# MKimiSH/video-filler

Measured on AMD Instinct MI355X. Metric: netG+netD fwd+bwd images/sec, 128x128 center-mask, higher is better.
Workload: dtype f32

## Files before the change

include/vf_hip.h:

```cpp
#ifndef VF_HIP_H
#define VF_HIP_H
#include <stddef.h>
#include <stdint.h>
#ifdef __cplusplus
extern "C" {
#endif

typedef struct vf_ctx vf_ctx;

enum { VF_ACT_NONE = 0, VF_ACT_LRELU = 1, VF_ACT_RELU = 2, VF_ACT_TANH = 3, VF_ACT_SIGMOID = 4 };

const char* vf_last_error(void);
int vf_version(void);
int vf_ctx_create(vf_ctx** out, int device, void* stream);
int vf_ctx_destroy(vf_ctx* ctx);
int vf_ctx_set_mfma_mode(vf_ctx* ctx, int mode);
int vf_ctx_set_stream(vf_ctx* ctx, void* stream);
int vf_ctx_set_workspace(vf_ctx* ctx, void* ptr, size_t bytes);
size_t vf_workspace_bytes_hint(void);
int vf_stream_synchronize(vf_ctx* ctx);
int vf_malloc(void** out, size_t bytes);
int vf_free(void* ptr);
int vf_memcpy_h2d(vf_ctx* ctx, void* dst, const void* src, size_t bytes);
int vf_memcpy_d2h(vf_ctx* ctx, void* dst, const void* src, size_t bytes);
// ... 192 lines not shown
                     float* pred_mapped, int B, int C, int fs, int overlapPred);

enum {
  VF_METRICS_N = 0, VF_METRICS_SSE = 1, VF_METRICS_SAE = 2, VF_METRICS_SSIM_Q = 3, VF_METRICS_SSIM_N = 4,
  VF_METRICS_FLICKER = 5, VF_METRICS_COLS = 6
};
int vf_frame_metrics(vf_ctx* ctx, const void* a, const void* b, int kind, int N, int C, int H, int W, int vh, int vw,
                     const unsigned char* mask, int clip, int64_t* table);

int vf_channel_copy(vf_ctx* ctx, const float* src, int Csrc, int c_src, float* dst, int Cdst, int c_dst, int Ccopy,
                    int64_t npix);
int vf_noise_fill(vf_ctx* ctx, float* out, int64_t n, uint64_t seed, const int32_t* counter_dev, uint64_t counter,
                  int normal);

int vf_wgrad_group_begin(vf_ctx* ctx);
int vf_wgrad_group_end(vf_ctx* ctx);
int vf_wgrad_group_abort(vf_ctx* ctx);
int vf_wgrad_group_count(vf_ctx* ctx, int* count);
int vf_wgrad_group_end_partial(vf_ctx* ctx, int count);

int vf_bias_grad_plan(int64_t P, int C, int* cq, int* rows_per_block, int* gx, int* gy);
int vf_bias_grad_multi(vf_ctx* ctx, const void* desc_dev, int n, int blocks1, int blocks2);

typedef struct vf_comm vf_comm;
#define VF_COMM_ID_BYTES 128
int vf_comm_available(void);
int vf_comm_unique_id(void* id128);
int vf_comm_init(vf_comm** out, const void* id128, int world, int rank);
int vf_comm_world(const vf_comm* c);
int vf_comm_rank(const vf_comm* c);
int vf_comm_allreduce_async(vf_comm* c, vf_ctx* ctx, void* buf, int64_t count, int dtype, int op, int* ticket);
int vf_comm_allreduce_avg_async(vf_comm* c, vf_ctx* ctx, float* buf, int64_t n, int* ticket);
int vf_comm_reduce_scatter_avg_async(vf_comm* c, vf_ctx* ctx, float* buf, int64_t shard_count, int* ticket);
int vf_comm_allgather_async(vf_comm* c, vf_ctx* ctx, float* buf, int64_t shard_count, int* ticket);
int vf_comm_broadcast_async(vf_comm* c, vf_ctx* ctx, float* buf, int64_t count, int root, int* ticket);
int vf_comm_wait(vf_comm* c, vf_ctx* ctx, int ticket);
int vf_comm_allreduce_inline(vf_comm* c, vf_ctx* ctx, void* buf, int64_t count, int dtype, int op);
int vf_comm_broadcast(vf_comm* c, vf_ctx* ctx, void* buf, int64_t count, int dtype, int root);
int vf_comm_barrier(vf_comm* c, vf_ctx* ctx);
int vf_comm_destroy(vf_comm* c);

int vf_prof_begin(vf_ctx* ctx);
int vf_prof_end(vf_ctx* ctx);
int vf_prof_count(void);
int vf_prof_get(int i, char* name, int name_cap, int64_t* launches, double* ms, double* flops, double* bytes);

enum { VF_L_CONV = 1, VF_L_FULLCONV = 2, VF_L_BN = 3, VF_L_ACT = 4, VF_L_VIEW = 5 };
typedef struct vf_layer_desc {
  int kind;
  int nin, nout;
  int k, stride, pad;
  int act;
  float slope;
  float eps, momentum;
} vf_layer_desc;
typedef struct vf_net vf_net;
int vf_net_create(vf_ctx* ctx, vf_net** out, const vf_layer_desc* layers, int nlayers, int B, int C, int H, int W);
int vf_net_destroy(vf_net* net);
int vf_net_reshape(vf_net* net, int B, int C, int H, int W);
int vf_net_parameters(vf_net* net, float** params, float** grads, int64_t* count);
int vf_net_bind_parameters(vf_net* net, float* params, float* grads, int64_t count);
int64_t vf_net_param_offset(const vf_net* net, int layer, int which, int64_t* length);
int vf_net_bn_running(vf_net* net, int layer, float** running_mean, float** running_var);
int vf_net_bind_bn_running(vf_net* net, int layer, float* running_mean, float* running_var);
int vf_net_bn_saved(vf_net* net, int layer, float** save_mean, float** save_invstd);
int vf_net_training(vf_net* net, int train);
int vf_net_zero_grad(vf_net* net);
int vf_net_zero_conv_biases(vf_net* net, vf_net* other);
int vf_net_forward(vf_net* net, const float* x, const float** y);
int vf_net_backward(vf_net* net, const float* x, const float* gy, const float** gx);
int vf_net_update_grad_input(vf_net* net, const float* x, const float* gy, const float** gx);
int vf_net_set_skip_input_grad(vf_net* net, int on);
int vf_net_set_batch_groups(vf_net* net, int G);
int vf_net_update_grad_input_group(vf_net* net, const float* x, const float* gy, int g, int G, const float** gx);
int vf_net_plan_size(const vf_net* net);
int vf_net_layer_has_act_bits(const vf_net* net, int layer);
int vf_net_bucket_split(const vf_net* net, double frac, int* plan_index, int64_t* flat_offset);
int vf_net_backward_range(vf_net* net, const float* x, const float* gy, int hi, int lo, int need_input_grad, const float** gx);
int vf_net_backward_split(vf_net* net, const float* x, const float* gy, int k, int need_input_grad, const float** gx);
int vf_net_backward_finish(vf_net* net);
int vf_net_set_fused_adam(vf_net* net, int on, int* count);
int vf_net_fused_adam_range(const vf_net* net, int i, int64_t* offset, int64_t* length);
int vf_net_adam_fused(vf_net* net, float* m, float* v, double beta1, double beta2, double eps, const int32_t* t_dev, int keep_grad);
int vf_net_fused_adam_pack_size(const vf_net* net, int64_t* floats);
int vf_net_fused_adam_pack(vf_net* net, float* segment);
int vf_net_adam_fused_gathered(vf_net* net, const float* all_segments, int world, int64_t seg_stride, float* m, float* v, double beta1,
                               double beta2, double eps, const int32_t* t_dev, int keep_grad);
int vf_net_fused_adam_rows_ok(const vf_net* net, int row_world);
int vf_net_fused_adam_row_range(const vf_net* net, int i, int row_rank, int row_world, int64_t* offset, int64_t* length);
int vf_net_forward_wait_fused(vf_net* net, vf_comm* comm, int ticket);
int vf_net_adam_fused_gathered_rows(vf_net* net, const float* all_segments, int world, int64_t seg_stride, float* m, float* v, double beta1,
                                    double beta2, double eps, const int32_t* t_dev, int keep_grad, int row_rank, int row_world);
int vf_net_set_sync_bn(vf_net* net, vf_comm* comm, int world, int force);
int vf_net_set_weight_planes_managed(vf_net* net, int on);
int vf_net_refresh_weight_planes(vf_net* net);
int vf_net_set_planes_gate(double min_gflop_per_pass, int min_rows);
int vf_net_layer_output(vf_net* net, int layer, const float** y);
int vf_net_layer_grad_input(vf_net* net, int layer, const float** gx);
int vf_net_layer_shape(const vf_net* net, int layer, int* B, int* C, int* H, int* W, int* Co, int* Ho, int* Wo);
int vf_net_bind_output(vf_net* net, int layer, float* y);
typedef int (*vf_net_act_observer)(void* user, int layer, float* y, int64_t numel);
int vf_net_set_act_observer(vf_net* net, vf_net_act_observer fn, void* user);

int vf_trace_available(void);
int vf_trace_enable(int on);
int vf_range_push(const char* name);
int vf_range_pop(void);
int vf_mark(const char* message);
int vf_range_depth(void);

#ifdef __cplusplus
}
#endif
#endif
```

video-filler_amd/_lib.py:

```python
import ctypes as C
import os
import re

_HERE = os.path.dirname(os.path.abspath(__file__))
_HEADER = os.path.join(_HERE, "..", "include", "vf_hip.h")

vp, f32, i32, i64, f64, sz, u64 = C.c_void_p, C.c_float, C.c_int, C.c_int64, C.c_double, C.c_size_t, C.c_uint64

SIGNATURES = {
    "vf_last_error": (C.c_char_p, []),
    "vf_version": (i32, []),
    "vf_ctx_create": (i32, [C.POINTER(vp), i32, vp]),
    "vf_ctx_destroy": (i32, [vp]),
    "vf_ctx_set_mfma_mode": (i32, [vp, i32]),
    "vf_ctx_set_stream": (i32, [vp, vp]),
    "vf_ctx_set_workspace": (i32, [vp, vp, sz]),
    "vf_workspace_bytes_hint": (sz, []),
    "vf_stream_synchronize": (i32, [vp]),
    "vf_malloc": (i32, [C.POINTER(vp), sz]),
    "vf_free": (i32, [vp]),
    "vf_memcpy_h2d": (i32, [vp, vp, vp, sz]),
    "vf_memcpy_d2h": (i32, [vp, vp, vp, sz]),
    "vf_zero": (i32, [vp, vp, sz]),
    "vf_zero_segments": (i32, [vp, vp, vp, vp, i32]),
# ... 60 lines not shown
    "vf_png_decode_workspace_bytes": (i32, [vp, vp, i32, i32, C.POINTER(sz), C.POINTER(sz)]),
    "vf_png_decode": (i32, [vp, vp, vp, i32, i32, vp, vp, vp, sz, vp, sz, vp]),
    "vf_png_bytes_to_float": (i32, [vp, vp, vp, i64]),
    "vf_png_workspace_bytes": (i32, [i32, i32, i32, i32, C.POINTER(sz), C.POINTER(sz)]),
    "vf_png_encode": (i32, [vp, vp, i32, i32, i32, i32, i32, vp, sz, vp, sz, vp]),
    "vf_jpeg_encode_workspace_bytes": (i32, [i32, i32, i32, i32, i32, C.POINTER(sz), C.POINTER(sz)]),
    "vf_jpeg_encode": (i32, [vp, vp, i32, i32, i32, i32, i32, i32, i32, vp, sz, vp, sz, vp]),
    "vf_jpeg_encode_opts_workspace_bytes": (i32, [i32] * 8 + [C.POINTER(sz), C.POINTER(sz)]),
    "vf_jpeg_encode_opts": (i32, [vp, vp] + [i32] * 10 + [vp, sz, vp, sz, vp]),
    "vf_gif_workspace_bytes": (i32, [i32, i32, i32, i32, C.POINTER(sz), C.POINTER(sz)]),
    "vf_gif_encode": (i32, [vp, vp, i32, i32, i32, i32, i32, i32, vp, sz, vp, sz, vp]),
    "vf_display_workspace_bytes": (i32, [i32] * 9 + [C.POINTER(sz)]),
    "vf_display_tensor": (i32, [vp, vp, i32, vp] + [i32] * 8 + [f64, i32, f64, i32, i32]),
    "vf_center_finish": (i32, [vp] * 6 + [i32] * 4),
    "vf_frame_metrics": (i32, [vp, vp, vp] + [i32] * 7 + [vp, i32, vp]),
    "vf_channel_copy": (i32, [vp, vp, i32, i32, vp, i32, i32, i32, i64]),
    "vf_noise_fill": (i32, [vp, vp, i64, u64, vp, u64, i32]),
    "vf_bce_fwd": (i32, [vp, vp, f32, i32, vp]),
    "vf_bce_bwd": (i32, [vp, vp, f32, vp, i32]),
    "vf_bce_fwd_bwd": (i32, [vp, vp, f32, f32, i32, i32, vp, vp, vp]),
    "vf_mse_fwd": (i32, [vp, vp, vp, i64, vp]),
    "vf_mse_bwd": (i32, [vp, vp, vp, vp, i64]),
    "vf_recon_grad_mix": (i32, [vp, vp, vp, vp, vp, f32, f32, f32, i32, i32, i32, i64, vp]),
    "vf_gdl_fwd": (i32, [vp, vp, vp, i32, i32, i32, i32, vp]),
    "vf_gdl_bwd": (i32, [vp, vp, vp, vp, i32, i32, i32, i32]),
    "vf_masked_mse_fwd": (i32, [vp, vp, vp, vp, f32, i64, vp]),
    "vf_masked_mse_bwd": (i32, [vp, vp, vp, vp, f32, vp, i64]),
    "vf_adam_step": (i32, [vp, vp, vp, vp, vp, i64, f64, f64, f64, f64, vp]),
    "vf_adam_prep": (i32, [vp, f64, f64, f64, vp]),
    "vf_adam_apply": (i32, [vp, vp, vp, vp, vp, i64, f64, f64, f64, vp]),
    "vf_adam_apply_ranges": (i32, [vp, vp, vp, vp, vp, C.POINTER(i64), C.POINTER(i64), i32, f64, f64, f64, vp]),
    "vf_wgrad_adam_outer_supported": (i32, [i32, i32, i32]),
    "vf_wgrad_adam_outer": (i32, [vp, vp, vp, i32, i32, i32, vp, vp, vp, vp, f64, f64, f64, vp]),
    "vf_wgrad_adam_outer_gathered": (i32, [vp, vp, vp, i32, i32, i64, i32, i32, vp, vp, vp, vp, C.c_float, f64, f64, f64, vp]),
    "vf_wgrad_adam_outer_rows": (i32, [vp, vp, vp, i32, i32, i64, i32, i32, i32, i32, vp, vp, vp, vp, C.c_float, f64, f64, f64, vp]),
    "vf_conv_is_fast": (i32, [i32, i32, i32, i32, i32]),
    "vf_conv2d_bwd_weight_planes": (i32, [vp, vp, vp, vp, vp, vp, vp, i32, i32, i32, i32, i32, i32, i32, i32, f32]),
    "vf_deconv2d_bwd_weight_planes": (i32, [vp, vp, vp, vp, vp, vp, vp, i32, i32, i32, i32, i32, i32, i32, i32, f32]),
    "vf_comm_available": (i32, []),
    "vf_comm_unique_id": (i32, [vp]),
    "vf_comm_init": (i32, [C.POINTER(vp), vp, i32, i32]),
    "vf_comm_world": (i32, [vp]),
    "vf_comm_rank": (i32, [vp]),
    "vf_comm_allreduce_async": (i32, [vp, vp, vp, i64, i32, i32, C.POINTER(i32)]),
    "vf_comm_allreduce_avg_async": (i32, [vp, vp, vp, i64, C.POINTER(i32)]),
    "vf_comm_reduce_scatter_avg_async": (i32, [vp, vp, vp, i64, C.POINTER(i32)]),
    "vf_comm_allgather_async": (i32, [vp, vp, vp, i64, C.POINTER(i32)]),
    "vf_comm_broadcast_async": (i32, [vp, vp, vp, i64, i32, C.POINTER(i32)]),
    "vf_comm_wait": (i32, [vp, vp, i32]),
    "vf_comm_allreduce_inline": (i32, [vp, vp, vp, i64, i32, i32]),
    "vf_comm_broadcast": (i32, [vp, vp, vp, i64, i32, i32]),
    "vf_comm_barrier": (i32, [vp, vp]),
    "vf_comm_destroy": (i32, [vp]),
    "vf_net_create": (i32, [vp, C.POINTER(vp), vp, i32, i32, i32, i32, i32]),
    "vf_net_destroy": (i32, [vp]),
    "vf_net_parameters": (i32, [vp, C.POINTER(vp), C.POINTER(vp), C.POINTER(i64)]),
    "vf_net_param_offset": (i64, [vp, i32, i32, C.POINTER(i64)]),
    "vf_net_bn_running": (i32, [vp, i32, C.POINTER(vp), C.POINTER(vp)]),
    "vf_net_training": (i32, [vp, i32]),
    "vf_net_zero_grad": (i32, [vp]),
    "vf_net_forward": (i32, [vp, vp, C.POINTER(vp)]),
    "vf_net_backward": (i32, [vp, vp, vp, C.POINTER(vp)]),
    "vf_net_update_grad_input": (i32, [vp, vp, vp, C.POINTER(vp)]),
    "vf_net_layer_output": (i32, [vp, i32, C.POINTER(vp)]),
    "vf_net_layer_grad_input": (i32, [vp, i32, C.POINTER(vp)]),
    "vf_net_layer_shape": (i32, [vp, i32] + [C.POINTER(i32)] * 7),
    "vf_net_reshape": (i32, [vp, i32, i32, i32, i32]),
    "vf_net_bind_parameters": (i32, [vp, vp, vp, i64]),
    "vf_net_bind_bn_running": (i32, [vp, i32, vp, vp]),
    "vf_net_bn_saved": (i32, [vp, i32, C.POINTER(vp), C.POINTER(vp)]),
    "vf_net_zero_conv_biases": (i32, [vp, vp]),
    "vf_net_set_skip_input_grad": (i32, [vp, i32]),
    "vf_net_set_batch_groups": (i32, [vp, i32]),
    "vf_net_update_grad_input_group": (i32, [vp, vp, vp, i32, i32, C.POINTER(vp)]),
    "vf_net_plan_size": (i32, [vp]),
    "vf_net_layer_has_act_bits": (i32, [vp, i32]),
    "vf_net_bucket_split": (i32, [vp, f64, C.POINTER(i32), C.POINTER(i64)]),
    "vf_net_backward_range": (i32, [vp, vp, vp, i32, i32, i32, C.POINTER(vp)]),
    "vf_net_backward_split": (i32, [vp, vp, vp, i32, i32, C.POINTER(vp)]),
    "vf_net_backward_finish": (i32, [vp]),
    "vf_net_set_fused_adam": (i32, [vp, i32, C.POINTER(i32)]),
    "vf_net_fused_adam_range": (i32, [vp, i32, C.POINTER(i64), C.POINTER(i64)]),
    "vf_net_adam_fused": (i32, [vp, vp, vp, f64, f64, f64, vp, i32]),
    "vf_net_fused_adam_pack_size": (i32, [vp, C.POINTER(i64)]),
    "vf_net_fused_adam_pack": (i32, [vp, vp]),
    "vf_net_adam_fused_gathered": (i32, [vp, vp, i32, i64, vp, vp, f64, f64, f64, vp, i32]),
    "vf_net_fused_adam_rows_ok": (i32, [vp, i32]),
    "vf_net_fused_adam_row_range": (i32, [vp, i32, i32, i32, C.POINTER(i64), C.POINTER(i64)]),
    "vf_net_forward_wait_fused": (i32, [vp, vp, i32]),
    "vf_net_adam_fused_gathered_rows": (i32, [vp, vp, i32, i64, vp, vp, f64, f64, f64, vp, i32, i32, i32]),
    "vf_net_set_sync_bn": (i32, [vp, vp, i32, i32]),
    "vf_net_set_weight_planes_managed": (i32, [vp, i32]),
    "vf_net_refresh_weight_planes": (i32, [vp]),
    "vf_net_set_planes_gate": (i32, [f64, i32]),
    "vf_net_bind_output": (i32, [vp, i32, vp]),
    "vf_net_set_act_observer": (i32, [vp, vp, vp]),
    "vf_trace_available": (i32, []),
    "vf_trace_enable": (i32, [i32]),
    "vf_range_push": (i32, [C.c_char_p]),
    "vf_range_pop": (i32, []),
    "vf_mark": (i32, [C.c_char_p]),
    "vf_range_depth": (i32, []),
    "vf_wgrad_group_count": (i32, [vp, C.POINTER(i32)]),
    "vf_wgrad_group_end_partial": (i32, [vp, i32]),
    "vf_prof_begin": (i32, [vp]),
    "vf_prof_end": (i32, [vp]),
    "vf_prof_count": (i32, []),
    "vf_prof_get": (i32, [i32, C.c_char_p, i32, C.POINTER(i64), C.POINTER(f64), C.POINTER(f64), C.POINTER(f64)]),
}


def header_symbols():
    with open(_HEADER) as fh:
        text = re.sub(r"/\*.*?\*/", "", fh.read(), flags=re.S)
    return sorted(set(re.findall(r"\b(vf_[a-z0-9_]+)\s*\(", text)))


def lib_path():
    return os.environ.get("VF_HIP_LIB") or os.path.join(_HERE, "lib", "libvf_hip.so")


_LIB = None


def load():
    global _LIB
    if _LIB is None:
        path = lib_path()
        if not os.path.exists(path):
            raise RuntimeError(
                "video-filler_amd: %s is missing — run `python -c 'import __graft_entry__ as g; g.build()'` "
                "(hipcc --offload-arch=gfx950).  There is no CPU fallback." % path)
        lib = C.CDLL(path)
        for name, (res, args) in SIGNATURES.items():
            fn = getattr(lib, name)
            fn.restype = res
            fn.argtypes = args
        _LIB = lib
    return _LIB


class VfError(RuntimeError):
    pass


def check(rc):
    if rc != 0:
        raise VfError(load().vf_last_error().decode())
```

video-filler_amd/build.py:

```python
import glob
import os
import subprocess
import sys

HERE = os.path.dirname(os.path.abspath(__file__))
SRC = ["vf_core.hip", "vf_bn.hip", "vf_conv.hip", "vf_conv_generic.hip", "vf_pipeline.hip", "vf_image.hip", "vf_jpeg.hip", "vf_png.hip", "vf_png_decode.hip", "vf_jpeg_enc.hip", "vf_gif.hip", "vf_display.hip", "vf_metrics.hip", "vf_pgemm.hip", "vf_conv_thin.hip", "vf_comm.hip", "vf_wgrad_small.hip", "vf_smallm.hip", "vf_trace.hip", "vf_net.hip"]
HIPCC = os.environ.get("HIPCC", "/opt/rocm/bin/hipcc")
FLAGS = ["--offload-arch=gfx950", "-O3", "-std=c++17", "-fPIC", "-fvisibility=hidden", "-ffp-contract=off",
         "-Wall", "-Wno-unused-function", "-Xclang", "-target-feature", "-Xclang", "-packed-fp32-ops"]


def lib_path():
    return os.path.join(HERE, "lib", "libvf_hip.so")


def build(force=False, verbose=False):
    csrc = os.path.join(HERE, "csrc")
    objdir = os.path.join(HERE, "lib", "obj")
    os.makedirs(objdir, exist_ok=True)
    hdrs = glob.glob(os.path.join(csrc, "*.h")) + [os.path.join(HERE, "..", "include", "vf_hip.h")]
    hdr_m = max(os.path.getmtime(h) for h in hdrs)
    objs, rebuilt = [], False
    procs = []
    for s in SRC:
        src = os.path.join(csrc, s)
        obj = os.path.join(objdir, s.replace(".hip", ".o"))
        objs.append(obj)
        if force or not os.path.exists(obj) or os.path.getmtime(obj) < max(os.path.getmtime(src), hdr_m):
            cmd = [HIPCC, *FLAGS, "-c", src, "-o", obj]
            if verbose:
                print(" ".join(cmd))
            procs.append((s, subprocess.Popen(cmd, stdout=subprocess.PIPE, stderr=subprocess.STDOUT)))
            rebuilt = True
    for s, p in procs:
        out, _ = p.communicate()
        if p.returncode != 0:
            sys.stderr.write(out.decode())
            raise RuntimeError("hipcc failed on " + s)
        if verbose and out:
            print("\n".join(ln for ln in out.decode().split("\n") if "-packed-fp32-ops' is not a recognized feature" not in ln))
    so = lib_path()
    if rebuilt or not os.path.exists(so):
        subprocess.check_call([HIPCC, "--offload-arch=gfx950", "-shared", "-fPIC", "-o", so, *objs, "-ldl"])
    return so


if __name__ == "__main__":
    print(build(force="--force" in sys.argv, verbose=True))
```

video-filler_amd/cnet.py:

```python
import ctypes as C

import torch

from . import _lib, nn
from .backend import ACT, get_backend, param_version, tensor_from_ptr, to_nhwc

VF_L_CONV, VF_L_FULLCONV, VF_L_BN, VF_L_ACT, VF_L_VIEW = 1, 2, 3, 4, 5


class LayerDesc(C.Structure):
    _fields_ = [("kind", C.c_int), ("nin", C.c_int), ("nout", C.c_int), ("k", C.c_int), ("stride", C.c_int), ("pad", C.c_int),
                ("act", C.c_int), ("slope", C.c_float), ("eps", C.c_float), ("momentum", C.c_float)]


_OBSERVER = C.CFUNCTYPE(C.c_int, C.c_void_p, C.c_int, C.c_void_p, C.c_int64)


def layer_descs(mods):
    arr = (LayerDesc * len(mods))()
    for i, m in enumerate(mods):
        if isinstance(m, nn.SpatialConvolution):
            arr[i] = LayerDesc(VF_L_FULLCONV if m._is_full else VF_L_CONV, m.nInputPlane, m.nOutputPlane, m.kH, m.dH, m.padH, 0, 0.0, 0.0, 0.0)
        elif isinstance(m, nn.SpatialBatchNormalization):
            arr[i] = LayerDesc(VF_L_BN, 0, m.nOutputPlane, 0, 0, 0, 0, 0.0, m.eps, m.momentum)
# ... 86 lines not shown
        def _sync_comm(v):
            if v[0] > 1:
                return comm
            return comm if (v[1] and comm is not None and lib.vf_comm_world(comm) == v[0]) else None
        self._push("sync", sync + (getattr(comm, "value", None),),
                   lambda v: lib.vf_net_set_sync_bn(self._net, _sync_comm(v), v[0], 1 if v[1] else 0))
        hook = nn.Sequential.act_hook
        if (hook is not None) != (self._cb is not None):
            if hook is not None:
                self._cb = _OBSERVER(self._observe)
                _lib.check(lib.vf_net_set_act_observer(self._net, C.cast(self._cb, C.c_void_p), None))
            else:
                _lib.check(lib.vf_net_set_act_observer(self._net, None, None))
                self._cb = None
        return lib

    def _push(self, key, value, fn):
        if self._pushed.get(key, None) != value:
            _lib.check(fn(value))
            self._pushed[key] = value

    def _sync_state(self):
        bns = [m for m in self.leaves() if isinstance(m, nn.SpatialBatchNormalization)]
        world = max([m.sync_world for m in bns] + [1])
        force = any(m.sync_force for m in bns)
        return (world, force)

    def _observe(self, user, layer, ptr, numel):
        try:
            a = self._layers[layer]
            lib = _lib.load()
            dims = [C.c_int() for _ in range(7)]
            prod = layer - 1 if (layer > 0 and not isinstance(self._layers[layer - 1], (nn._Act, nn.View))) else layer
            _lib.check(lib.vf_net_layer_shape(self._net, prod, *[C.byref(d) for d in dims]))
            Bn, _, _, _, Co, Ho, Wo = [d.value for d in dims]
            assert Bn * Co * Ho * Wo == numel
            y = tensor_from_ptr(ptr, (Bn, Ho, Wo, Co), get_backend().device).permute(0, 3, 1, 2)
            edited = nn.Sequential.act_hook(a, y)
            return 0 if edited is False else 1
        except BaseException as e:
            self._cb_error = e
            return -1

    def _call(self, fn, *args):
        rc = fn(*args)
        if self._cb_error is not None:
            e, self._cb_error = self._cb_error, None
            raise e
        _lib.check(rc)

    def _final_shape(self):
        lib = _lib.load()
        dims = [C.c_int() for _ in range(7)]
        last = max(i for i, m in enumerate(self._layers) if not isinstance(m, (nn.View,)))
        _lib.check(lib.vf_net_layer_shape(self._net, last, *[C.byref(d) for d in dims]))
        Bn, _, _, _, Co, Ho, Wo = [d.value for d in dims]
        return Bn, Co, Ho, Wo

    def updateOutput(self, input, before=None):
        assert before is None, "stream joins in mid-forward belong to the module-by-module mirror"
        assert torch.is_tensor(input), "vf_net hosts chain nets (tensor in, tensor out)"
        x = to_nhwc(input)
        lib = self._ensure(x)
        if self._wp_managed and self._wp_stale():
            self.refresh_weight_planes()
        yp = C.c_void_p()
        self._call(lib.vf_net_forward, self._net, C.c_void_p(x.data_ptr()), C.byref(yp))
        Bn, Co, Ho, Wo = self._final_shape()
        y = tensor_from_ptr(yp.value, (Bn, Ho, Wo, Co), x.device).permute(0, 3, 1, 2)
        tail = self._layers[-1]
        if isinstance(tail, nn.View):
            y = y.reshape(Bn, *tail.sizes)
        self.output = y
        return y

    def _entry_input_shape(self, lo):
        plan = self._plan or self._build_plan()
        lib = _lib.load()
        dims = [C.c_int() for _ in range(7)]
        _lib.check(lib.vf_net_layer_shape(self._net, self._index[id(plan[lo][0])], *[C.byref(d) for d in dims]))
        Bn, Cc, H, W = [d.value for d in dims[:4]]
        return Bn, Cc, H, W

    def set_fused_adam(self, on=True):
        assert self._net is not None, "set_fused_adam after the first forward"
        lib = _lib.load()
        cnt = C.c_int()
        _lib.check(lib.vf_net_set_fused_adam(self._net, 1 if on else 0, C.byref(cnt)))
        self._fused_ranges = []
        for i in range(cnt.value):
            o, n = C.c_int64(), C.c_int64()
            _lib.check(lib.vf_net_fused_adam_range(self._net, i, C.byref(o), C.byref(n)))
            self._fused_ranges.append((o.value, o.value + n.value))
        return list(self._fused_ranges)

    def fused_adam_ranges(self):
        return list(getattr(self, "_fused_ranges", []))

    def adam_fused(self, m, v, beta1, beta2, eps, t_dev, keep_grad=False):
        _lib.check(_lib.load().vf_net_adam_fused(self._net, C.c_void_p(m.data_ptr()), C.c_void_p(v.data_ptr()), beta1, beta2, eps,
                                                 C.c_void_p(t_dev.data_ptr()), 1 if keep_grad else 0))

    def fused_adam_pack_size(self):
        n = C.c_int64()
        _lib.check(_lib.load().vf_net_fused_adam_pack_size(self._net, C.byref(n)))
        return n.value

    def fused_adam_pack(self, segment):
        assert segment.is_contiguous() and segment.numel() >= self.fused_adam_pack_size()
        _lib.check(_lib.load().vf_net_fused_adam_pack(self._net, C.c_void_p(segment.data_ptr())))

    def adam_fused_gathered(self, all_segments, world, m, v, beta1, beta2, eps, t_dev, keep_grad=False, rows=None):
        seg = all_segments.numel() // world
        assert seg * world == all_segments.numel() and seg % 4 == 0
        args = (self._net, C.c_void_p(all_segments.data_ptr()), world, seg, C.c_void_p(m.data_ptr()), C.c_void_p(v.data_ptr()), beta1,
                beta2, eps, C.c_void_p(t_dev.data_ptr()), 1 if keep_grad else 0)
        if rows is None:
            _lib.check(_lib.load().vf_net_adam_fused_gathered(*args))
        else:
            _lib.check(_lib.load().vf_net_adam_fused_gathered_rows(*args, int(rows[0]), int(rows[1])))

    def fused_adam_rows_ok(self, ranks):
        return self._net is not None and bool(_lib.load().vf_net_fused_adam_rows_ok(self._net, int(ranks)))

    def fused_adam_row_ranges(self, ranks):
        lib = _lib.load()
        out = []
        for i in range(len(self.fused_adam_ranges())):
            per = []
            for r in range(ranks):
                o, n = C.c_int64(), C.c_int64()
                _lib.check(lib.vf_net_fused_adam_row_range(self._net, i, r, int(ranks), C.byref(o), C.byref(n)))
                per.append((o.value, o.value + n.value))
            out.append(per)
        return out

    def forward_wait_fused(self, comm, tickets):
        for t in tickets:
            _lib.check(_lib.load().vf_net_forward_wait_fused(self._net, comm, int(t)))

    def backward_finish(self):
        if self._net is not None:
            _lib.check(_lib.load().vf_net_backward_finish(self._net))

    def _walk(self, input, gradOutput, want_gp, need_input_grad=True, hi=None, lo=0, group=None, defer_cut=None):
        assert self._net is not None, "backward before forward"
        lib = _lib.load()
        x = to_nhwc(input)
        g = to_nhwc(gradOutput) if gradOutput.dim() == 4 else gradOutput.contiguous()
        if self._wp_managed and self._wp_stale():
            self.refresh_weight_planes()
        gxp = C.c_void_p()
        xp, gp = C.c_void_p(x.data_ptr()), C.c_void_p(g.data_ptr())
        if group is not None:
            assert not want_gp and hi is None and lo == 0
            self._call(lib.vf_net_update_grad_input_group, self._net, xp, gp, group[0], group[1], C.byref(gxp))
        elif want_gp and defer_cut is not None:
            assert hi is None and lo == 0
            self._call(lib.vf_net_backward_split, self._net, xp, gp, int(defer_cut), 1 if need_input_grad else 0, C.byref(gxp))
        elif want_gp:
            self._call(lib.vf_net_backward_range, self._net, xp, gp, -1 if hi is None else hi, lo, 1 if need_input_grad else 0, C.byref(gxp))
        else:
            assert hi is None and lo == 0, "updateGradInput walks the whole net"
            self._call(lib.vf_net_update_grad_input, self._net, xp, gp, C.byref(gxp))
        out = None
        if gxp.value:
            Bn, Cc, H, W = self._entry_input_shape(lo)
            if group is not None:
                Bn //= group[1]
            out = tensor_from_ptr(gxp.value, (Bn, H, W, Cc), x.device).permute(0, 3, 1, 2)
        if lo == 0:
            self.gradInput = out
        return out

    def refresh_weight_planes(self):
        if self._flat is not None:
            self._wp_version = param_version(self._flat[0])
        if self._net is not None:
            _lib.check(_lib.load().vf_net_refresh_weight_planes(self._net))

    def setBatchGroups(self, G):
        super().setBatchGroups(G)
        self._groups = int(G)
        return self

    def zeroConvBiases(self):
        if self._net is None:
            return super().zeroConvBiases()
        _lib.check(_lib.load().vf_net_zero_conv_biases(self._net, None))

    def zeroConvBiasesWith(self, other):
        if self._net is None or not isinstance(other, CNet) or other._net is None:
            self.zeroConvBiases()
            other.zeroConvBiases()
            return
        _lib.check(_lib.load().vf_net_zero_conv_biases(self._net, other._net))

    def zeroGradParameters(self):
        if self.lazy_zero:
            if self._net is not None:
                _lib.check(_lib.load().vf_net_zero_grad(self._net))
        elif self._flat is not None:
            get_backend().zero(self._flat[1])

    def redirect_last_output(self, cur, buf):
        if self._net is None or self.output is None or cur.data_ptr() != self.output.data_ptr() or tuple(cur.shape) != tuple(buf.shape):
            return False
        last = max(i for i, m in enumerate(self._layers) if isinstance(m, nn.SpatialConvolution))
        _lib.check(_lib.load().vf_net_bind_output(self._net, last, C.c_void_p(buf.data_ptr())))
        return True

    def layer_output(self, i):
        lib = _lib.load()
        p = C.c_void_p()
        _lib.check(lib.vf_net_layer_output(self._net, i, C.byref(p)))
        dims = [C.c_int() for _ in range(7)]
        j = i
        while j > 0 and isinstance(self._layers[j], (nn._Act, nn.View)):
            j -= 1
        _lib.check(lib.vf_net_layer_shape(self._net, j, *[C.byref(d) for d in dims]))
        Bn, _, _, _, Co, Ho, Wo = [d.value for d in dims]
        return tensor_from_ptr(p.value, (Bn, Ho, Wo, Co), get_backend().device).permute(0, 3, 1, 2)


def adopt_if_chain(seq):
    return CNet.adopt(seq) if is_chain(seq) else seq
```

video-filler_amd/csrc/vf_common.h:

```cpp
#pragma once
#include <hip/hip_runtime.h>
#include <hip/hip_ext.h>

#include <cstdarg>
#include <cstdint>
#include <cstdio>
#include <cstring>

#include "../../include/vf_hip.h"
#include "vf_internal.h"

#define VF_API extern "C" __attribute__((visibility("default")))

struct VfBnSt {
  int mode;
  const float* vec;
  const float* x;
  double* part;
  int rows_per_group;
  int tiles_per_group;
  int zpar;
};
struct VfBnRequest {
  VfBnSt st = {};
// ... 142 lines not shown
    const size_t o = at;
    at += vf_up256(bytes);
    return o;
  }
};
static inline int vf_check_encode_entry(const char* who, int kind, const char* ch, const char* batch, size_t ws_bytes, size_t ws_need,
                                        size_t out_cap, size_t out_need) {
  VF_REQUIRE(kind == 0 || kind == 1, "%s: kind %d is not 0 (float N x %s x H x W) or 1 (uint8 N x H x W x %s)", who, kind, ch, ch);
  VF_REQUIRE(ws_bytes >= ws_need, "%s: the workspace holds %zu bytes, %s need %zu", who, ws_bytes, batch, ws_need);
  VF_REQUIRE(out_cap >= out_need, "%s: the output holds %zu bytes, %s may take %zu", who, out_cap, batch, out_need);
  return 0;
}
#define VF_OOB 0x80000000u

struct VfColsumDesc {
  const float* g;
  float* gb;
  double* part;
  int64_t P;
  int C, cq, rows_per_block, gx, gy;
  int blk1_off, blk2_off;
  float beta;
};
static_assert(sizeof(VfColsumDesc) == 64, "descriptor layout is shared with the host mirror");
struct VfWpDesc {
  const float* w;
  void* nat;
  void* tr;
  int d0, d1;
  int gx, gz;
  int blk_off;
  int pad;
};
static_assert(sizeof(VfWpDesc) == 48, "descriptor layout is shared with the host mirror");

template <class G>
static inline bool vf_plan_bn_stats(VfConvExtras* ex, G& g, int bm, int gm, int zpar) {
  g.st.mode = 0;
  if (!ex || !ex->bn.st.mode) return false;
  const VfBnRequest& r = ex->bn;
  VfBnSt st = r.st;
  st.zpar = g.ksplit == 1 ? zpar : 1;
  if (g.ksplit == 1) {
    if (g.M % r.groups != 0 || (g.M / r.groups) % bm != 0 || (int64_t)(gm / r.groups) * zpar > r.rows_cap) return false;
    st.tiles_per_group = gm / r.groups;
  } else if (!vf_internal_slab_st_ok(g.out_elems, g.N, r.groups, r.rows_cap, &st.tiles_per_group)) {
    return false;
  }
  st.rows_per_group = st.tiles_per_group * st.zpar;
  g.st = st;
  ex->bn_result_rows = st.rows_per_group;
  if (st.mode == 2) {
    g.dmask = r.yact;
    g.dact = r.act;
    g.dslope = r.slope;
  }
  return g.ksplit > 1;
}

__device__ __forceinline__ void vf_adam_upd(float& xv, float gv, float& mv, float& vv, float b1, float omb1, float b2, float omb2,
                                            float eps, float step) {
  float mi = mv * b1;
  mi = mi + omb1 * gv;
  float vi = vv * b2;
  vi = vi + (omb2 * gv) * gv;
  float d = sqrtf(vi);
  d = d + eps;
  mv = mi;
  vv = vi;
  xv = xv - (step * mi) / d;
}

struct VfFusedLayer {
  const float *U, *V;
  float *x, *m, *v, *g_out;
  int K, Nu, Ncols;
  int kps;
  int64_t seg;
  float gscale;
  int row0, ldu;
};
#define VF_FUSED_MAX 4

__device__ __forceinline__ float vf_act_apply(float v, int act, float slope) {
  switch (act) {
    case VF_ACT_LRELU: return v > 0.f ? v : v * slope;
    case VF_ACT_RELU: return v > 0.f ? v : 0.f;
    case VF_ACT_TANH: return tanhf(v);
    case VF_ACT_SIGMOID: return 1.f / (1.f + expf(-v));
    default: return v;
  }
}
__device__ __forceinline__ float vf_act_grad(float y, float g, int act, float slope) {
  switch (act) {
    case VF_ACT_LRELU: return y > 0.f ? g : g * slope;
    case VF_ACT_RELU: return y > 0.f ? g : 0.f;
    case VF_ACT_TANH: return g * (1.f - y * y);
    case VF_ACT_SIGMOID: return g * (1.f - y) * y;
    default: return g;
  }
}
```

video-filler_amd/csrc/vf_conv.hip:

```cpp
#include <algorithm>
#include <vector>
#include <cstdlib>

#include "vf_device.h"

template <int LD>
__device__ __forceinline__ bf16x8 vf_tr_frag(const __bf16* tile, int col0, int k0, int lane) {
  const int grp = lane >> 4, i = lane & 15;
  const __bf16* a = tile + (k0 + 8 * (grp >> 1) + (i >> 2)) * LD + col0 + 16 * (grp & 1) + 4 * (i & 3);
  typedef __attribute__((address_space(3))) bf16x4 lds_bf16x4;
  const bf16x4 lo = __builtin_amdgcn_ds_read_tr16_b64_v4bf16((lds_bf16x4*)a);
  const bf16x4 hi = __builtin_amdgcn_ds_read_tr16_b64_v4bf16((lds_bf16x4*)(a + 4 * LD));
  return __builtin_shufflevector(lo, hi, 0, 1, 2, 3, 4, 5, 6, 7);
}

struct IGemm {
  const float* A;
  const float* Wt;
  const float* bias;
  float* Y;
  float* slab;
  int64_t out_elems;
  unsigned a_bytes, w_bytes;
  int M, lgMh, lgMw;
// ... 1442 lines not shown
  int64_t v_elems() const { return (int64_t)B * Hv * Wv * Cv; }
  bool in_range(int bytes) const { return u_elems() * bytes < ((int64_t)1 << 31) && v_elems() * bytes < ((int64_t)1 << 31); }
  WgRoute fp32_route() const { return vecU && vecV && (ksplit == 1 || total % 4 == 0) ? WG_FP32_GROUP : WG_FP32_SINGLE; }
  int blocks() const { return gx * gy * ksplit; }
  size_t slab_bytes() const { return ksplit > 1 ? vf_up256((size_t)ksplit * total * sizeof(float)) : 0; }
  double flops() const { return 2.0 * (double)P * Nu * 16.0 * Cv; }
};
static WgPlan wg_plan(vf_ctx* ctx, const VfConvShape& s, bool full, const float* U, const float* V, const void* Up, const void* Vp) {
  const int mode = ctx->mfma_bf16;
  WgPlan p;
  p.B = s.B; p.stride = s.stride; p.pad = s.pad;
  p.Hl = full ? s.H : s.out_h(); p.Wl = full ? s.W : s.out_w(); p.Nu = full ? s.Cin : s.Cout;
  p.Hv = full ? s.full_out_h() : s.H; p.Wv = full ? s.full_out_w() : s.W; p.Cv = full ? s.Cout : s.Cin;
  p.P = s.B * p.Hl * p.Wl;
  p.vecU = (p.Nu % 4 == 0) && vf_aligned16(U);
  p.vecV = (p.Cv % 4 == 0) && vf_aligned16(V);
  p.nk = (int)vf_cdiv(p.P, mode ? 32 : 16);
  p.bm = p.Nu > 64 ? 128 : 64;
  p.gy = (int)vf_cdiv(p.Nu, p.bm);
  p.gx = (int)vf_cdiv(16 * (int64_t)p.Cv, 128);
  p.total = (int64_t)p.Nu * 16 * p.Cv;
  const bool pw64 = p.Nu == 64 && mode == 3;
  const bool use_pw = Up && Vp && (mode == 3 || mode == 1) && s.stride == 2 && s.pad == 1 && (p.Nu % 128 == 0 || pw64) && p.Cv % 64 == 0 &&
                      p.P % 32 == 0 && p.in_range(6) && p.total % 4 == 0;
  p.target = use_pw && !pw64 ? 256 : 512;
  const int64_t tiles = (int64_t)p.gx * p.gy;
  p.ksplit = 1;
  if (tiles < p.target * 3 / 4 && p.nk >= 16) {
    p.ksplit = (int)std::min<int64_t>(p.nk / 8, vf_cdiv(p.target, tiles));
    while (p.ksplit > 1 && (size_t)p.ksplit * p.total * sizeof(float) > vf_ws_avail(ctx)) --p.ksplit;
    if (p.ksplit < 1) p.ksplit = 1;
    const int steps = (int)vf_cdiv(p.nk, p.ksplit);
    p.ksplit = (int)vf_cdiv(p.nk, steps);
  }
  p.route = p.is_bottleneck() ? WG_SMALLK : use_pw ? (pw64 ? WG_PLANES_64 : WG_PLANES_128) : p.fp32_route();
  p.rider = p.is_bottleneck() && (mode == 3 || mode == 1) && p.bm == 128 && p.ksplit == 1 && (16 * p.Cv) % 128 == 0 && p.vecU && p.vecV;
  return p;
}
template <class D>
static D wg_desc_base(const WgPlan& p, float beta) {
  D d;
  memset(&d, 0, sizeof(d));
  d.P = p.P; d.lgMh = vf_ilog2(p.Hl); d.lgMw = vf_ilog2(p.Wl);
  d.Nu = p.Nu; d.Cv = p.Cv; d.Hv = p.Hv; d.Wv = p.Wv;
  d.gx = p.gx; d.gy = p.gy; d.gz = p.ksplit;
  d.ksplit = p.ksplit; d.nk = p.nk;
  d.beta = beta;
  return d;
}
static WGrad wg_desc(const WgPlan& p, const float* U, const float* V, float* dW, float* slab, float beta) {
  WGrad g = wg_desc_base<WGrad>(p, beta);
  g.U = U; g.V = V; g.dW = dW; g.slab = slab;
  g.u_bytes = (unsigned)(p.u_elems() * 4);
  g.v_bytes = (unsigned)(p.v_elems() * 4);
  g.stride = p.stride; g.pad = p.pad;
  g.ntaps = 16;
  return g;
}
static VfPWGrad wg_desc_planes(const WgPlan& p, const void* Up, const void* Vp, float* dW, float* slab, float beta) {
  VfPWGrad w = wg_desc_base<VfPWGrad>(p, beta);
  w.Up = Up; w.Vp = Vp;
  w.out = p.ksplit > 1 ? slab : dW;
  w.u_ps = (unsigned)(p.u_elems() * 2);
  w.v_ps = (unsigned)(p.v_elems() * 2);
  return w;
}
static VfPWGrad wg_desc_rider(const WgPlan& p, const float* U, const float* V, float* dW, float beta) {
  VfPWGrad w = wg_desc_base<VfPWGrad>(p, beta);
  w.Uf = U; w.Vf = V;
  w.out = dW;
  return w;
}

struct WgRec {
  WgPlan p;
  WGrad g;
  VfPWGrad pw;
  int bf;
};
struct WgRecorder {
  std::vector<WgRec> recs;
  size_t ws_used = 0;
  bool open = false;
  void clear() {
    recs.clear();
    ws_used = 0;
  }
  bool reserve(size_t bytes, size_t avail, size_t* off) {
    if (ws_used + bytes > avail) return false;
    *off = ws_used;
    ws_used += bytes;
    return true;
  }
};
static WgRecorder& wg_recorder(vf_ctx* ctx) {
  if (!ctx->wg) ctx->wg = new WgRecorder();
  return *ctx->wg;
}
void vf_internal_wg_free(vf_ctx* ctx) {
  delete ctx->wg;
  ctx->wg = nullptr;
}
template <class F>
static void wg_dispatch(int bm, int bf, F&& f) {
  auto with_mode = [&](auto BM) {
    if (bf == 3) f(BM, VfIntC<3>{});
    else if (bf) f(BM, VfIntC<1>{});
    else f(BM, VfIntC<0>{});
  };
  if (bm == 128) with_mode(VfIntC<128>{});
  else with_mode(VfIntC<64>{});
}
template <class Table, int CAP, class Pick, class Put, class Launch>
static int wg_pack(const std::vector<WgRec>& recs, int align, Pick&& pick, Put&& put, Launch&& launch) {
  Table G;
  int blocks = 0;
  double work = 0;
  G.n = 0;
  auto fire = [&]() -> int {
    if (G.n == 0) return 0;
    G.blk_off[G.n] = blocks;
    const int rc = launch(G, blocks, work);
    G.n = 0;
    blocks = 0;
    work = 0;
    return rc;
  };
  for (const WgRec& r : recs) {
    if (!pick(r)) continue;
    G.blk_off[G.n] = blocks;
    blocks += (put(G.d[G.n], r, work) + align - 1) / align * align;
    if (++G.n == CAP)
      if (int rc = fire()) return rc;
  }
  return fire();
}
static int wg_flush(vf_ctx* ctx) {
  WgRecorder& R = wg_recorder(ctx);
  if (R.recs.empty()) return 0;
  bool any_planes = false;
  for (const WgRec& r : R.recs) any_planes |= (r.bf == 4);
  if (any_planes)
    for (WgRec& r : R.recs)
      if (r.p.rider) r.bf = 4;
  const int rc = wg_pack<VfPWGradGroup, VF_PWG_MAX>(
      R.recs, 8, [](const WgRec& r) { return r.bf == 4; },
      [](VfPWGrad& d, const WgRec& r, double& fl) {
        d = r.pw;
        fl += r.p.flops();
        return d.gx * d.gy * d.gz;
      },
      [&](const VfPWGradGroup& G, int blocks, double fl) {
        int n64 = 0;
        for (int i = 0; i < G.n; ++i) n64 += G.d[i].Up != nullptr && G.d[i].Nu == 64;
        const char* name = n64 == 0 ? "pwgrad_group_128x128x32" : (n64 == G.n ? "pwgrad_group_64x128x32" : "pwgrad_group_64+128x128x32");
        return vf_internal_pwgrad_group(ctx, G, blocks, name, fl);
      });
  if (rc) return rc;
  for (int bm : {128, 64})
    for (int bf : {3, 1, 0})
      wg_pack<WGradGroup, VF_WG_GROUP_MAX>(
          R.recs, 8, [&](const WgRec& r) { return r.p.bm == bm && r.bf == bf; },
          [](WGrad& d, const WgRec& r, double& fl) {
            d = r.g;
            fl += r.p.flops();
            return r.p.blocks();
          },
          [&](const WGradGroup& G, int blocks, double fl) {
            char name[64];
            snprintf(name, sizeof(name), "wgrad_group_%dx128%s", bm, bf == 3 ? "_bf16x3" : (bf ? "_bf16" : ""));
            wg_dispatch(bm, bf, [&](auto BM, auto BF) {
              VF_LAUNCH_TIMED(ctx, name, fl, 0.0, (k_wgrad_group<decltype(BM)::value, true, true, decltype(BF)::value>), dim3(blocks),
                              dim3(256), G);
            });
            return 0;
          });
  VF_LAUNCH_CHECK();
  wg_pack<SlabGroup, VF_WG_GROUP_MAX>(
      R.recs, 1, [](const WgRec& r) { return r.g.ksplit > 1; },
      [](auto& d, const WgRec& r, double& bytes) {
        d.slab = r.g.slab;
        d.dst = r.g.dW;
        d.total4 = r.p.total / 4;
        d.ksplit = r.g.ksplit;
        d.beta = r.g.beta;
        bytes += 4.0 * (double)r.p.total * (r.g.ksplit + 1);
        return (int)vf_cdiv(r.p.total / 4, 64);
      },
      [&](const SlabGroup& S, int blocks, double bytes) {
        VfProf prof(ctx, "slab_reduce_wgrad_group", 0.0, bytes);
        hipLaunchKernelGGL(k_slab_reduce4_group, dim3(blocks), dim3(256), 0, ctx->stream, S);
        return 0;
      });
  VF_LAUNCH_CHECK();
  R.clear();
  return 0;
}
VF_API int vf_wgrad_group_begin(vf_ctx* ctx) {
  WgRecorder& R = wg_recorder(ctx);
  if (R.open) R.clear();
  R.open = true;
  return 0;
}
VF_API int vf_wgrad_group_abort(vf_ctx* ctx) {
  WgRecorder& R = wg_recorder(ctx);
  R.clear();
  R.open = false;
  return 0;
}
VF_API int vf_wgrad_group_end(vf_ctx* ctx) {
  WgRecorder& R = wg_recorder(ctx);
  VF_REQUIRE(R.open, "vf_wgrad_group_end: no group is open");
  R.open = false;
  return wg_flush(ctx);
}

VF_API int vf_wgrad_group_count(vf_ctx* ctx, int* count) {
  VF_REQUIRE(count != nullptr, "vf_wgrad_group_count: NULL");
  WgRecorder& R = wg_recorder(ctx);
  *count = R.open ? (int)R.recs.size() : 0;
  return 0;
}
VF_API int vf_wgrad_group_end_partial(vf_ctx* ctx, int count) {
  WgRecorder& R = wg_recorder(ctx);
  VF_REQUIRE(R.open, "vf_wgrad_group_end_partial: no group is open");
  if (R.recs.empty() || count <= 0) return 0;
  std::vector<WgRec> rest;
  if (count < (int)R.recs.size()) {
    rest.assign(R.recs.begin() + count, R.recs.end());
    R.recs.resize((size_t)count);
  }
  const size_t used = R.ws_used;
  const int rc = wg_flush(ctx);
  R.recs = rest;
  R.ws_used = used;
  return rc;
}

static int wgrad(vf_ctx* ctx, const float* U, const float* V, float* dW, const VfConvShape& s, bool full, float beta, const void* Up,
                 const void* Vp) {
  WgPlan p = wg_plan(ctx, s, full, U, V, Up, Vp);
  if (p.route == WG_SMALLK) {
    const int rc = vf_internal_wgrad_smallk(ctx, U, V, dW, p.B, p.Nu, 16 * p.Cv, beta);
    if (rc >= 0) return rc;
    p.route = p.fp32_route();
  }
  VF_REQUIRE(p.in_range(4), "operand exceeds the 2 GiB buffer-descriptor range");
  WgRecorder& R = wg_recorder(ctx);
  auto slab_at = [&](size_t off) { return p.ksplit > 1 ? (float*)(vf_ws_ptr(ctx) + off) : nullptr; };
  size_t off = 0;
  if (p.planes() || (R.open && p.route == WG_FP32_GROUP)) {
    if (!R.reserve(p.slab_bytes(), vf_ws_avail(ctx), &off)) {
      if (int rc = wg_flush(ctx)) return rc;
      R.clear();
      VF_REQUIRE(R.reserve(p.slab_bytes(), vf_ws_avail(ctx), &off), "workspace too small for this layer's split-K slabs");
    }
    WgRec r;
    r.p = p;
    r.g = wg_desc(p, U, V, dW, slab_at(off), beta);
    r.bf = p.planes() ? 4 : ctx->mfma_bf16;
    if (p.planes()) r.pw = wg_desc_planes(p, Up, Vp, dW, r.g.slab, beta);
    else if (p.rider) r.pw = wg_desc_rider(p, U, V, dW, beta);
    R.recs.push_back(r);
    return R.open ? 0 : wg_flush(ctx);
  }
  float* slab = slab_at(0);
  if (R.open) {
    if (R.reserve(p.slab_bytes(), vf_ws_avail(ctx), &off)) slab = slab_at(off);
    else if (int rc = wg_flush(ctx)) return rc;
  }
  const WGrad g = wg_desc(p, U, V, dW, slab, beta);
  const int bf = ctx->mfma_bf16;
  const char* wname = p.bm == 128 ? (bf == 3 ? "wgrad_128x128_bf16x3" : bf ? "wgrad_128x128_bf16" : "wgrad_128x128")
                                  : (bf == 3 ? "wgrad_64x128_bf16x3" : bf ? "wgrad_64x128_bf16" : "wgrad_64x128");
  const double wfl = p.flops();
  const dim3 grid((unsigned)p.blocks()), block(256);
  wg_dispatch(p.bm, bf, [&](auto BM, auto BF) {
    constexpr int bm_ = decltype(BM)::value, bf_ = decltype(BF)::value;
    if (p.vecU && p.vecV) VF_LAUNCH_TIMED(ctx, wname, wfl, 0.0, (k_wgrad<bm_, true, true, bf_>), grid, block, g);
    else if (p.vecU) VF_LAUNCH_TIMED(ctx, wname, wfl, 0.0, (k_wgrad<bm_, true, false, bf_>), grid, block, g);
    else if (p.vecV) VF_LAUNCH_TIMED(ctx, wname, wfl, 0.0, (k_wgrad<bm_, false, true, bf_>), grid, block, g);
    else VF_LAUNCH_TIMED(ctx, wname, wfl, 0.0, (k_wgrad<bm_, false, false, bf_>), grid, block, g);
  });
  VF_LAUNCH_CHECK();
  if (p.ksplit > 1) {
    VfProf prof(ctx, "slab_reduce_wgrad", 0.0, 4.0 * (double)p.total * (p.ksplit + 1));
    return launch_slab_reduce(ctx, g.slab, dW, nullptr, p.total, 1, p.ksplit, VF_ACT_NONE, 0.f, beta);
  }
  return 0;
}

VF_API int vf_conv_is_fast(int H, int W, int k, int stride, int pad) { return VfConvShape{0, H, W, 0, 0, k, stride, pad}.matrix_core_conv(); }

int vf_internal_conv2d_fwd(vf_ctx* ctx, const float* x, const float* w, const float* bias, float* y, const VfConvShape& s, int act,
                           float slope, VfConvExtras* ex) {
  if (!s.matrix_core_conv()) return vf_internal_gconv_fwd(ctx, x, w, bias, y, s, act, slope);
  if (int rc = check_conv_args(s)) return rc;
  if (s.stride == 2 && s.Cin == 3 && !ex->bn.st.mode) {
    const int rc = vf_internal_conv_thin_fwd(ctx, x, w, bias, y, nullptr, s, act, slope, ex);
    if (rc >= 0) return rc;
  }
  return conv_like_fwd(ctx, x, w, bias, y, s, act, slope, ex);
}
VF_API int vf_conv2d_fwd(vf_ctx* ctx, const float* x, const float* w, const float* bias, float* y, int B, int H, int W,
                         int Cin, int Cout, int k, int stride, int pad, int act, float slope) {
  const VfConvShape s{B, H, W, Cin, Cout, k, stride, pad};
  return vf_take_pending(ctx, [&](VfConvExtras* ex) { return vf_internal_conv2d_fwd(ctx, x, w, bias, y, s, act, slope, ex); });
}

int vf_internal_conv2d_bwd_data(vf_ctx* ctx, const float* gy, const float* w, float* gx, const VfConvShape& s, VfConvExtras* ex) {
  if (!s.matrix_core_conv()) return vf_internal_gconv_bwd_data(ctx, gy, w, gx, s);
  if (int rc = check_conv_args(s)) return rc;
  if (s.stride == 1) {
    VF_REQUIRE(s.H == 4 && s.W == 4, "stride-1 conv data-grad is built for the 4x4 bottleneck input only");
    if (s.Cout == 1) {
      const int64_t n = (int64_t)s.B * 16 * s.Cin;
      hipLaunchKernelGGL(k_dot_bwd_data, dim3((int)vf_cdiv(n, 256)), dim3(256), 0, ctx->stream, gy, w, gx, s.B, 16 * s.Cin, ex->dot_act_y,
                         ex->dot_act, ex->dot_act_slope);
      VF_LAUNCH_CHECK();
      return 0;
    }
  }
  return conv_like_bwd(ctx, gy, w, nullptr, gx, s.gradient_of_conv(), VF_ACT_NONE, 0.f, ex);
}
VF_API int vf_conv2d_bwd_data(vf_ctx* ctx, const float* gy, const float* w, float* gx, int B, int H, int W, int Cin,
                              int Cout, int k, int stride, int pad) {
  const VfConvShape s{B, H, W, Cin, Cout, k, stride, pad};
  return vf_take_pending(ctx, [&](VfConvExtras* ex) { return vf_internal_conv2d_bwd_data(ctx, gy, w, gx, s, ex); });
}

int vf_internal_conv2d_bwd_data_act(vf_ctx* ctx, const float* gy, const float* w, float* gx, const float* x_act, int act, float slope,
                                    const VfConvShape& s, VfConvExtras* ex) {
  if (int rc = check_conv_args(s)) return rc;
  VF_REQUIRE(x_act != nullptr && (act == VF_ACT_LRELU || act == VF_ACT_RELU),
             "vf_conv2d_bwd_data_act: needs the activated input and a (leaky) ReLU");
  VF_REQUIRE(s.stride == 2, "vf_conv2d_bwd_data_act: only the stride-2 layers follow a bare conv + activation pair");
  return conv_like_bwd(ctx, gy, w, nullptr, gx, s.gradient_of_conv(), VF_ACT_NONE, 0.f, ex, x_act, act, slope);
}
VF_API int vf_conv2d_bwd_data_act(vf_ctx* ctx, const float* gy, const float* w, float* gx, const float* x_act, int act,
                                  float slope, int B, int H, int W, int Cin, int Cout, int k, int stride, int pad) {
  const VfConvShape s{B, H, W, Cin, Cout, k, stride, pad};
  return vf_take_pending(ctx, [&](VfConvExtras* ex) { return vf_internal_conv2d_bwd_data_act(ctx, gy, w, gx, x_act, act, slope, s, ex); });
}

int vf_internal_conv2d_bwd_weight(vf_ctx* ctx, const float* x, const float* gy, const void* x_planes, const void* gy_planes, float* gw,
                                  float* gb, const VfConvShape& s, float beta, const VfConvExtras* ex) {
  if (!s.matrix_core_conv()) return vf_internal_gconv_bwd_weight(ctx, x, gy, gw, gb, s, beta);
  if (int rc = check_conv_args(s)) return rc;
  if (s.Cout == 1 && s.stride == 1 && s.H == 4 && s.W == 4) {
    const VfConvExtras plain;
    if (!ex) ex = &plain;
    hipLaunchKernelGGL(k_dot_bwd_weight, dim3((int)vf_cdiv(16 * s.Cin, 64)), dim3(512), 0, ctx->stream, x, gy, gw, gb, s.B,
                       16 * s.Cin, beta, ex->dot_act_y, ex->dot_act, ex->dot_act_slope);
    VF_LAUNCH_CHECK();
    return 0;
  }
  if (int rc = wgrad(ctx, gy, x, gw, s, false, beta, gy_planes, x_planes)) return rc;
  if (gb) return vf_internal_colsum(ctx, gy, gb, (int64_t)s.B * s.out_h() * s.out_w(), s.Cout, beta);
  return 0;
}
VF_API int vf_conv2d_bwd_weight(vf_ctx* ctx, const float* x, const float* gy, float* gw, float* gb, int B, int H, int W,
                                int Cin, int Cout, int k, int stride, int pad, float beta) {
  return vf_conv2d_bwd_weight_planes(ctx, x, gy, nullptr, nullptr, gw, gb, B, H, W, Cin, Cout, k, stride, pad, beta);
}
VF_API int vf_conv2d_bwd_weight_planes(vf_ctx* ctx, const float* x, const float* gy, const void* x_planes, const void* gy_planes,
                                       float* gw, float* gb, int B, int H, int W, int Cin, int Cout, int k, int stride, int pad,
                                       float beta) {
  return vf_internal_conv2d_bwd_weight(ctx, x, gy, x_planes, gy_planes, gw, gb, VfConvShape{B, H, W, Cin, Cout, k, stride, pad}, beta, nullptr);
// ... 40 lines not shown
```

video-filler_amd/csrc/vf_internal.h:

```cpp
#pragma once
struct vf_ctx; struct VfBnSt; struct VfBnRequest; struct VfConvExtras; struct VfPWGradGroup; struct VfFusedLayer; struct WgRecorder;

struct VfConvShape {
  int B, H, W, Cin, Cout, k, stride, pad;
  int out_h() const { return (H + 2 * pad - k) / stride + 1; }
  int out_w() const { return (W + 2 * pad - k) / stride + 1; }
  int full_out_h() const { return (H - 1) * stride - 2 * pad + k; }
  int full_out_w() const { return (W - 1) * stride - 2 * pad + k; }
  bool pow2_map() const { return H > 0 && (H & (H - 1)) == 0 && W > 0 && (W & (W - 1)) == 0; }
  bool main_net_taps() const { return k == 4 && ((stride == 2 && pad == 1) || (stride == 1 && pad == 0)); }
  bool matrix_core_conv() const { return main_net_taps() && (stride == 2 || (H == 4 && W == 4)) && pow2_map(); }
  VfConvShape gradient_of_conv() const { return {B, out_h(), out_w(), Cout, Cin, k, stride, pad}; }
  VfConvShape gradient_of_full() const { return {B, full_out_h(), full_out_w(), Cout, Cin, k, stride, pad}; }
};

void vf_internal_wg_free(vf_ctx* ctx);
int vf_internal_slab_reduce(vf_ctx* ctx, const float* slab, float* dst, const float* bias, int64_t total, int N, int ksplit, int act,
                            float slope, const float* dmask, int dact, float dslope, const VfBnSt* st, int st_groups);
bool vf_internal_slab_st_ok(int64_t total, int N, int groups, int rows_cap, int* blocks_per_group);
int vf_internal_conv2d_fwd(vf_ctx* ctx, const float* x, const float* w, const float* bias, float* y, const VfConvShape& s, int act,
                           float slope, VfConvExtras* ex);
int vf_internal_conv2d_bwd_data(vf_ctx* ctx, const float* gy, const float* w, float* gx, const VfConvShape& s, VfConvExtras* ex);
int vf_internal_conv2d_bwd_data_act(vf_ctx* ctx, const float* gy, const float* w, float* gx, const float* x_act, int act, float slope,
                                    const VfConvShape& s, VfConvExtras* ex);
int vf_internal_conv2d_bwd_weight(vf_ctx* ctx, const float* x, const float* gy, const void* x_planes, const void* gy_planes, float* gw,
                                  float* gb, const VfConvShape& s, float beta, const VfConvExtras* ex);
int vf_internal_deconv2d_fwd(vf_ctx* ctx, const float* x, const float* w, const float* bias, float* y, const VfConvShape& s, int act,
                             float slope, VfConvExtras* ex);
int vf_internal_deconv2d_bwd_data(vf_ctx* ctx, const float* gy, const float* w, float* gx, const VfConvShape& s, VfConvExtras* ex);
int vf_internal_deconv2d_bwd_weight(vf_ctx* ctx, const float* x, const float* gy, const void* x_planes, const void* gy_planes, float* gw,
                                    float* gb, const VfConvShape& s, float beta);
int vf_internal_bn_request_fwd(VfBnRequest* r, const float* shift, double* part, int part_rows_cap, int groups);
int vf_internal_bn_request_bwd(VfBnRequest* r, const float* x, const float* y_act, int act, float slope, const float* save_mean,
                               double* part, int part_rows_cap, int groups);

int vf_internal_conv2d_fwd_planes(vf_ctx* ctx, const float* x, const float* w, const float* bias, float* y, void* y_planes,
                                  const VfConvShape& s, int act, float slope, VfConvExtras* ex);
int vf_internal_conv_thin_fwd(vf_ctx* ctx, const float* x, const float* w, const float* bias, float* y, void* y_planes,
                              const VfConvShape& s, int act, float slope, VfConvExtras* ex);
int vf_internal_deconv_thin_out(vf_ctx* ctx, const float* x, const float* w, const float* bias, float* y, const VfConvShape& s, int act,
                                float slope);

int vf_internal_gconv_fwd(vf_ctx* ctx, const float* x, const float* w, const float* bias, float* y, const VfConvShape& s, int act,
                          float slope);
int vf_internal_gconv_bwd_data(vf_ctx* ctx, const float* gy, const float* w, float* gx, const VfConvShape& s);
int vf_internal_gconv_bwd_weight(vf_ctx* ctx, const float* x, const float* gy, float* gw, float* gb, const VfConvShape& s, float beta);

bool vf_internal_pconv_supported(int mfma_mode, const VfConvShape& s, bool transposed);
int vf_internal_pconv_gather(vf_ctx* ctx, const void* ap, const void* wp, const float* bias, float* y, const VfConvShape& s, int act,
                             float slope, VfConvExtras* ex);
int vf_internal_pconv_scatter(vf_ctx* ctx, const void* ap, const void* wp, const float* bias, float* y, const VfConvShape& s, int act,
                              float slope, const float* dmask, int dact, float dslope, VfConvExtras* ex);
int vf_internal_pwgrad_group(vf_ctx* ctx, const VfPWGradGroup& G, int blocks, const char* name, double flops);

int vf_internal_smallm_plan(int form, int M, int N, int K, size_t ws_bytes);
int vf_internal_smallm_launch(vf_ctx* ctx, int form, const float* A, const float* W, float* slab, int M, int N, int K, int ksplit);

int vf_internal_wgrad_smallk(vf_ctx* ctx, const float* U, const float* V, float* dW, int K, int Nu, int Ncols, float beta);
int vf_internal_adam_fused_multi(vf_ctx* ctx, const VfFusedLayer* layers, int nl, double beta1, double beta2, double eps,
                                 const int32_t* t_dev);

int vf_internal_colsum(vf_ctx* ctx, const float* g, float* gb, int64_t P, int C, float beta);
```

video-filler_amd/csrc/vf_net.hip:

```cpp
#include <algorithm>
#include <cstdlib>
#include <cstring>
#include <map>
#include <string>
#include <vector>

#include "vf_common.h"

namespace {

double g_gate_gflop = getenv("VF_PCONV_MIN_GFLOP") ? atof(getenv("VF_PCONV_MIN_GFLOP")) : 3.0;
int g_gate_rows = getenv("VF_PCONV_MIN_ROWS") ? atoi(getenv("VF_PCONV_MIN_ROWS")) : 1024;
const bool g_no_pconv = getenv("VF_NO_PCONV") != nullptr;
const bool g_no_bn_fuse = getenv("VF_NO_BN_FUSE") != nullptr;
const bool g_pwgrad = !(getenv("VF_PWGRAD") && strcmp(getenv("VF_PWGRAD"), "1") != 0);

struct Layer {
  vf_layer_desc d;
  int C = 0, H = 0, W = 0;
  int Co = 0, Ho = 0, Wo = 0;
  int64_t w_off = -1, b_off = -1, w_n = 0, b_n = 0;
  float* y = nullptr;
  float* y_own = nullptr;
  float* gx = nullptr;
  float* gtmp = nullptr;
  float *rm = nullptr, *rv = nullptr, *sm = nullptr, *si = nullptr;
  double* sums = nullptr;
  double* part = nullptr;
  int part_rows_cap = 0;
  void* xp = nullptr;
  void* gp = nullptr;
  void* yp = nullptr;
  void* bgp = nullptr;
  unsigned* ybits = nullptr;
  bool bits_live = false;
  const void* out_planes = nullptr;
  const void* grad_planes = nullptr;
  void *wp_nat = nullptr, *wp_tr = nullptr;
  bool wp_live = false;
  int wp_mode = 0;
  const float* x_seen = nullptr;
  const void* xp_seen = nullptr;
  const float* g_seen = nullptr;
  const void* gp_seen = nullptr;
  int fused_act = VF_ACT_NONE;
  float fused_slope = 0.f;
  bool absorbed = false;
  bool fresh = true;
  bool fa = false;
  const float *fa_u = nullptr, *fa_v = nullptr;
  int fa_k = 0;
  VfConvShape shape(int Bn) const { return {Bn, H, W, C, Co, d.k, d.stride, d.pad}; }
  VfConvShape grad_shape(int Bn) const { return d.kind == VF_L_FULLCONV ? shape(Bn).gradient_of_full() : shape(Bn).gradient_of_conv(); }
};

struct Entry {
  int main;
  int act;
};

inline bool is_conv(const Layer& l) { return l.d.kind == VF_L_CONV || l.d.kind == VF_L_FULLCONV; }
inline bool is_full(const Layer& l) { return l.d.kind == VF_L_FULLCONV; }
inline bool is_s2(const Layer& l) { return l.d.k == 4 && l.d.stride == 2 && l.d.pad == 1; }
inline bool relu_like(int act) { return act == VF_ACT_LRELU || act == VF_ACT_RELU; }

}

struct vf_net {
  vf_ctx* ctx = nullptr;
  int B = 0, C0 = 0, H0 = 0, W0 = 0;
  std::vector<Layer> L;
  std::vector<Entry> plan;
  float *params = nullptr, *grads = nullptr;
  float *params_own = nullptr, *grads_own = nullptr;
  int64_t nparams = 0;
  bool train = true;
  int groups = 1;
  int gcap = 0;
  bool skip_input_grad = false;
  bool wp_managed = false;
  int act_done_at = -1;
  int bn_pre_at = -1, bn_pre_rows = 0;
  vf_comm* comm = nullptr;
  int sync_world = 1;
  bool sync_force = false;
  vf_net_act_observer observer = nullptr;
  void* observer_user = nullptr;
  std::map<std::string, std::pair<void*, std::vector<int>>> colsum_plans;
  void* wp_table = nullptr;
  int wp_n = 0, wp_blocks = 0;
  std::vector<int> wp_key;
  int64_t* bias_offs = nullptr;
  int64_t* bias_lens = nullptr;
  int nbias = 0;
  struct BothTable {
    int64_t *offs, *lens;
    const float *base, *other_base;
  };
  std::map<const vf_net*, BothTable> both_tables;
  bool fused_adam = false;
  std::vector<int> fa_layers;
  vf_comm* fwd_wait_comm = nullptr;
  std::vector<int> fwd_wait_tickets;
  bool split_pending = false;
  std::string pending_bias;
  std::vector<void*> owned;
  std::vector<void*> act_owned;
};

namespace {

int net_alloc(std::vector<void*>& pool, void** out, size_t bytes) {
  void* p = nullptr;
  VF_CHECK_HIP(hipMalloc(&p, bytes ? bytes : 4));
  pool.push_back(p);
  *out = p;
  return 0;
}

bool sync_on(const vf_net* n) { return (n->comm && n->sync_world > 1) || n->sync_force; }
bool bn_fusable(const vf_net* n, const Layer& l) { return n->train && !sync_on(n) && l.C % 4 == 0 && !g_no_bn_fuse; }

bool pconv_layer(const Layer& l) {
  return is_conv(l) && is_s2(l) && std::min(l.d.nin, l.d.nout) >= 32 && l.d.nin % 4 == 0 && l.d.nout % 4 == 0;
}
bool pconv_ok(const vf_net* n, const Layer& l, const VfConvShape& s, bool transposed) {
  const int mode = n->ctx->mfma_bf16;
  if (g_no_pconv || (mode != 3 && mode != 1) || !is_s2(l)) return false;
  const int64_t rows = (int64_t)s.B * s.H * s.W / (transposed ? 1 : 4);
  const double gflop = 2.0 * (double)rows * 16.0 * s.Cin * s.Cout * 1e-9;
  if (rows < g_gate_rows || gflop < g_gate_gflop) return false;
  return vf_internal_pconv_supported(mode, s, transposed);
}

int ensure_planes(vf_net* n, void** slot, int64_t numel) {
  if (*slot) return 0;
  return net_alloc(n->act_owned, slot, (size_t)numel * 6);
}

const float* entry_out(const vf_net* n, int idx, const float* x_in) {
  for (int e = idx; e >= 0; --e) {
    const Layer& l = n->L[n->plan[e].main];
    if (l.y) return l.y;
  }
  return x_in;
}

int run_observer(vf_net* n, int act_layer, float* y, int64_t numel, const void* planes) {
  if (!n->observer) return 0;
  VF_CHECK_HIP(hipGetLastError());
  const int edited = n->observer(n->observer_user, act_layer, y, numel);
  if (edited < 0) {
    vf_set_error("vf_net: the activation observer reported an error at layer %d", act_layer);
    return 2;
  }
  if (edited > 0 && planes) return vf_planes_split(n->ctx, y, const_cast<void*>(planes), numel);
  return 0;
}

int weight_planes(vf_net* n, Layer& l, bool transposed, const void** out) {
  const float* w = n->params + l.w_off;
  const int d0 = is_full(l) ? l.d.nin : l.d.nout, d1 = is_full(l) ? l.d.nout : l.d.nin;
  if (!l.wp_live || l.wp_mode != n->ctx->mfma_bf16) {
    if (!l.wp_nat) {
      if (int rc = net_alloc(n->owned, &l.wp_nat, (size_t)l.w_n * 6)) return rc;
      if (int rc = net_alloc(n->owned, &l.wp_tr, (size_t)l.w_n * 6)) return rc;
    }
    if (int rc = vf_weight_planes(n->ctx, w, l.wp_nat, l.wp_tr, d0, d1)) return rc;
    l.wp_live = true;
    l.wp_mode = n->ctx->mfma_bf16;
  }
  *out = transposed ? l.wp_tr : l.wp_nat;
  return 0;
}

int refresh_weight_planes(vf_net* n) {
  if (g_no_pconv || (n->ctx->mfma_bf16 != 3 && n->ctx->mfma_bf16 != 1)) return 0;
  std::vector<int> live;
  for (size_t i = 0; i < n->L.size(); ++i)
    if (n->L[i].wp_live && n->L[i].wp_mode == n->ctx->mfma_bf16) live.push_back((int)i);
  if (live.empty()) return 0;
  if (live != n->wp_key || !n->wp_table) {
    std::vector<VfWpDesc> desc(live.size());
    int blocks = 0;
    for (size_t j = 0; j < live.size(); ++j) {
      Layer& l = n->L[live[j]];
      const int d0 = is_full(l) ? l.d.nin : l.d.nout, d1 = is_full(l) ? l.d.nout : l.d.nin;
      const int gx = (d0 + 31) / 32, gz = (d1 + 31) / 32;
      desc[j] = VfWpDesc{n->params + l.w_off, l.wp_nat, l.wp_tr, d0, d1, gx, gz, blocks, 0};
      blocks += gx * 16 * gz;
    }
    void* dev = nullptr;
    if (int rc = net_alloc(n->owned, &dev, desc.size() * sizeof(VfWpDesc))) return rc;
    VF_CHECK_HIP(hipMemcpy(dev, desc.data(), desc.size() * sizeof(VfWpDesc), hipMemcpyHostToDevice));
    n->wp_table = dev;
    n->wp_n = (int)live.size();
    n->wp_blocks = blocks;
    n->wp_key = live;
  }
  return vf_weight_planes_multi(n->ctx, n->wp_table, n->wp_n, n->wp_blocks);
}

int conv_forward(vf_net* n, Layer& l, const float* x, const void* in_planes, int Bn, int act, float slope, bool want_planes,
                 VfConvExtras* ex) {
  vf_ctx* ctx = n->ctx;
  const float* w = n->params + l.w_off;
  const float* b = n->params + l.b_off;
  const bool full = is_full(l);
  const VfConvShape s = l.shape(Bn);
  l.out_planes = nullptr;
  l.bits_live = false;
  const bool simple_act = act == VF_ACT_NONE || relu_like(act);
  if (want_planes && !full && l.C == 3 && simple_act && is_s2(l) && l.Co % 64 == 0 && l.H % 16 == 0 && l.W % 16 == 0) {
    if (int rc = ensure_planes(n, &l.yp, (int64_t)n->B * l.Ho * l.Wo * l.Co)) return rc;
    if (relu_like(act) && !n->observer) {
      if (!l.ybits)
        if (int rc = net_alloc(n->act_owned, (void**)&l.ybits, sizeof(unsigned) * (size_t)n->B * l.Ho * l.Wo * (l.Co / 32))) return rc;
      ex->act_bits_out = l.ybits;
    }
    const int frc = vf_internal_conv2d_fwd_planes(ctx, x, w, b, l.y, l.yp, s, act, slope, ex);
    l.bits_live = ex->act_bits_written && relu_like(act) && !n->observer;
    if (frc) return frc;
    l.out_planes = l.yp;
    l.x_seen = nullptr;
    return 0;
  }
  if (simple_act && pconv_ok(n, l, s, full)) {
    const void* xp = in_planes;
    if (!xp) {
      if (int rc = ensure_planes(n, &l.xp, (int64_t)n->B * l.H * l.W * l.C)) return rc;
      if (int rc = vf_planes_split(ctx, x, l.xp, (int64_t)Bn * l.H * l.W * l.C)) return rc;
      xp = l.xp;
    }
    l.x_seen = x;
    l.xp_seen = xp;
    const void* wp = nullptr;
    if (int rc = weight_planes(n, l, full, &wp)) return rc;
    return full ? vf_internal_pconv_scatter(ctx, xp, wp, b, l.y, s, act, slope, nullptr, VF_ACT_NONE, 0.f, ex)
                : vf_internal_pconv_gather(ctx, xp, wp, b, l.y, s, act, slope, ex);
  }
// ... 15 lines not shown
    if (int rc = ensure_planes(n, &l.yp, (int64_t)n->B * l.H * l.W * l.C)) return rc;
    yp = l.yp;
  }
  if (pre_rows > 0) {
    int rc = vf_bn_train_fwd_pre(ctx, l.part, pre_rows, x, l.y, gamma, beta, l.rm, l.rv, l.sm, l.si, l.sums, npix / G, l.C, G,
                                 l.d.momentum, l.d.eps, act, slope, yp);
    l.out_planes = yp;
    return rc;
  }
  if (!sync_on(n)) {
    int rc = yp ? vf_bn_train_fwd_planes(ctx, x, l.y, gamma, beta, l.rm, l.rv, l.sm, l.si, l.sums, npix / G, l.C, G, l.d.momentum,
                                         l.d.eps, act, slope, yp)
                : vf_bn_train_fwd_groups(ctx, x, l.y, gamma, beta, l.rm, l.rv, l.sm, l.si, l.sums, npix / G, l.C, G, l.d.momentum,
                                         l.d.eps, act, slope);
    l.out_planes = yp;
    return rc;
  }
  VF_REQUIRE(G == 1, "SyncBN with batch groups is not part of the path");
  if (int rc = vf_bn_stats(ctx, x, l.rm, l.sums, npix, l.C)) return rc;
  if (n->comm)
    if (int rc = vf_comm_allreduce_inline(n->comm, ctx, l.sums, 2 * l.C, 1, 0)) return rc;
  if (int rc = vf_bn_finalize(ctx, l.sums, l.rm, l.rv, l.sm, l.si, npix * n->sync_world, l.C, l.d.momentum, l.d.eps)) return rc;
  return vf_bn_apply(ctx, x, l.y, gamma, beta, l.sm, l.si, npix, l.C, act, slope);
}

int conv_bwd_data(vf_net* n, Layer& l, const float* x, const float* go, int Bn, int in_act, float in_slope, const void* g_planes,
                  VfConvExtras* ex) {
  vf_ctx* ctx = n->ctx;
  const float* w = n->params + l.w_off;
  const bool full = is_full(l);
  const VfConvShape s = l.shape(Bn), gs = l.grad_shape(Bn);
  if (pconv_ok(n, l, gs, !full) && (in_act == VF_ACT_NONE || !full)) {
    const void* gp = g_planes;
    if (!gp) {
      if (int rc = ensure_planes(n, &l.gp, (int64_t)n->B * l.Ho * l.Wo * l.Co)) return rc;
      if (int rc = vf_planes_split(ctx, go, l.gp, (int64_t)Bn * l.Ho * l.Wo * l.Co)) return rc;
      gp = l.gp;
    }
    l.g_seen = go;
    l.gp_seen = gp;
    const void* wp = nullptr;
    if (int rc = weight_planes(n, l, !full, &wp)) return rc;
    if (full) return vf_internal_pconv_gather(ctx, gp, wp, nullptr, l.gx, gs, VF_ACT_NONE, 0.f, ex);
    return vf_internal_pconv_scatter(ctx, gp, wp, nullptr, l.gx, gs, VF_ACT_NONE, 0.f, in_act != VF_ACT_NONE ? x : nullptr, in_act, in_slope,
                                     ex);
  }
  l.g_seen = nullptr;
  if (in_act != VF_ACT_NONE)
    return vf_internal_conv2d_bwd_data_act(ctx, go, w, l.gx, x, in_act, in_slope, s, ex);
  return full ? vf_internal_deconv2d_bwd_data(ctx, go, w, l.gx, s, ex) : vf_internal_conv2d_bwd_data(ctx, go, w, l.gx, s, ex);
}

struct Deferred {
  const float* g;
  float* gb;
  int64_t P;
  int C;
  float beta;
};

int conv_acc(vf_net* n, Layer& l, const float* x, const float* go, int Bn, std::vector<Deferred>* deferred, const VfConvExtras* ex) {
  vf_ctx* ctx = n->ctx;
  const bool full = is_full(l);
  float* gw = n->grads + l.w_off;
  float* gb = n->grads + l.b_off;
  const float beta = l.fresh ? 0.f : 1.f;
  l.fresh = false;
  if (deferred && l.Co % 4 == 0 && ((uintptr_t)go & 15) == 0) {
    deferred->push_back(Deferred{go, gb, (int64_t)Bn * l.Ho * l.Wo, l.Co, beta});
    gb = nullptr;
  }
  VF_REQUIRE(!(n->fused_adam && l.fa && l.fa_k > 0 && beta != 0.f),
             "fused Adam: a second backward pass accumulates onto a weight gradient that was never written (one backward per zeroGradParameters)");
  if (n->fused_adam && l.fa && beta == 0.f) {
    l.fa_u = full ? x : go;
    l.fa_v = full ? go : x;
    l.fa_k = Bn;
    l.g_seen = nullptr;
    l.gp_seen = nullptr;
    if (!gb) return 0;
    return vf_internal_colsum(ctx, go, gb, (int64_t)Bn * l.Ho * l.Wo, l.Co, beta);
  }
  l.fa_k = 0;
  const bool planes = g_pwgrad && !g_no_pconv && l.x_seen == x && l.xp_seen && l.g_seen == go && l.gp_seen;
  const void *xp = l.xp_seen, *gp = l.gp_seen;
  l.g_seen = nullptr;
  l.gp_seen = nullptr;
  if (!planes) xp = gp = nullptr;
  return full ? vf_internal_deconv2d_bwd_weight(ctx, x, go, xp, gp, gw, gb, l.shape(Bn), beta)
              : vf_internal_conv2d_bwd_weight(ctx, x, go, xp, gp, gw, gb, l.shape(Bn), beta, ex);
}

int bn_backward(vf_net* n, Layer& l, const float* x, const float* gy, int Bn, bool want_gx, bool want_gp, int act, float slope,
                const float* y_act, int gsel, int pre_rows, bool want_planes) {
  vf_ctx* ctx = n->ctx;
  VF_REQUIRE(n->train, "vf_net_backward: BatchNorm backward in evaluate mode is not part of the path");
  const float* gamma = n->params + l.w_off;
  float* gg = want_gp ? n->grads + l.w_off : nullptr;
  float* gbt = want_gp ? n->grads + l.b_off : nullptr;
  float* gx = want_gx ? l.gx : nullptr;
  float pbeta = 1.f;
  if (want_gp) {
    pbeta = l.fresh ? 0.f : 1.f;
    l.fresh = false;
  }
  l.grad_planes = nullptr;
  const int G = gsel >= 0 ? 1 : n->groups;
  const int row = gsel >= 0 ? gsel : 0;
  float *sm = l.sm + (int64_t)row * l.C, *si = l.si + (int64_t)row * l.C;
  double* su = l.sums + (int64_t)row * 2 * l.C;
  const int64_t npix_g = (int64_t)Bn * l.H * l.W / G;
  void* gp = nullptr;
  if (want_planes && gx && !sync_on(n)) {
    if (int rc = ensure_planes(n, &l.bgp, (int64_t)n->B * l.H * l.W * l.C)) return rc;
    gp = l.bgp;
  }
  if (pre_rows > 0) {
    int rc = vf_bn_bwd_pre(ctx, l.part, pre_rows, x, gy, gx, gg, gbt, gamma, sm, si, su, npix_g, l.C, G, pbeta, gp);
    l.grad_planes = gp;
    return rc;
  }
  if (!sync_on(n)) {
    int rc = gp ? vf_bn_bwd_planes(ctx, x, y_act, gy, gx, gg, gbt, gamma, sm, si, su, npix_g, l.C, G, act, slope, pbeta, gp)
                : vf_bn_bwd_groups(ctx, x, y_act, gy, gx, gg, gbt, gamma, sm, si, su, npix_g, l.C, G, act, slope, pbeta);
    l.grad_planes = gp;
    return rc;
  }
  VF_REQUIRE(G == 1 && gsel < 0, "SyncBN with batch groups is not part of the path");
  const int64_t npix = (int64_t)Bn * l.H * l.W, n_total = npix * n->sync_world;
  if (int rc = vf_bn_bwd_stats(ctx, x, y_act, gy, sm, su, npix, l.C, act, slope)) return rc;
  if (want_gp)
    if (int rc = vf_bn_bwd_apply(ctx, x, y_act, gy, nullptr, gg, gbt, gamma, sm, si, su, npix, n_total, l.C, act, slope, pbeta)) return rc;
  if (n->comm)
    if (int rc = vf_comm_allreduce_inline(n->comm, ctx, su, 2 * l.C, 1, 0)) return rc;
  if (want_gx) return vf_bn_bwd_apply(ctx, x, y_act, gy, gx, nullptr, nullptr, gamma, sm, si, su, npix, n_total, l.C, act, slope, 1.f);
  return 0;
}

int bias_grad_flush(vf_net* n, const std::vector<Deferred>& items) {
  if (items.empty()) return 0;
  std::string key((const char*)items.data(), items.size() * sizeof(Deferred));
  auto it = n->colsum_plans.find(key);
  if (it == n->colsum_plans.end()) {
    std::vector<VfColsumDesc> desc(items.size());
    char* ws = vf_ws_ptr(n->ctx);
    size_t off = 0;
    int b1 = 0, b2 = 0;
    for (size_t i = 0; i < items.size(); ++i) {
      const Deferred& d = items[i];
      int cq, rpb, gx, gy;
      if (int rc = vf_bias_grad_plan(d.P, d.C, &cq, &rpb, &gx, &gy)) return rc;
      desc[i] = VfColsumDesc{d.g, d.gb, (double*)(ws + off), d.P, d.C, cq, rpb, gx, gy, b1, b2, d.beta};
      off += ((size_t)gx * d.C * 8 + 255) / 256 * 256;
      b1 += gx * gy;
      b2 += (d.C + 3) / 4;
    }
    VF_REQUIRE(off <= vf_ws_avail(n->ctx), "vf_net: workspace too small for the bias-gradient partials");
    void* dev = nullptr;
    if (int rc = net_alloc(n->owned, &dev, desc.size() * sizeof(VfColsumDesc))) return rc;
    VF_CHECK_HIP(hipMemcpy(dev, desc.data(), desc.size() * sizeof(VfColsumDesc), hipMemcpyHostToDevice));
    it = n->colsum_plans.emplace(key, std::make_pair(dev, std::vector<int>{(int)items.size(), b1, b2})).first;
  }
  const std::vector<int>& g = it->second.second;
  return vf_bias_grad_multi(n->ctx, it->second.first, g[0], g[1], g[2]);
}

int net_walk_back(vf_net* n, const float* x_in, const float* gy, const float** gx_out, bool want_gp, bool need_input_grad, int hi,
                  int lo, int gi, int G, int defer_cut = -1) {
  vf_ctx* ctx = n->ctx;
  const int np = (int)n->plan.size();
  if (hi < 0 || hi > np) hi = np;
  VF_REQUIRE(lo >= 0 && lo <= hi, "vf_net backward: bad plan range [%d, %d)", lo, hi);
  VF_REQUIRE(gi < 0 || (!want_gp && G >= 1 && gi < G && n->B % G == 0), "vf_net: bad batch group %d of %d", gi, G);
  VF_REQUIRE(!(want_gp && n->split_pending), "vf_net: a split backward is pending — call vf_net_backward_finish first");
  const int Bn = gi >= 0 ? n->B / G : n->B;
  int cut_wg = -1;
  size_t cut_bias = 0;
  const float* g = gy;
  const void* g_pl = nullptr;
  std::vector<Deferred> deferred;
  bool act_done = hi < np ? (n->act_done_at == hi) : false;
  int bn_pre = 0, pre = 0;
  if (!n->wp_managed)
    if (int rc = refresh_weight_planes(n)) return rc;
  if (hi < np && n->bn_pre_at == hi) bn_pre = n->bn_pre_rows;
  n->bn_pre_at = -1;
  int rc = 0;
  if (want_gp && (rc = vf_wgrad_group_begin(ctx))) return rc;
  auto slice = [&](const float* p, int64_t per_sample) { return (gi >= 0 && p) ? p + (int64_t)gi * Bn * per_sample : p; };
  for (int idx = hi - 1; idx >= lo && !rc; --idx) {
    if (want_gp && defer_cut >= 0 && idx == defer_cut - 1) {
      if ((rc = vf_wgrad_group_count(ctx, &cut_wg))) break;
      cut_bias = deferred.size();
    }
    const Entry& e = n->plan[idx];
    Layer& l = n->L[e.main];
    const float* x = idx == 0 ? x_in : slice(entry_out(n, idx - 1, nullptr), (int64_t)l.H * l.W * l.C);
    const float* mout = slice(entry_out(n, idx, nullptr), (int64_t)l.Ho * l.Wo * l.Co);
    const bool want_gx = need_input_grad || idx > 0;
    const int64_t out_e = (int64_t)Bn * l.Ho * l.Wo * l.Co;
    if (l.d.kind == VF_L_BN) {
      const int rows = bn_pre;
      bn_pre = 0;
      bool want_pl = false;
      if (want_gx && idx > 0) {
        const Layer& below = n->L[n->plan[idx - 1].main];
        want_pl = is_conv(below) && pconv_layer(below) && (idx - 1 > 0 || need_input_grad) &&
                  pconv_ok(n, below, below.grad_shape(Bn), !is_full(below));
      }
      rc = bn_backward(n, l, x, g, Bn, want_gx, want_gp, l.fused_act, l.fused_slope, l.fused_act != VF_ACT_NONE ? mout : nullptr,
                       gi, rows, want_pl);
      g = l.gx;
      g_pl = l.grad_planes;
      act_done = false;
      continue;
    }
    if (is_conv(l)) {
      const float* go = g;
      VfConvExtras ex;
      const bool dot_head = l.d.kind == VF_L_CONV && l.Co == 1 && l.d.k == 4 && l.d.stride == 1 && l.d.pad == 0 && l.H == 4 && l.W == 4 &&
                            l.fused_act != VF_ACT_NONE && !relu_like(l.fused_act) && !act_done;
      if (l.fused_act != VF_ACT_NONE && !act_done && !dot_head) {
        const bool ours = g != gy;
        if (relu_like(l.fused_act) && ours) {
          rc = vf_act_bwd(ctx, mout, g, const_cast<float*>(g), out_e, l.fused_act, l.fused_slope);
          g_pl = nullptr;
        } else {
          if (!l.gtmp && (rc = net_alloc(n->act_owned, (void**)&l.gtmp, sizeof(float) * (size_t)n->B * l.Ho * l.Wo * l.Co))) break;
          rc = vf_act_bwd(ctx, mout, g, l.gtmp, out_e, l.fused_act, l.fused_slope);
          go = l.gtmp;
          g_pl = nullptr;
        }
        if (rc) break;
      }
      int in_act = VF_ACT_NONE;
      float in_slope = 0.f;
      const unsigned* in_bits = nullptr;
      if (want_gx && idx > 0 && l.d.kind == VF_L_CONV && is_s2(l)) {
        const Layer& pm = n->L[n->plan[idx - 1].main];
        if (is_conv(pm) && relu_like(pm.fused_act)) {
          in_act = pm.fused_act;
          in_slope = pm.fused_slope;
          if (pm.bits_live && pm.ybits && !n->observer)
            in_bits = pm.ybits + (gi >= 0 ? (int64_t)gi * Bn * pm.Ho * pm.Wo * (pm.Co / 32) : 0);
        }
      }
      bool fuse_below = false;
      if (want_gx && idx > 1) {
        Layer& pm = n->L[n->plan[idx - 1].main];
        if (pm.d.kind == VF_L_BN && bn_fusable(n, pm) && (pm.fused_act == VF_ACT_NONE || relu_like(pm.fused_act)) && pm.C == l.C &&
            (gi < 0 || n->groups == G)) {
          const float* xbn = slice(entry_out(n, idx - 2, nullptr), (int64_t)pm.H * pm.W * pm.C);
          const float* yact = pm.fused_act != VF_ACT_NONE ? x : nullptr;
          const float* smv = gi >= 0 ? pm.sm + (int64_t)gi * pm.C : pm.sm;
          if ((rc = vf_internal_bn_request_bwd(&ex.bn, xbn, yact, pm.fused_act, pm.fused_slope, smv, pm.part, pm.part_rows_cap,
                                               gi >= 0 ? 1 : n->groups)))
            break;
          fuse_below = true;
        }
      }
      ex.dot_act_y = dot_head ? mout : nullptr;
      ex.dot_act = l.fused_act;
      ex.dot_act_slope = l.fused_slope;
      if (want_gx) {
        if (!fuse_below && in_act != VF_ACT_NONE) ex.dmask_bits = in_bits;
        rc = conv_bwd_data(n, l, x, go, Bn, fuse_below ? VF_ACT_NONE : in_act, in_slope, g_pl, &ex);
        pre = ex.bn_result_rows;
        if (rc) break;
      }
      if (want_gp) {
        rc = conv_acc(n, l, x, go, Bn, &deferred, &ex);
        if (rc) break;
      }
      g = want_gx ? l.gx : nullptr;
      g_pl = nullptr;
      act_done = !fuse_below && in_act != VF_ACT_NONE && want_gx;
      bn_pre = pre;
      pre = 0;
      continue;
    }
    if (l.d.kind == VF_L_ACT && !l.absorbed) {
      rc = vf_act_bwd(ctx, mout, g, l.gx, out_e, l.d.act, l.d.slope);
      g = l.gx;
      g_pl = nullptr;
    }
    act_done = false;
  }
  if (want_gp) {
    if (rc) {
      (void)vf_wgrad_group_abort(ctx);
      return rc;
    }
    if (defer_cut >= 0 && cut_wg >= 0) {
      if ((rc = vf_wgrad_group_end_partial(ctx, cut_wg))) return rc;
      std::vector<Deferred> first(deferred.begin(), deferred.begin() + cut_bias);
      if ((rc = bias_grad_flush(n, first))) return rc;
      n->pending_bias.assign((const char*)(deferred.data() + cut_bias), (deferred.size() - cut_bias) * sizeof(Deferred));
      n->split_pending = true;
    } else {
      if ((rc = vf_wgrad_group_end(ctx))) return rc;
      if ((rc = bias_grad_flush(n, deferred))) return rc;
    }
  }
  if (rc) return rc;
  n->act_done_at = act_done ? lo : -1;
  if (bn_pre && lo > 0) {
    n->bn_pre_at = lo;
    n->bn_pre_rows = bn_pre;
  }
  if (gx_out) *gx_out = g;
  return 0;
}

void free_pool(std::vector<void*>& pool) {
  for (void* p : pool) (void)hipFree(p);
  pool.clear();
}

int net_shape(vf_net* n, int B, int C, int H, int W) {
  free_pool(n->act_owned);
  n->colsum_plans.clear();
  n->B = B; n->C0 = C; n->H0 = H; n->W0 = W;
  n->act_done_at = n->bn_pre_at = -1;
  int c = C, h = H, w = W;
  for (size_t i = 0; i < n->L.size(); ++i) {
    Layer& l = n->L[i];
    l.C = c; l.H = h; l.W = w;
    l.Co = c; l.Ho = h; l.Wo = w;
    switch (l.d.kind) {
      case VF_L_CONV:
      case VF_L_FULLCONV:
        VF_REQUIRE(l.d.nin == c, "vf_net: layer %d expects %d input planes, gets %d", (int)i, l.d.nin, c);
        l.Co = l.d.nout;
        l.Ho = is_full(l) ? l.shape(B).full_out_h() : l.shape(B).out_h();
        l.Wo = is_full(l) ? l.shape(B).full_out_w() : l.shape(B).out_w();
        break;
      case VF_L_BN:
        VF_REQUIRE(l.d.nout == c, "vf_net: BatchNorm layer %d has %d channels, gets %d", (int)i, l.d.nout, c);
        break;
      default:
        break;
    }
    VF_REQUIRE(l.Ho > 0 && l.Wo > 0, "vf_net: layer %d has an empty output", (int)i);
    c = l.Co; h = l.Ho; w = l.Wo;
    l.y = l.y_own = l.gx = l.gtmp = nullptr;
    l.xp = l.gp = l.yp = l.bgp = nullptr;
    l.ybits = nullptr;
    l.bits_live = false;
    l.out_planes = l.grad_planes = nullptr;
    l.x_seen = l.g_seen = nullptr;
    l.xp_seen = l.gp_seen = nullptr;
    l.part = nullptr;
    l.sm = l.si = nullptr;
    l.sums = nullptr;
  }
  n->gcap = std::max(n->groups, 2);
  for (size_t i = 0; i < n->L.size(); ++i) {
    Layer& l = n->L[i];
    const size_t in_e = (size_t)B * l.H * l.W * l.C, out_e = (size_t)B * l.Ho * l.Wo * l.Co;
    const bool own_out = is_conv(l) || l.d.kind == VF_L_BN || (l.d.kind == VF_L_ACT && !l.absorbed);
    if (own_out) {
      if (int rc = net_alloc(n->act_owned, (void**)&l.y_own, sizeof(float) * out_e)) return rc;
      l.y = l.y_own;
    }
    if (is_conv(l) || l.d.kind == VF_L_BN || (l.d.kind == VF_L_ACT && !l.absorbed))
      if (int rc = net_alloc(n->act_owned, (void**)&l.gx, sizeof(float) * in_e)) return rc;
    if (l.d.kind == VF_L_BN) {
      const size_t gc = (size_t)n->gcap * l.C;
      if (int rc = net_alloc(n->act_owned, (void**)&l.sm, 4 * gc)) return rc;
      if (int rc = net_alloc(n->act_owned, (void**)&l.si, 4 * gc)) return rc;
      if (int rc = net_alloc(n->act_owned, (void**)&l.sums, 16 * gc)) return rc;
      const int64_t npix = (int64_t)B * l.H * l.W;
      l.part_rows_cap = (int)std::max<int64_t>(npix / 64, 512) + 8 * n->gcap;
      if (int rc = net_alloc(n->act_owned, (void**)&l.part, sizeof(double) * (size_t)l.part_rows_cap * 2 * l.C)) return rc;
      (void)hipMemsetAsync(l.sm, 0, 4 * gc, n->ctx->stream);
      (void)hipMemsetAsync(l.si, 0, 4 * gc, n->ctx->stream);
      (void)hipMemsetAsync(l.sums, 0, 16 * gc, n->ctx->stream);
    }
  }
  return 0;
}

}
// ... 107 lines not shown
      if (hipMemcpy(n->bias_offs, boffs.data(), 8 * boffs.size(), hipMemcpyHostToDevice) != hipSuccess ||
          hipMemcpy(n->bias_lens, blens.data(), 8 * blens.size(), hipMemcpyHostToDevice) != hipSuccess) {
        vf_set_error("vf_net_create: hipMemcpy failed");
        rc = 1;
      }
    }
  }
  if (!rc) rc = net_shape(n, B, C, H, W);
  if (rc) {
    vf_net_destroy(n);
    return rc;
  }
  *out = n;
  return 0;
}

VF_API int vf_net_reshape(vf_net* n, int B, int C, int H, int W) {
  VF_REQUIRE(n && B > 0 && C > 0 && H > 0 && W > 0, "vf_net_reshape: bad arguments");
  if (B == n->B && C == n->C0 && H == n->H0 && W == n->W0) return 0;
  VF_CHECK_HIP(hipStreamSynchronize(n->ctx->stream));
  return net_shape(n, B, C, H, W);
}

VF_API int vf_net_parameters(vf_net* n, float** params, float** grads, int64_t* count) {
  VF_REQUIRE(n != nullptr, "vf_net_parameters: NULL net");
  if (params) *params = n->params;
  if (grads) *grads = n->grads;
  if (count) *count = n->nparams;
  return 0;
}
VF_API int vf_net_bind_parameters(vf_net* n, float* params, float* grads, int64_t count) {
  VF_REQUIRE(n != nullptr, "vf_net_bind_parameters: NULL net");
  if (!params && !grads) {
    n->params = n->params_own;
    n->grads = n->grads_own;
  } else {
    VF_REQUIRE(params && grads && count >= n->nparams, "vf_net_bind_parameters: need both buffers of >= %lld floats", (long long)n->nparams);
    VF_REQUIRE((((uintptr_t)params | (uintptr_t)grads) & 15) == 0, "vf_net_bind_parameters: buffers must be 16-byte aligned");
    n->params = params;
    n->grads = grads;
  }
  for (Layer& l : n->L) l.wp_live = false;
  n->wp_key.clear();
  n->colsum_plans.clear();
  n->both_tables.clear();
  return 0;
}
VF_API int64_t vf_net_param_offset(const vf_net* n, int layer, int which, int64_t* length) {
  if (!n || layer < 0 || layer >= (int)n->L.size() || n->L[layer].w_off < 0) return -1;
  const Layer& l = n->L[layer];
  if (length) *length = which ? l.b_n : l.w_n;
  return which ? l.b_off : l.w_off;
}
VF_API int vf_net_bn_running(vf_net* n, int layer, float** running_mean, float** running_var) {
  VF_REQUIRE(n && layer >= 0 && layer < (int)n->L.size() && n->L[layer].d.kind == VF_L_BN, "vf_net_bn_running: layer %d is not a BatchNorm", layer);
  if (running_mean) *running_mean = n->L[layer].rm;
  if (running_var) *running_var = n->L[layer].rv;
  return 0;
}
VF_API int vf_net_bind_bn_running(vf_net* n, int layer, float* running_mean, float* running_var) {
  VF_REQUIRE(n && layer >= 0 && layer < (int)n->L.size() && n->L[layer].d.kind == VF_L_BN, "vf_net_bind_bn_running: layer %d is not a BatchNorm", layer);
  VF_REQUIRE(running_mean && running_var, "vf_net_bind_bn_running: NULL buffer");
  n->L[layer].rm = running_mean;
  n->L[layer].rv = running_var;
  return 0;
}
VF_API int vf_net_bn_saved(vf_net* n, int layer, float** save_mean, float** save_invstd) {
  VF_REQUIRE(n && layer >= 0 && layer < (int)n->L.size() && n->L[layer].d.kind == VF_L_BN, "vf_net_bn_saved: layer %d is not a BatchNorm", layer);
  if (save_mean) *save_mean = n->L[layer].sm;
  if (save_invstd) *save_invstd = n->L[layer].si;
  return 0;
}
VF_API int vf_net_training(vf_net* n, int train) {
  VF_REQUIRE(n != nullptr, "vf_net_training: NULL net");
  n->train = train != 0;
  return 0;
}
VF_API int vf_net_zero_grad(vf_net* n) {
  VF_REQUIRE(n != nullptr, "vf_net_zero_grad: NULL net");
  for (Layer& l : n->L) {
    l.fresh = true;
    l.fa_k = 0;
  }
  return 0;
}
VF_API int vf_net_zero_conv_biases(vf_net* n, vf_net* other) {
  VF_REQUIRE(n != nullptr, "vf_net_zero_conv_biases: NULL net");
  if (!other || other == n || other->nbias == 0) {
    if (n->nbias == 0) return 0;
    return vf_zero_segments(n->ctx, n->params, n->bias_offs, n->bias_lens, n->nbias);
  }
  auto it = n->both_tables.find(other);
  if (it != n->both_tables.end() && (it->second.base != n->params || it->second.other_base != other->params)) {
    n->both_tables.erase(it);
    it = n->both_tables.end();
  }
  if (it == n->both_tables.end()) {
    std::vector<int64_t> offs((size_t)n->nbias + other->nbias), lens(offs.size());
    if (n->nbias) {
      VF_CHECK_HIP(hipMemcpy(offs.data(), n->bias_offs, 8 * (size_t)n->nbias, hipMemcpyDeviceToHost));
      VF_CHECK_HIP(hipMemcpy(lens.data(), n->bias_lens, 8 * (size_t)n->nbias, hipMemcpyDeviceToHost));
    }
    VF_CHECK_HIP(hipMemcpy(offs.data() + n->nbias, other->bias_offs, 8 * (size_t)other->nbias, hipMemcpyDeviceToHost));
    VF_CHECK_HIP(hipMemcpy(lens.data() + n->nbias, other->bias_lens, 8 * (size_t)other->nbias, hipMemcpyDeviceToHost));
    const int64_t delta = other->params - n->params;
    for (int i = 0; i < other->nbias; ++i) offs[n->nbias + i] += delta;
    int64_t *d_offs = nullptr, *d_lens = nullptr;
    if (int rc = net_alloc(n->owned, (void**)&d_offs, 8 * offs.size())) return rc;
    if (int rc = net_alloc(n->owned, (void**)&d_lens, 8 * lens.size())) return rc;
    VF_CHECK_HIP(hipMemcpy(d_offs, offs.data(), 8 * offs.size(), hipMemcpyHostToDevice));
    VF_CHECK_HIP(hipMemcpy(d_lens, lens.data(), 8 * lens.size(), hipMemcpyHostToDevice));
    it = n->both_tables.emplace(other, vf_net::BothTable{d_offs, d_lens, n->params, other->params}).first;
  }
  return vf_zero_segments(n->ctx, n->params, it->second.offs, it->second.lens, n->nbias + other->nbias);
}

VF_API int vf_net_layer_output(vf_net* n, int layer, const float** y) {
  VF_REQUIRE(n && y && layer >= 0 && layer < (int)n->L.size(), "vf_net_layer_output: bad layer");
  const float* p = nullptr;
  for (int i = 0; i <= layer; ++i)
    if (n->L[i].y) p = n->L[i].y;
  *y = p;
  return 0;
}
VF_API int vf_net_layer_grad_input(vf_net* n, int layer, const float** gx) {
  VF_REQUIRE(n && gx && layer >= 0 && layer < (int)n->L.size(), "vf_net_layer_grad_input: bad layer");
  *gx = n->L[layer].gx;
  return 0;
}
VF_API int vf_net_layer_shape(const vf_net* n, int layer, int* B, int* C, int* H, int* W, int* Co, int* Ho, int* Wo) {
  VF_REQUIRE(n && layer >= 0 && layer < (int)n->L.size(), "vf_net_layer_shape: bad layer");
  const Layer& l = n->L[layer];
  if (B) *B = n->B;
  if (C) *C = l.C;
  if (H) *H = l.H;
  if (W) *W = l.W;
  if (Co) *Co = l.Co;
  if (Ho) *Ho = l.Ho;
  if (Wo) *Wo = l.Wo;
  return 0;
}
VF_API int vf_net_bind_output(vf_net* n, int layer, float* y) {
  VF_REQUIRE(n && layer >= 0 && layer < (int)n->L.size() && n->L[layer].y_own, "vf_net_bind_output: layer %d owns no output", layer);
  n->L[layer].y = y ? y : n->L[layer].y_own;
  return 0;
}

VF_API int vf_net_set_batch_groups(vf_net* n, int G) {
  VF_REQUIRE(n && G >= 1 && G <= 64, "vf_net_set_batch_groups: bad group count %d", G);
  if (G > n->gcap) {
    n->groups = G;
    VF_CHECK_HIP(hipStreamSynchronize(n->ctx->stream));
    return net_shape(n, n->B, n->C0, n->H0, n->W0);
  }
  n->groups = G;
  return 0;
}
VF_API int vf_net_set_skip_input_grad(vf_net* n, int on) {
  VF_REQUIRE(n != nullptr, "vf_net_set_skip_input_grad: NULL net");
  n->skip_input_grad = on != 0;
  return 0;
}
VF_API int vf_net_set_weight_planes_managed(vf_net* n, int on) {
  VF_REQUIRE(n != nullptr, "vf_net_set_weight_planes_managed: NULL net");
  n->wp_managed = on != 0;
  return 0;
// ... 65 lines not shown
        if ((rc = vf_comm_wait(n->fwd_wait_comm, ctx, t))) return rc;
      n->fwd_wait_tickets.clear();
      n->fwd_wait_comm = nullptr;
    }
    if (is_conv(l)) {
      VfConvExtras ex;
      if (l.fused_act == VF_ACT_NONE && nxt && nxt->d.kind == VF_L_BN && bn_fusable(n, *nxt) && nxt->d.nout == l.Co) {
        if ((rc = vf_internal_bn_request_fwd(&ex.bn, nxt->rm, nxt->part, nxt->part_rows_cap, n->groups))) return rc;
        if ((rc = conv_forward(n, l, cur, cur_pl, n->B, VF_ACT_NONE, 0.f, false, &ex))) return rc;
        pre_rows = ex.bn_result_rows;
        cur = l.y;
        cur_pl = nullptr;
        continue;
      }
      const bool want_pl = nxt && is_conv(*nxt) && pconv_layer(*nxt) &&
                           pconv_ok(n, *nxt, nxt->shape(n->B), is_full(*nxt));
      if ((rc = conv_forward(n, l, cur, cur_pl, n->B, l.fused_act, l.fused_slope, want_pl, &ex))) return rc;
      cur = l.y;
      cur_pl = l.out_planes;
      if (relu_like(l.fused_act) && (rc = run_observer(n, e.act, l.y, (int64_t)n->B * l.Ho * l.Wo * l.Co, cur_pl))) return rc;
      continue;
    }
    if (l.d.kind == VF_L_BN) {
      const int rows = pre_rows;
      pre_rows = 0;
      const bool want_pl = n->train && nxt && is_conv(*nxt) && pconv_layer(*nxt) && (l.fused_act == VF_ACT_NONE || relu_like(l.fused_act)) &&
                           pconv_ok(n, *nxt, nxt->shape(n->B), is_full(*nxt));
      if ((rc = bn_forward(n, l, cur, n->B, l.fused_act, l.fused_slope, rows, want_pl))) return rc;
      cur = l.y;
      cur_pl = l.out_planes;
      if (relu_like(l.fused_act) && (rc = run_observer(n, e.act, l.y, (int64_t)n->B * l.H * l.W * l.C, cur_pl))) return rc;
      continue;
    }
    cur_pl = nullptr;
    if (l.d.kind == VF_L_ACT && !l.absorbed) {
      if ((rc = vf_act_fwd(ctx, cur, l.y, (int64_t)n->B * l.H * l.W * l.C, l.d.act, l.d.slope))) return rc;
      cur = l.y;
      if (relu_like(l.d.act) && (rc = run_observer(n, e.main, l.y, (int64_t)n->B * l.H * l.W * l.C, nullptr))) return rc;
    }
  }
  if (y) *y = cur;
  return 0;
}

VF_API int vf_net_backward(vf_net* n, const float* x, const float* gy, const float** gx) {
  VF_REQUIRE(n && x && gy, "vf_net_backward: NULL argument");
  return net_walk_back(n, x, gy, gx, true, !n->skip_input_grad, -1, 0, -1, 1);
}
VF_API int vf_net_backward_range(vf_net* n, const float* x, const float* gy, int hi, int lo, int need_input_grad, const float** gx) {
  VF_REQUIRE(n && x && gy, "vf_net_backward_range: NULL argument");
  return net_walk_back(n, x, gy, gx, true, need_input_grad != 0, hi, lo, -1, 1);
}
VF_API int vf_net_backward_split(vf_net* n, const float* x, const float* gy, int k, int need_input_grad, const float** gx) {
  VF_REQUIRE(n && x && gy && k >= 0 && k <= (int)n->plan.size(), "vf_net_backward_split: bad arguments");
  return net_walk_back(n, x, gy, gx, true, need_input_grad != 0, -1, 0, -1, 1, k);
}
VF_API int vf_net_backward_finish(vf_net* n) {
  VF_REQUIRE(n != nullptr, "vf_net_backward_finish: NULL net");
  if (!n->split_pending) return 0;
  n->split_pending = false;
  if (int rc = vf_wgrad_group_end(n->ctx)) return rc;
  std::vector<Deferred> rest(n->pending_bias.size() / sizeof(Deferred));
  memcpy(rest.data(), n->pending_bias.data(), n->pending_bias.size());
  n->pending_bias.clear();
  return bias_grad_flush(n, rest);
}
static bool fused_adam_shape(const Layer& l) {
  if (!is_conv(l) || l.d.k != 4 || l.d.stride != 1 || l.d.pad != 0 || l.w_off < 0 || (l.w_off & 3)) return false;
  const bool full = is_full(l);
  const int Nu = full ? l.C : l.Co, Cv = full ? l.Co : l.C;
  const bool maps = full ? (l.H == 1 && l.W == 1 && l.Ho == 4 && l.Wo == 4) : (l.H == 4 && l.W == 4 && l.Ho == 1 && l.Wo == 1);
  return maps && vf_wgrad_adam_outer_supported(1, Nu, 16 * Cv) && (int64_t)Nu * 16 * Cv == l.w_n;
}
VF_API int vf_net_set_fused_adam(vf_net* n, int on, int* count) {
  VF_REQUIRE(n != nullptr, "vf_net_set_fused_adam: NULL net");
  n->fa_layers.clear();
  for (size_t i = 0; i < n->L.size(); ++i) {
    Layer& l = n->L[i];
    l.fa = on && fused_adam_shape(l);
    l.fa_k = 0;
    if (l.fa) n->fa_layers.push_back((int)i);
  }
  n->fused_adam = !n->fa_layers.empty();
  if (count) *count = (int)n->fa_layers.size();
  return 0;
}
VF_API int vf_net_fused_adam_range(const vf_net* n, int i, int64_t* offset, int64_t* length) {
  VF_REQUIRE(n && offset && length && i >= 0 && i < (int)n->fa_layers.size(), "vf_net_fused_adam_range: layer %d of %d", i,
             n ? (int)n->fa_layers.size() : 0);
  const Layer& l = n->L[n->fa_layers[i]];
  *offset = l.w_off;
  *length = l.w_n;
  return 0;
}
static int64_t pad4(int64_t n) { return (n + 3) & ~(int64_t)3; }
static void fused_row_block(int Nu, int rank, int world, int* row0, int* nrows) {
  const int bs = 2 * ((Nu + 2 * world - 1) / (2 * world));
  const int r0 = std::min(Nu, rank * bs), r1 = std::min(Nu, r0 + bs);
  *row0 = r0;
  *nrows = r1 - r0;
}
static int fused_layers_launch(vf_net* n, const float* all, int world, int64_t seg_stride, float* m, float* v, double beta1, double beta2,
                               double eps, const int32_t* t_dev, int keep_grad, int row_rank = 0, int row_world = 1) {
  VfFusedLayer F[VF_FUSED_MAX];
  int nf = 0;
  int64_t off = 0;
  for (int i : n->fa_layers) {
    Layer& l = n->L[i];
    const bool full = is_full(l);
    const int Nu = full ? l.C : l.Co, Cv = full ? l.Co : l.C;
    float *x = n->params + l.w_off, *g = n->grads + l.w_off;
    if (all) VF_REQUIRE(l.fa_k == n->B, "vf_net_adam_fused_gathered: layer %d has no pending gradient", i);
    if (l.fa_k <= 0) {
      if (int rc = vf_adam_apply(n->ctx, x, g, m + l.w_off, v + l.w_off, l.w_n, beta1, beta2, eps, t_dev)) return rc;
      continue;
    }
    if (nf == VF_FUSED_MAX) {
      if (int rc = vf_internal_adam_fused_multi(n->ctx, F, nf, beta1, beta2, eps, t_dev)) return rc;
      nf = 0;
    }
    VfFusedLayer& L = F[nf++];
    if (all) {
      L.U = all + off;
      off += pad4((int64_t)l.fa_k * Nu);
      L.V = all + off;
      off += pad4((int64_t)l.fa_k * 16 * Cv);
      VF_REQUIRE(off <= seg_stride || world == 1, "vf_net_adam_fused_gathered: segments of %lld floats overlap", (long long)seg_stride);
    } else {
      L.U = l.fa_u;
      L.V = l.fa_v;
    }
    L.x = x; L.m = m + l.w_off; L.v = v + l.w_off; L.g_out = keep_grad ? g : nullptr;
    L.K = world * l.fa_k; L.Nu = Nu; L.Ncols = 16 * Cv;
    L.kps = l.fa_k; L.seg = all ? seg_stride : 0; L.gscale = 1.f / (float)world;
    L.row0 = 0; L.ldu = 0;
    if (row_world > 1) {
      int r0, nr;
      fused_row_block(Nu, row_rank, row_world, &r0, &nr);
      VF_REQUIRE(nr >= 64, "vf_net_adam_fused_gathered_rows: %d rows do not split over %d ranks (rank %d would hold %d; at least 64)", Nu,
                 row_world, row_rank, nr);
      L.ldu = Nu;
      L.Nu = nr;
      L.row0 = r0;
    }
    l.fa_k = 0;
  }
  return nf ? vf_internal_adam_fused_multi(n->ctx, F, nf, beta1, beta2, eps, t_dev) : 0;
}
VF_API int vf_net_adam_fused(vf_net* n, float* m, float* v, double beta1, double beta2, double eps, const int32_t* t_dev, int keep_grad) {
  VF_REQUIRE(n && m && v && t_dev, "vf_net_adam_fused: NULL argument");
  return fused_layers_launch(n, nullptr, 1, 0, m, v, beta1, beta2, eps, t_dev, keep_grad);
}
VF_API int vf_net_fused_adam_pack_size(const vf_net* n, int64_t* floats) {
  VF_REQUIRE(n && floats, "vf_net_fused_adam_pack_size: NULL argument");
  int64_t t = 0;
  for (int i : n->fa_layers) {
    const Layer& l = n->L[i];
    const bool full = is_full(l);
    const int Nu = full ? l.C : l.Co, Cv = full ? l.Co : l.C;
    t += pad4((int64_t)n->B * Nu) + pad4((int64_t)n->B * 16 * Cv);
  }
  *floats = t;
  return 0;
}
VF_API int vf_net_fused_adam_pack(vf_net* n, float* seg) {
  VF_REQUIRE(n && seg, "vf_net_fused_adam_pack: NULL argument");
  for (int i : n->fa_layers) {
    const Layer& l = n->L[i];
    const bool full = is_full(l);
    const int Nu = full ? l.C : l.Co, Cv = full ? l.Co : l.C;
    VF_REQUIRE(l.fa_k == n->B, "vf_net_fused_adam_pack: layer %d has no pending gradient of the net's batch (a backward pass with "
               "vf_net_set_fused_adam on comes first)", i);
    VF_CHECK_HIP(hipMemcpyAsync(seg, l.fa_u, (size_t)l.fa_k * Nu * sizeof(float), hipMemcpyDeviceToDevice, n->ctx->stream));
    seg += pad4((int64_t)l.fa_k * Nu);
    VF_CHECK_HIP(hipMemcpyAsync(seg, l.fa_v, (size_t)l.fa_k * 16 * Cv * sizeof(float), hipMemcpyDeviceToDevice, n->ctx->stream));
    seg += pad4((int64_t)l.fa_k * 16 * Cv);
  }
  return 0;
}
VF_API int vf_net_adam_fused_gathered(vf_net* n, const float* all, int world, int64_t seg_stride, float* m, float* v, double beta1,
                                      double beta2, double eps, const int32_t* t_dev, int keep_grad) {
  VF_REQUIRE(n && all && m && v && t_dev && world >= 1, "vf_net_adam_fused_gathered: bad argument");
  return fused_layers_launch(n, all, world, seg_stride, m, v, beta1, beta2, eps, t_dev, keep_grad);
}
VF_API int vf_net_fused_adam_rows_ok(const vf_net* n, int row_world) {
  if (!n || row_world < 1) return 0;
  int cnt = 0;
  for (const Layer& l : n->L) {
    if (!fused_adam_shape(l)) continue;
    const int Nu = is_full(l) ? l.C : l.Co;
    int r0, nr;
    fused_row_block(Nu, row_world - 1, row_world, &r0, &nr);
    if (nr < 64) return 0;
    ++cnt;
  }
  return cnt > 0;
}
VF_API int vf_net_fused_adam_row_range(const vf_net* n, int i, int row_rank, int row_world, int64_t* offset, int64_t* length) {
  VF_REQUIRE(n && offset && length && i >= 0 && i < (int)n->fa_layers.size() && row_world >= 1 && row_rank >= 0 && row_rank < row_world,
             "vf_net_fused_adam_row_range: bad argument");
  const Layer& l = n->L[n->fa_layers[i]];
  const bool full = is_full(l);
  const int Nu = full ? l.C : l.Co, Cv = full ? l.Co : l.C;
  int r0, nr;
  fused_row_block(Nu, row_rank, row_world, &r0, &nr);
  *offset = l.w_off + (int64_t)r0 * 16 * Cv;
  *length = (int64_t)nr * 16 * Cv;
  return 0;
}
VF_API int vf_net_forward_wait_fused(vf_net* n, vf_comm* comm, int ticket) {
  VF_REQUIRE(n && comm && ticket >= 0, "vf_net_forward_wait_fused: bad argument");
  VF_REQUIRE(n->fwd_wait_comm == nullptr || n->fwd_wait_comm == comm, "vf_net_forward_wait_fused: tickets of two communicators");
  n->fwd_wait_comm = comm;
  n->fwd_wait_tickets.push_back(ticket);
  return 0;
}
VF_API int vf_net_adam_fused_gathered_rows(vf_net* n, const float* all, int world, int64_t seg_stride, float* m, float* v, double beta1,
                                           double beta2, double eps, const int32_t* t_dev, int keep_grad, int row_rank, int row_world) {
  VF_REQUIRE(n && all && m && v && t_dev && world >= 1 && row_world >= 1 && row_rank >= 0 && row_rank < row_world,
             "vf_net_adam_fused_gathered_rows: bad argument");
  return fused_layers_launch(n, all, world, seg_stride, m, v, beta1, beta2, eps, t_dev, keep_grad, row_rank, row_world);
}
VF_API int vf_net_update_grad_input(vf_net* n, const float* x, const float* gy, const float** gx) {
  VF_REQUIRE(n && x && gy, "vf_net_update_grad_input: NULL argument");
  return net_walk_back(n, x, gy, gx, false, true, -1, 0, -1, 1);
}
VF_API int vf_net_update_grad_input_group(vf_net* n, const float* x, const float* gy, int g, int G, const float** gx) {
  VF_REQUIRE(n && x && gy, "vf_net_update_grad_input_group: NULL argument");
  return net_walk_back(n, x, gy, gx, false, true, -1, 0, g, G);
}
```

video-filler_amd/csrc/vf_wgrad_small.hip:

```cpp
#include <algorithm>
#include <cstdlib>

#include "vf_device.h"

namespace {

struct VfAdamFuse {
  float *x, *m, *v, *g;
  const int32_t* state;
  float b1, omb1, b2, omb2, eps;
  int round_bf16;
  int kps, kshift;
  int64_t seg;
  float gscale;
  const bf16x8* uf;
  const bf16x8* vf;
  int kg;
};
template <int NJ, bool FUSE, int RB, bool PF>
__device__ __forceinline__ void wgrad_smallk_body(const float* __restrict__ U, const float* __restrict__ V, float* __restrict__ dW, int K, int Nu,
                                                  int ldu, int Ncols, int tiles_c, float beta, const VfAdamFuse& A, int wt) {
  typedef float fvec __attribute__((ext_vector_type(NJ)));
  const int lane = threadIdx.x & 63;
  const int tr = wt / tiles_c, tc = wt - tr * tiles_c;
// ... 192 lines not shown
  int nl;
  int blk_off[VF_FUSED_MAX + 1];
  int tiles_c[VF_FUSED_MAX];
  int K[VF_FUSED_MAX], Nu[VF_FUSED_MAX], ldu[VF_FUSED_MAX], Ncols[VF_FUSED_MAX];
  const float* U[VF_FUSED_MAX];
  const float* V[VF_FUSED_MAX];
  VfAdamFuse A[VF_FUSED_MAX];
};
struct VfPrepTable {
  int nl;
  int blk_off[VF_FUSED_MAX + 1];
  int ut[VF_FUSED_MAX], vt[VF_FUSED_MAX];
  bf16x8* uf[VF_FUSED_MAX];
  bf16x8* vf[VF_FUSED_MAX];
};
__global__ __launch_bounds__(256) void k_fused_planes_prep(const VfFusedTable T, const VfPrepTable P) {
  int l = 0;
  while (l + 1 < P.nl && (int)blockIdx.x >= P.blk_off[l + 1]) ++l;
  const VfAdamFuse& A = T.A[l];
  const int kg = A.kg;
  const int64_t e = ((int64_t)((int)blockIdx.x - P.blk_off[l]) * 256 + threadIdx.x);
  const int lane = (int)(e & 63);
  const int64_t r = e >> 6;
  const int g = (int)(r % kg);
  const int64_t th = r / kg;
  const bool is_v = th >= 2 * (int64_t)P.ut[l];
  const int64_t th2 = is_v ? th - 2 * (int64_t)P.ut[l] : th;
  const int t = (int)(th2 >> 1), h = (int)(th2 & 1);
  const int ncols = is_v ? T.Ncols[l] : T.Nu[l];
  if (th >= 2 * (int64_t)(P.ut[l] + P.vt[l])) return;
  const int col = t * 64 + 2 * (lane & 31) + h;
  const float* base = is_v ? T.V[l] : T.U[l];
  const int ld = is_v ? T.Ncols[l] : T.ldu[l];
  float x[8];
#pragma unroll
  for (int q = 0; q < 8; ++q) {
    const int k = 16 * g + 8 * (lane >> 5) + q;
    float v = 0.f;
    if (k < T.K[l] && col < ncols) {
      if (A.seg != 0) {
        const int sg = A.kshift >= 0 ? k >> A.kshift : k / A.kps, kr = k - sg * A.kps;
        v = base[sg * A.seg + (int64_t)kr * ld + col];
      } else {
        v = base[(int64_t)k * ld + col];
      }
    }
    x[q] = v;
  }
  bf16x8* dst = (is_v ? P.vf[l] : P.uf[l]) + (((int64_t)(t * 2 + h) * kg + g) * 3) * 64 + lane;
#pragma unroll
  for (int p = 0; p < 3; ++p) {
    typedef unsigned short u16x8 __attribute__((ext_vector_type(8)));
    u16x8 o;
#pragma unroll
    for (int q = 0; q < 8; ++q) o[q] = (unsigned short)vf_trunc16(x[q]);
    *(u16x8*)(dst + p * 64) = o;
  }
}

template <int RB, int OCC>
__global__ __launch_bounds__(256, OCC) void k_adam_fused_multi(const VfFusedTable T) {
  int l = 0;
  while (l + 1 < T.nl && (int)blockIdx.x >= T.blk_off[l + 1]) ++l;
  const int wt = ((int)blockIdx.x - T.blk_off[l]) * 4 + (threadIdx.x >> 6);
  wgrad_smallk_body<2, true, RB, false>(T.U[l], T.V[l], (float*)nullptr, T.K[l], T.Nu[l], T.ldu[l], T.Ncols[l], T.tiles_c[l], 0.f, T.A[l], wt);
}

}

int vf_internal_wgrad_smallk(vf_ctx* ctx, const float* U, const float* V, float* dW, int K, int Nu, int Ncols, float beta) {
  if (ctx->mfma_bf16 == 1) return -1;
  if (K < 1 || K > 32 || Ncols % 128 != 0 || Nu % 2 != 0 || Nu < 64) return -1;
  if ((((uintptr_t)U) & 7) || (((uintptr_t)V) & 15) || (((uintptr_t)dW) & 15)) return -1;
  const int tiles_c = Ncols / 64, tiles_r = (int)vf_cdiv(Nu, 64);
  const int64_t wtiles = (int64_t)tiles_c * tiles_r;
  VfProf prof(ctx, "wgrad_smallk_f32", 2.0 * (double)K * Nu * Ncols, 4.0 * ((double)Nu * Ncols * (beta != 0.f ? 2 : 1) + (double)K * (Nu + Ncols)));
  hipLaunchKernelGGL((k_wgrad_smallk<2, false>), dim3((unsigned)vf_cdiv(wtiles, 4)), dim3(256), 0, ctx->stream, U, V, dW, K, Nu, Ncols, tiles_c, beta, VfAdamFuse{});
  VF_LAUNCH_CHECK();
  return 0;
}

VF_API int vf_wgrad_adam_outer_supported(int K, int Nu, int Ncols) {
  return K >= 1 && Ncols % 128 == 0 && Nu % 2 == 0 && Nu >= 64 && (int64_t)Nu * Ncols < ((int64_t)1 << 31);
}
int vf_internal_adam_fused_multi(vf_ctx* ctx, const VfFusedLayer* layers, int nl, double beta1, double beta2, double eps,
                                 const int32_t* t_dev) {
  VF_REQUIRE(ctx && layers && t_dev && nl >= 1 && nl <= VF_FUSED_MAX, "fused update: %d layers (at most %d per launch)", nl, VF_FUSED_MAX);
  VfFusedTable T;
  memset(&T, 0, sizeof(T));
  T.nl = nl;
  double flops = 0, bytes = 0;
  for (int i = 0; i < nl; ++i) {
    const VfFusedLayer& L = layers[i];
    VF_REQUIRE(L.U && L.V && L.x && L.m && L.v, "vf_wgrad_adam_outer: NULL argument");
    VF_REQUIRE(vf_wgrad_adam_outer_supported(L.K, L.Nu, L.Ncols), "vf_wgrad_adam_outer: K %d, %d x %d is not this kernel's shape", L.K, L.Nu,
               L.Ncols);
    VF_REQUIRE(L.kps >= 1 && L.K % L.kps == 0 && (L.K == L.kps || L.seg % 4 == 0),
               "vf_wgrad_adam_outer: %d batch rows in segments of %d (stride %lld floats)", L.K, L.kps, (long long)L.seg);
    const int ldu = L.ldu ? L.ldu : L.Nu, row0 = L.ldu ? L.row0 : 0;
    VF_REQUIRE(row0 >= 0 && row0 % 2 == 0 && row0 + L.Nu <= ldu, "vf_wgrad_adam_outer: rows [%d, %d) of %d", row0, row0 + L.Nu, ldu);
    VF_REQUIRE(!((((uintptr_t)L.U) | ((uintptr_t)L.V)) & 7) &&
                   !((((uintptr_t)L.x) | ((uintptr_t)L.m) | ((uintptr_t)L.v) | ((uintptr_t)L.g_out)) & 15),
               "vf_wgrad_adam_outer: U, V must be 8-byte aligned, x, m, v, g 16-byte aligned");
    const int64_t roff = (int64_t)row0 * L.Ncols;
    VfAdamFuse& F = T.A[i];
    F.x = L.x + roff; F.m = L.m + roff; F.v = L.v + roff; F.g = L.g_out ? L.g_out + roff : nullptr;
    F.state = t_dev;
    F.b1 = (float)beta1; F.omb1 = (float)(1.0 - beta1);
    F.b2 = (float)beta2; F.omb2 = (float)(1.0 - beta2);
    F.eps = (float)eps;
    F.round_bf16 = ctx->mfma_bf16 == 1;
    F.kps = L.kps; F.kshift = vf_is_pow2(L.kps) ? vf_ilog2(L.kps) : -1;
    F.seg = L.K == L.kps ? 0 : L.seg;
    F.gscale = L.gscale;
    T.U[i] = L.U + row0; T.V[i] = L.V;
    T.K[i] = L.K; T.Nu[i] = L.Nu; T.ldu[i] = ldu; T.Ncols[i] = L.Ncols;
    T.tiles_c[i] = L.Ncols / 64;
    const int64_t tiles = (int64_t)T.tiles_c[i] * vf_cdiv(L.Nu, 64);
    T.blk_off[i + 1] = T.blk_off[i] + (int)vf_cdiv(tiles, 4);
    const double n = (double)L.Nu * L.Ncols;
    flops += 2.0 * L.K * n;
    bytes += (L.g_out ? 28.0 : 24.0) * n + 4.0 * L.K * ((double)L.Nu + L.Ncols);
  }
  {
    bool ok = ctx->mfma_bf16 == 3;
    size_t need = 0;
    for (int i = 0; i < nl && ok; ++i) {
      ok = T.K[i] >= 64 && T.K[i] % 16 == 0;
      need += (size_t)(vf_cdiv(T.Nu[i], 64) + T.Ncols[i] / 64) * 2 * (T.K[i] / 16) * 3 * 64 * 16;
    }
    if (ok && need <= vf_ws_avail(ctx)) {
      VfPrepTable P;
      memset(&P, 0, sizeof(P));
      P.nl = nl;
      bf16x8* w = (bf16x8*)vf_ws_ptr(ctx);
      for (int i = 0; i < nl; ++i) {
        const int kg = T.K[i] / 16;
        P.ut[i] = (int)vf_cdiv(T.Nu[i], 64);
        P.vt[i] = T.Ncols[i] / 64;
        P.uf[i] = w;
        w += (size_t)P.ut[i] * 2 * kg * 3 * 64;
        P.vf[i] = w;
        w += (size_t)P.vt[i] * 2 * kg * 3 * 64;
        T.A[i].uf = P.uf[i];
        T.A[i].vf = P.vf[i];
        T.A[i].kg = kg;
        P.blk_off[i + 1] = P.blk_off[i] + (int)vf_cdiv((int64_t)(P.ut[i] + P.vt[i]) * 2 * kg * 64, 256);
      }
      VfProf prof(ctx, "adam_fused_operand_planes", 0.0, (double)need * (1.0 + 4.0 / 6.0));
      hipLaunchKernelGGL(k_fused_planes_prep, dim3((unsigned)P.blk_off[nl]), dim3(256), 0, ctx->stream, T, P);
      VF_LAUNCH_CHECK();
    }
  }
  VF_LAUNCH_TIMED(ctx, "adam_fused_wgrad", flops, bytes, (k_adam_fused_multi<4, 3>), dim3((unsigned)T.blk_off[nl]), dim3(256), T);
  VF_LAUNCH_CHECK();
  return 0;
}
VF_API int vf_wgrad_adam_outer_gathered(vf_ctx* ctx, const float* U, const float* V, int K, int rows_per_seg, int64_t seg_stride, int Nu,
                                        int Ncols, float* x, float* m, float* v, float* g, float gscale, double beta1, double beta2,
                                        double eps, const int32_t* t_dev) {
  VF_REQUIRE(ctx && U && V && x && m && v && t_dev, "vf_wgrad_adam_outer: NULL argument");
  VfFusedLayer L;
  L.U = U; L.V = V; L.x = x; L.m = m; L.v = v; L.g_out = g;
  L.K = K; L.Nu = Nu; L.Ncols = Ncols;
  L.kps = rows_per_seg; L.seg = seg_stride; L.gscale = gscale;
  L.row0 = 0; L.ldu = 0;
  return vf_internal_adam_fused_multi(ctx, &L, 1, beta1, beta2, eps, t_dev);
}
VF_API int vf_wgrad_adam_outer_rows(vf_ctx* ctx, const float* U, const float* V, int K, int rows_per_seg, int64_t seg_stride, int Nu,
                                    int Ncols, int row0, int nrows, float* x, float* m, float* v, float* g, float gscale, double beta1,
                                    double beta2, double eps, const int32_t* t_dev) {
  VF_REQUIRE(ctx && U && V && x && m && v && t_dev, "vf_wgrad_adam_outer_rows: NULL argument");
  VfFusedLayer L;
  L.U = U; L.V = V; L.x = x; L.m = m; L.v = v; L.g_out = g;
  L.K = K; L.Nu = nrows; L.Ncols = Ncols;
  L.kps = rows_per_seg; L.seg = seg_stride; L.gscale = gscale;
  L.row0 = row0; L.ldu = Nu;
  return vf_internal_adam_fused_multi(ctx, &L, 1, beta1, beta2, eps, t_dev);
}
VF_API int vf_wgrad_adam_outer(vf_ctx* ctx, const float* U, const float* V, int K, int Nu, int Ncols, float* x, float* m, float* v,
                               float* g, double beta1, double beta2, double eps, const int32_t* t_dev) {
  return vf_wgrad_adam_outer_gathered(ctx, U, V, K, K, 0, Nu, Ncols, x, m, v, g, 1.f, beta1, beta2, eps, t_dev);
}
```

video-filler_amd/optim.py:

```python
import torch

from .backend import bump_param_version, get_backend


def adam(opfunc, x, state):
    fx, dfdx = opfunc(x)
    adam_update(x, dfdx, state)
    return x, [fx]


def adam_init(x, state):
    if "m" not in state:
        state["t"] = 0
        state["m"] = torch.zeros_like(x)
        state["v"] = torch.zeros_like(x)
        state["t_dev"] = get_backend().zeros(2, dtype=torch.int32)
    return state


def adam_update(x, dfdx, state):
    B = get_backend()
    lr = state.get("learningRate", 0.001)
    beta1 = state.get("beta1", 0.9)
    beta2 = state.get("beta2", 0.999)
    eps = state.get("epsilon", 1e-8)
    if "m" not in state:
        adam_init(x, state)
    state["t"] += 1
    B.adam_step(x, dfdx, state["m"], state["v"], lr, beta1, beta2, eps, state["t_dev"])
    bump_param_version(x)


def adam_update_split(x, dfdx, state, side_ranges, side):
    B = get_backend()
    lr = state.get("learningRate", 0.001)
    beta1 = state.get("beta1", 0.9)
    beta2 = state.get("beta2", 0.999)
    eps = state.get("epsilon", 1e-8)
    adam_init(x, state)
    state["t"] += 1
    m, v, t_dev = state["m"], state["v"], state["t_dev"]
    B.adam_prep(lr, beta1, beta2, t_dev)
    with side.on():
        for lo, hi in side_ranges:
            side.adam_apply(x[lo:hi], dfdx[lo:hi], m[lo:hi], v[lo:hi], beta1, beta2, eps, t_dev)
    pos = 0
    for lo, hi in sorted(side_ranges) + [(x.numel(), x.numel())]:
        if lo > pos:
            B.adam_apply(x[pos:lo], dfdx[pos:lo], m[pos:lo], v[pos:lo], beta1, beta2, eps, t_dev)
        pos = hi
    bump_param_version(x)


def adam_update_fused(x, dfdx, state, net, keep_grad=False, gathered=None, rows=None):
    B = get_backend()
    lr = state.get("learningRate", 0.001)
    beta1 = state.get("beta1", 0.9)
    beta2 = state.get("beta2", 0.999)
    eps = state.get("epsilon", 1e-8)
    adam_init(x, state)
    state["t"] += 1
    m, v, t_dev = state["m"], state["v"], state["t_dev"]
    B.adam_prep(lr, beta1, beta2, t_dev)
    pos, plain = 0, []
    for lo, hi in sorted(net.fused_adam_ranges()) + [(x.numel(), x.numel())]:
        if lo > pos:
            plain.append((pos, lo))
        pos = hi
    if hasattr(B, "adam_apply_ranges") and len(plain) <= 8 and all(a % 4 == 0 and b % 4 == 0 for a, b in plain):
        B.adam_apply_ranges(x, dfdx, m, v, plain, beta1, beta2, eps, t_dev)
    else:
        for a, b in plain:
            B.adam_apply(x[a:b], dfdx[a:b], m[a:b], v[a:b], beta1, beta2, eps, t_dev)
    if gathered is not None:
        net.adam_fused_gathered(gathered[0], gathered[1], m, v, beta1, beta2, eps, t_dev, keep_grad, rows=rows)
    else:
        net.adam_fused(m, v, beta1, beta2, eps, t_dev, keep_grad)
    bump_param_version(x)
```

video-filler_amd/trainers.py:

```python
import os

import torch

from . import data, nn, optim
from .backend import bump_param_version, get_backend, to_nhwc

DEFAULT_OPT_TRAIN = dict(batchSize=64, fineSize=128, nBottleneck=100, nef=64, ngf=64, ndf=64, nc=3, wtl2=0.0,
                         overlapPred=0, lr=0.0002, beta1=0.5, nz=100, conditionAdv=False, noiseGen=False,
                         noisetype="normal")
DEFAULT_OPT_VID = dict(batchSize=16, fineSize=128, nBottleneck=4000, nef=64, ngf=64, ndf=64, nc=3, predLen=4,
                       wtl2=0.999, weight_nomask=0.05, wtgdl=0.0, overlapPred=0, lr=0.0002, beta1=0.5,
                       nc_in=None, nc_out=None)


DEFAULT_HOST = os.environ.get("VF_HOST", "cabi")


def _host_nets(host, netG, netD, sync_world=1):
    host = host or DEFAULT_HOST
    assert host in ("mirror", "cabi"), host
    if getattr(get_backend(), "name", "") != "hip-gfx950":
        host = "mirror"
    if host == "cabi" and sync_world > 1 and getattr(get_backend(), "comm", None) is None:
        host = "mirror"
# ... 221 lines not shown

    def set_batch_d(self, on=True):
        assert not (on and self._pipelined), "the pipelined data-parallel step keeps netD's real pass separate"
        assert not (on and any(getattr(m, "sync_world", 1) > 1 for m in self.netD.leaves())), "batch_d and SyncBN do not combine"
        assert self._graph is None and self._graphs is None, "set_batch_d before capture()"
        self.batch_d = bool(on)
        self.netD.setBatchGroups(2 if on else 1)
        return self

    def _netD_both(self, real_in, fake_in):
        B = get_backend()
        n = real_in.shape[0]
        shp = (2 * n,) + tuple(real_in.shape[1:])
        if self._cat is None or tuple(self._cat.shape) != shp:
            self._cat = B.empty_act(*shp)
            self._cat_real = None
        key = (real_in.data_ptr(), self._batch_ver)
        if self._cat_real != key:
            B.copy(self._cat[:n], real_in)
            self._cat_real = key
        if fake_in.data_ptr() != self._cat[n:].data_ptr():
            B.copy(self._cat[n:], fake_in)
            self.netG.redirect_last_output(fake_in, self._cat[n:])
        out = self.netD.forward(self._cat)
        if self._cat_df is None or tuple(self._cat_df.shape) != tuple(out.shape):
            self._cat_df = B.zeros(out.numel()).view(out.shape)
        if hasattr(B, "bce_fwd_bwd") and out.is_contiguous():
            s0, s1 = self.criterion.next_slot(), self.criterion.next_slot()
            B.bce_fwd_bwd(out, self.real_label, self.fake_label, n, 2, s0, s1, self._cat_df)
            errD_real, errD_fake = nn.DeviceScalar.of(s0), nn.DeviceScalar.of(s1)
        else:
            errD_real = self.criterion.forward(out[:n], self.real_label)
            errD_fake = self.criterion.forward(out[n:], self.fake_label)
            B.bce_bwd(out[:n], self.real_label, self._cat_df[:n])
            B.bce_bwd(out[n:], self.fake_label, self._cat_df[n:])
        self.netD.backward(self._cat, self._cat_df, need_input_grad=not self.skip_dead_grads)
        return errD_real + errD_fake

    def _refresh_cat_real(self, real_in):
        self._batch_ver += 1
        if self.batch_d and self._cat is not None and self._cat.shape[0] == 2 * real_in.shape[0] and tuple(self._cat.shape[1:]) == tuple(real_in.shape[1:]):
            get_backend().copy(self._cat[:real_in.shape[0]], real_in)
            self._cat_real = (real_in.data_ptr(), self._batch_ver)

    def _netD_stale_output(self):
        out = self.netD.output
        return out[out.shape[0] // 2:] if self.batch_d else out

    def _netD_grad_input(self, x, df_do):
        if self.batch_d:
            return self.netD.updateGradInput(x, df_do, group=(1, 2))
        return self.netD.updateGradInput(x, df_do)

    def _allreduce_avg(self, flat):
        if self._comm_on() and not self._defer_comm:
            get_backend().all_reduce_avg(flat, self.world, self.group)

    def fDx(self, x):
        for _ in self._fDx_gen():
            pass
        return self.errD, self.gradParametersD

    def _backward_G(self, df_dg):
        need = not self.skip_dead_grads
        if self._split_g is not None:
            k, _ = self._split_g
            self.netG.backward_split(self._g_in(), df_dg, k, need)
            return
        self.netG.backward(self._g_in(), df_dg, need_input_grad=need)
        self._allreduce_avg(self.gradParametersG)

    def step(self):
        B = get_backend()
        assert not self.shard_adam, "shard_adam keeps its own 1 / world Adam state: use step_phased() (ADVICE r2)"
        every = self.__dict__.get("_sync_every")
        if every is None:
            every = self._sync_every = _eager_sync_every()
        if every and torch.cuda.is_available() and not torch.cuda.is_current_stream_capturing():
            self._eager_n = self.__dict__.get("_eager_n", 0) + 1
            if self._eager_n % every == 0:
                torch.cuda.synchronize()
        rng = B.range if hasattr(B, "range") else _no_range
        with rng("optim.adam(fDx)"):
            optim.adam(self.fDx, self.parametersD, self.optimStateD)
        with rng("optim.adam(fGx)"):
            if (self.defer_adam_g and self.side_g is not None) or self.adam_overlap:
                self.fGx(self.parametersG)
                self._pending_g = True
            elif self._fuse_adam_ranges():
                try:
                    self.fGx(self.parametersG)
                    optim.adam_update_fused(self.parametersG, self.gradParametersG, self.optimStateG, self.netG, self.fuse_adam == "keep")
                finally:
                    self.netG.set_fused_adam(False)
            else:
                optim.adam(self.fGx, self.parametersG, self.optimStateG)

    def _fuse_adam_possible(self, dp=None):
        from .cnet import CNet
        if dp is None:
            dp = self._comm_on()
        hosted = (isinstance(self.netG, CNet) and self.netG._net is not None) or getattr(self.netG, "fused_adam_emulated", False)
        ok = (self.fuse_adam != "off" and hosted and not self.shard_adam and not self.defer_adam_g and not self.adam_overlap)
        if dp and self.dp_fused == "reduced":
            return False
        return ok and (self._comm_on() and not self._pipelined if dp else not self._comm_on())

    def _dp_rows(self):
        rows = self.dp_fused == "rows" and self.world > 1 and bool(self._dpf) and self.netG.fused_adam_rows_ok(self.world)
        mark = self.optimStateG.get("row_shard")
        if mark is not None and (not rows or tuple(mark) != (self.rank, self.world)) and bool(self._dpf):
            raise RuntimeError("optimStateG holds Adam moments sharded by weight rows for rank %d of %d; this step would run as %s on rank "
                               "%d of %d: call gather_adam_state() first" % (mark[0], mark[1], "rows" if rows else self.dp_fused, self.rank, self.world))
        return rows

    def _exchange_rows(self, defer):
        B = get_backend()
        hs = []
        for per_rank in self._row_ranges or []:
            hs += B.all_gather_ranges(self.parametersG, per_rank, self.rank, self.group, async_op=True)
        self._rows_stale = False
        comm = getattr(B, "comm", None)
        tickets = [h.ticket for h in hs if hasattr(h, "ticket")]
        hook = defer and comm is not None and self._graphs is None and hasattr(self.netG, "forward_wait_fused") and len(tickets) == len(hs)
        if hook:
            self.netG.forward_wait_fused(comm, tickets)
        else:
            for h in hs:
                h.wait()
        if hs or self._row_ranges:
            bump_param_version(self.parametersG)
        return hook

    def gather_adam_state(self):
        if self.optimStateG.get("row_shard") is None:
            return
        B = get_backend()
        for key in ("m", "v"):
            for per_rank in self._row_ranges or []:
                B.all_gather_ranges(self.optimStateG[key], per_rank, self.rank, self.group)
        del self.optimStateG["row_shard"]

    def _fuse_adam_ranges(self):
        return self.netG.set_fused_adam(True) if self._fuse_adam_possible(dp=False) else []

    def fuse_adam_slices(self):
        if not self._fuse_adam_possible():
            return []
        r = self.netG.set_fused_adam(True)
        if not (self._comm_on() and self._dpf):
            self.netG.set_fused_adam(False)
        return r

    def fused_adam_ranges(self):
        return self.fuse_adam_slices() if self.fuse_adam == "on" else []

    def enable_adam_overlap(self, on=True, min_numel=4 << 20):
        assert self._graph is None and self._graphs is None, "enable_adam_overlap before capture()"
        self.adam_overlap = False
        from .cnet import CNet
        if not on or self._comm_on() or not hasattr(get_backend(), "fork") or isinstance(self.netG, CNet):
            return self
        plan = self.netG._plan or self.netG._build_plan()
        big = [(m, o, n) for m, name, gname, o, n in self.netG._flat[2] if name == "weight" and n >= min_numel]
        idxs = [i for i, (pm, _) in enumerate(plan) if any(pm is m for m, _, _ in big)]
        if not big or len(idxs) != len(big):
            return self
        if self.side_a is None:
            self.side_a = get_backend().fork(workspace_bytes=1 << 20)
        self._g_big = ([(o, o + n) for _, o, n in big], min(idxs))
        self.adam_overlap = True
        self.netG.set_weight_planes_managed(False)
        return self

    def _pending_then_forward(self, fwd):
        if self._pending_g and self.adam_overlap:
            ranges, idx = self._g_big
            optim.adam_update_split(self.parametersG, self.gradParametersG, self.optimStateG, ranges, self.side_a)
            self._pending_g = False
            self.netG.zeroConvBiases()
            return fwd(before=(idx, self.side_a.join))
        self._apply_pending_g_and_sweep()
        return fwd()

    def _apply_pending_g(self):
        if self._pending_g:
            optim.adam_update(self.parametersG, self.gradParametersG, self.optimStateG)
            self._pending_g = False
            self.netG.refresh_weight_planes()

    def _apply_pending_g_and_sweep(self):
        if self._pending_g:
            self._apply_pending_g()
            self.netG.zeroConvBiases()

    def _wait_inflight(self):
        for h in self._inflight:
            if h is not None:
                h.wait()
        self._inflight = []

    def flush(self):
        if self._rows_stale:
            self._exchange_rows(defer=False)
        if self._pending_g:
            assert not self.shard_adam, "shard_adam has no deferred full-vector update to flush"
            self._wait_inflight()
            self._apply_pending_g()
            if (self._graph is not None and (self.defer_adam_g or self.adam_overlap)) or (self._graphs is not None and self._pipelined):
                self._graph_stale = True

    def _phase_a(self):
        self._defer_comm = True
        self.fDx(self.parametersD)
        self._defer_comm = False

    def _phase_b(self):
        optim.adam_update(self.parametersD, self.gradParametersD, self.optimStateD)
        self._defer_comm = True
        self._split_g = self.netG.bucket_split()
        self._dpf = self.netG.set_fused_adam(True) if self._fuse_adam_possible(dp=True) else []
        try:
            self.fGx(self.parametersG)
            if self._dpf:
                seg = self.netG.fused_adam_pack_size()
                if self._opbuf is None or self._opbuf.numel() != seg * self.world:
                    self._opbuf = get_backend().zeros(seg * self.world)
# ... 469 lines not shown
```

Measured before the change: 23030.

## Fuse split-K weight-gradient slab reduction and weight-plane refresh into Adam finish kernel

Split-K weight-gradient slabs are held in the workspace instead of being reduced right after backward. A new multi-layer Adam finish kernel sums the slabs, applies Adam, and writes the bf16 native and transposed weight planes in one pass. This removes separate slab-reduce launches, a separate weight-plane refresh pass, and extra reads and writes of gradients and weights. In exchange the workspace stays occupied until the optimizer step, there is a large new kernel and API path, and the fused path now also runs for the discriminator.

Result: no change. 23230 (median of 3 runs) (+0.9%).

```diff
diff --git a/include/vf_hip.h b/include/vf_hip.h
--- a/include/vf_hip.h
+++ b/include/vf_hip.h
@@ -298,6 +298,8 @@
 int vf_net_set_fused_adam(vf_net* net, int on, int* count);
 int vf_net_fused_adam_range(const vf_net* net, int i, int64_t* offset, int64_t* length);
 int vf_net_adam_fused(vf_net* net, float* m, float* v, double beta1, double beta2, double eps, const int32_t* t_dev, int keep_grad);
+int vf_net_adam_finish(vf_net* net, float* m, float* v, double beta1, double beta2, double eps, const int32_t* t_dev, int keep_grad, int* planes_current);
+int vf_net_layer_finish_info(const vf_net* net, int layer, const void** planes_native, const void** planes_transposed, int* held_ksplit);
 int vf_net_fused_adam_pack_size(const vf_net* net, int64_t* floats);
 int vf_net_fused_adam_pack(vf_net* net, float* segment);
 int vf_net_adam_fused_gathered(vf_net* net, const float* all_segments, int world, int64_t seg_stride, float* m, float* v, double beta1,
diff --git a/video-filler_amd/_lib.py b/video-filler_amd/_lib.py
--- a/video-filler_amd/_lib.py
+++ b/video-filler_amd/_lib.py
@@ -166,6 +166,8 @@
     "vf_net_set_fused_adam": (i32, [vp, i32, C.POINTER(i32)]),
     "vf_net_fused_adam_range": (i32, [vp, i32, C.POINTER(i64), C.POINTER(i64)]),
     "vf_net_adam_fused": (i32, [vp, vp, vp, f64, f64, f64, vp, i32]),
+    "vf_net_adam_finish": (i32, [vp, vp, vp, f64, f64, f64, vp, i32, C.POINTER(i32)]),
+    "vf_net_layer_finish_info": (i32, [vp, i32, C.POINTER(vp), C.POINTER(vp), C.POINTER(i32)]),
     "vf_net_fused_adam_pack_size": (i32, [vp, C.POINTER(i64)]),
     "vf_net_fused_adam_pack": (i32, [vp, vp]),
     "vf_net_adam_fused_gathered": (i32, [vp, vp, i32, i64, vp, vp, f64, f64, f64, vp, i32]),
diff --git a/video-filler_amd/build.py b/video-filler_amd/build.py
--- a/video-filler_amd/build.py
+++ b/video-filler_amd/build.py
@@ -4,7 +4,7 @@
 import sys
 
 HERE = os.path.dirname(os.path.abspath(__file__))
-SRC = ["vf_core.hip", "vf_bn.hip", "vf_conv.hip", "vf_conv_generic.hip", "vf_pipeline.hip", "vf_image.hip", "vf_jpeg.hip", "vf_png.hip", "vf_png_decode.hip", "vf_jpeg_enc.hip", "vf_gif.hip", "vf_display.hip", "vf_metrics.hip", "vf_pgemm.hip", "vf_conv_thin.hip", "vf_comm.hip", "vf_wgrad_small.hip", "vf_smallm.hip", "vf_trace.hip", "vf_net.hip"]
+SRC = ["vf_core.hip", "vf_bn.hip", "vf_conv.hip", "vf_conv_generic.hip", "vf_pipeline.hip", "vf_image.hip", "vf_jpeg.hip", "vf_png.hip", "vf_png_decode.hip", "vf_jpeg_enc.hip", "vf_gif.hip", "vf_display.hip", "vf_metrics.hip", "vf_pgemm.hip", "vf_conv_thin.hip", "vf_comm.hip", "vf_wgrad_small.hip", "vf_finish.hip", "vf_smallm.hip", "vf_trace.hip", "vf_net.hip"]
 HIPCC = os.environ.get("HIPCC", "/opt/rocm/bin/hipcc")
 FLAGS = ["--offload-arch=gfx950", "-O3", "-std=c++17", "-fPIC", "-fvisibility=hidden", "-ffp-contract=off",
          "-Wall", "-Wno-unused-function", "-Xclang", "-target-feature", "-Xclang", "-packed-fp32-ops"]
diff --git a/video-filler_amd/cnet.py b/video-filler_amd/cnet.py
--- a/video-filler_amd/cnet.py
+++ b/video-filler_amd/cnet.py
@@ -192,11 +192,12 @@
         Bn, Cc, H, W = [d.value for d in dims[:4]]
         return Bn, Cc, H, W
 
-    def set_fused_adam(self, on=True):
+    def set_fused_adam(self, on=True, finish=False):
         assert self._net is not None, "set_fused_adam after the first forward"
         lib = _lib.load()
         cnt = C.c_int()
-        _lib.check(lib.vf_net_set_fused_adam(self._net, 1 if on else 0, C.byref(cnt)))
+        self._finish = bool(on and finish)
+        _lib.check(lib.vf_net_set_fused_adam(self._net, (2 if finish else 1) if on else 0, C.byref(cnt)))
         self._fused_ranges = []
         for i in range(cnt.value):
             o, n = C.c_int64(), C.c_int64()
@@ -210,6 +211,26 @@
     def adam_fused(self, m, v, beta1, beta2, eps, t_dev, keep_grad=False):
         _lib.check(_lib.load().vf_net_adam_fused(self._net, C.c_void_p(m.data_ptr()), C.c_void_p(v.data_ptr()), beta1, beta2, eps,
                                                  C.c_void_p(t_dev.data_ptr()), 1 if keep_grad else 0))
+
+    def finish_armed(self):
+        return self._net is not None and getattr(self, "_finish", False)
+
+    def adam_finish(self, m, v, beta1, beta2, eps, t_dev, keep_grad=False):
+        cur = C.c_int()
+        _lib.check(_lib.load().vf_net_adam_finish(self._net, C.c_void_p(m.data_ptr()), C.c_void_p(v.data_ptr()), beta1, beta2, eps,
+                                                  C.c_void_p(t_dev.data_ptr()), 1 if keep_grad else 0, C.byref(cur)))
+        return bool(cur.value)
+
+    def finish_info(self, module):
+        nat, tr, ks = C.c_void_p(), C.c_void_p(), C.c_int()
+        _lib.check(_lib.load().vf_net_layer_finish_info(self._net, self._index[id(module)], C.byref(nat), C.byref(tr), C.byref(ks)))
+        shape = (3, module.weight.numel())
+        view = lambda p: tensor_from_ptr(p.value, shape, module.weight.device, "<i2") if p.value else None
+        return view(nat), view(tr), ks.value
+
+    def planes_current(self):
+        if self._flat is not None:
+            self._wp_version = self._wp_written = param_version(self._flat[0])
 
     def fused_adam_pack_size(self):
         n = C.c_int64()
@@ -285,6 +306,8 @@
 
     def refresh_weight_planes(self):
         if self._flat is not None:
+            if getattr(self, "_wp_written", None) == param_version(self._flat[0]):
+                return
             self._wp_version = param_version(self._flat[0])
         if self._net is not None:
             _lib.check(_lib.load().vf_net_refresh_weight_planes(self._net))
diff --git a/video-filler_amd/csrc/vf_common.h b/video-filler_amd/csrc/vf_common.h
--- a/video-filler_amd/csrc/vf_common.h
+++ b/video-filler_amd/csrc/vf_common.h
@@ -248,6 +248,25 @@
 };
 #define VF_FUSED_MAX 4
 
+enum { VF_FIN_LINEAR = 0, VF_FIN_SCALAR = 1, VF_FIN_TILED = 2 };
+struct VfFinishEntry {
+  int64_t off, n;
+  const float* slab;
+  void *nat, *tr;
+  int kind, ksplit, lanes;
+  float beta;
+  int d0, d1, npl, tiles_c;
+};
+#define VF_FINISH_MAX 32
+struct VfHeldSlab {
+  float* dW;
+  const float* slab;
+  int64_t total;
+  int ksplit, lanes;
+  float beta;
+  size_t end;
+};
+
 __device__ __forceinline__ float vf_act_apply(float v, int act, float slope) {
   switch (act) {
     case VF_ACT_LRELU: return v > 0.f ? v : v * slope;
diff --git a/video-filler_amd/csrc/vf_conv.hip b/video-filler_amd/csrc/vf_conv.hip
--- a/video-filler_amd/csrc/vf_conv.hip
+++ b/video-filler_amd/csrc/vf_conv.hip
@@ -1548,6 +1548,8 @@
   std::vector<WgRec> recs;
   size_t ws_used = 0;
   bool open = false;
+  bool hold = false;
+  std::vector<VfHeldSlab> direct;
   void clear() {
     recs.clear();
     ws_used = 0;
@@ -1601,9 +1603,30 @@
   }
   return fire();
 }
-static int wg_flush(vf_ctx* ctx) {
+static int slab_reduce_lanes(const float* slab, const float* dst, int64_t total, int ksplit) {
+  if (total % 4 != 0 || ((((uintptr_t)slab) | ((uintptr_t)dst)) & 15) != 0 || ksplit <= 0) return 0;
+  return (total / 4 <= 8192 && ksplit >= 64) ? 16 : 4;
+}
+static int wg_flush(vf_ctx* ctx, std::vector<VfHeldSlab>* held = nullptr, size_t tail_bytes = 0) {
   WgRecorder& R = wg_recorder(ctx);
+  const size_t avail = vf_ws_avail(ctx);
+  auto slab_end = [&](const float* slab, size_t bytes) { return (size_t)((const char*)slab - vf_ws_ptr(ctx)) + bytes; };
+  auto fits = [&](size_t end) { return held && ((end + 255) & ~(size_t)255) + tail_bytes <= avail; };
+  for (VfHeldSlab& h : R.direct) {
+    h.end = slab_end(h.slab, (size_t)h.ksplit * h.total * sizeof(float));
+    if (fits(h.end)) {
+      held->push_back(h);
+      continue;
+    }
+    VfProf prof(ctx, "slab_reduce_wgrad", 0.0, 4.0 * (double)h.total * (h.ksplit + 1));
+    if (int rc = launch_slab_reduce(ctx, h.slab, h.dW, nullptr, h.total, 1, h.ksplit, VF_ACT_NONE, 0.f, h.beta)) return rc;
+  }
+  R.direct.clear();
   if (R.recs.empty()) return 0;
+  auto keeps = [&](const WgRec& r) {
+    return r.g.ksplit > 1 && r.g.beta == 0.f && r.p.total % 4 == 0 && (((uintptr_t)r.g.slab | (uintptr_t)r.g.dW) & 15) == 0 &&
+           fits(slab_end(r.g.slab, r.p.slab_bytes()));
+  };
   bool any_planes = false;
   for (const WgRec& r : R.recs) any_planes |= (r.bf == 4);
   if (any_planes)
@@ -1643,7 +1666,7 @@
           });
   VF_LAUNCH_CHECK();
   wg_pack<SlabGroup, VF_WG_GROUP_MAX>(
-      R.recs, 1, [](const WgRec& r) { return r.g.ksplit > 1; },
+      R.recs, 1, [&](const WgRec& r) { return r.g.ksplit > 1 && !keeps(r); },
       [](auto& d, const WgRec& r, double& bytes) {
         d.slab = r.g.slab;
         d.dst = r.g.dW;
@@ -1659,26 +1682,50 @@
         return 0;
       });
   VF_LAUNCH_CHECK();
+  if (held)
+    for (const WgRec& r : R.recs)
+      if (keeps(r)) held->push_back(VfHeldSlab{r.g.dW, r.g.slab, r.p.total, r.g.ksplit, 4, r.g.beta, slab_end(r.g.slab, r.p.slab_bytes())});
   R.clear();
   return 0;
 }
 VF_API int vf_wgrad_group_begin(vf_ctx* ctx) {
   WgRecorder& R = wg_recorder(ctx);
   if (R.open) R.clear();
+  R.direct.clear();
   R.open = true;
+  R.hold = false;
   return 0;
 }
 VF_API int vf_wgrad_group_abort(vf_ctx* ctx) {
   WgRecorder& R = wg_recorder(ctx);
   R.clear();
-  R.open = false;
+  R.direct.clear();
+  R.open = R.hold = false;
   return 0;
 }
 VF_API int vf_wgrad_group_end(vf_ctx* ctx) {
   WgRecorder& R = wg_recorder(ctx);
   VF_REQUIRE(R.open, "vf_wgrad_group_end: no group is open");
-  R.open = false;
+  R.open = R.hold = false;
   return wg_flush(ctx);
+}
+int vf_internal_wgrad_group_hold(vf_ctx* ctx) {
+  WgRecorder& R = wg_recorder(ctx);
+  VF_REQUIRE(R.open, "vf_internal_wgrad_group_hold: no group is open");
+  R.hold = true;
+  return 0;
+}
+int vf_internal_wgrad_group_end_hold(vf_ctx* ctx, size_t tail_bytes, VfHeldSlab* held, int cap, int* nheld) {
+  WgRecorder& R = wg_recorder(ctx);
+  VF_REQUIRE(R.open && held && nheld, "vf_internal_wgrad_group_end_hold: no group is open");
+  const bool hold = R.hold;
+  R.open = R.hold = false;
+  std::vector<VfHeldSlab> h;
+  const int rc = wg_flush(ctx, hold ? &h : nullptr, tail_bytes);
+  VF_REQUIRE((int)h.size() <= cap, "vf_internal_wgrad_group_end_hold: %d held layers, room for %d", (int)h.size(), cap);
+  std::copy(h.begin(), h.end(), held);
+  *nheld = (int)h.size();
+  return rc;
 }
 
 VF_API int vf_wgrad_group_count(vf_ctx* ctx, int* count) {
@@ -1731,9 +1778,12 @@
     return R.open ? 0 : wg_flush(ctx);
   }
   float* slab = slab_at(0);
+  bool own_slabs = false;
   if (R.open) {
-    if (R.reserve(p.slab_bytes(), vf_ws_avail(ctx), &off)) slab = slab_at(off);
-    else if (int rc = wg_flush(ctx)) return rc;
+    if (R.reserve(p.slab_bytes(), vf_ws_avail(ctx), &off)) {
+      slab = slab_at(off);
+      own_slabs = true;
+    } else if (int rc = wg_flush(ctx)) return rc;
   }
   const WGrad g = wg_desc(p, U, V, dW, slab, beta);
   const int bf = ctx->mfma_bf16;
@@ -1750,6 +1800,11 @@
   });
   VF_LAUNCH_CHECK();
   if (p.ksplit > 1) {
+    const int lanes = slab_reduce_lanes(g.slab, dW, p.total, p.ksplit);
+    if (R.open && R.hold && own_slabs && beta == 0.f && lanes != 0) {
+      R.direct.push_back(VfHeldSlab{dW, g.slab, p.total, p.ksplit, lanes, beta, 0});
+      return 0;
+    }
     VfProf prof(ctx, "slab_reduce_wgrad", 0.0, 4.0 * (double)p.total * (p.ksplit + 1));
     return launch_slab_reduce(ctx, g.slab, dW, nullptr, p.total, 1, p.ksplit, VF_ACT_NONE, 0.f, beta);
   }
diff --git a/video-filler_amd/csrc/vf_finish.hip b/video-filler_amd/csrc/vf_finish.hip
--- /dev/null
+++ b/video-filler_amd/csrc/vf_finish.hip
@@ -0,0 +1,254 @@
+#include <algorithm>
+
+#include "vf_device.h"
+
+namespace {
+
+struct VfFinishTable {
+  int n;
+  int blk_off[VF_FINISH_MAX + 1];
+  VfFinishEntry e[VF_FINISH_MAX];
+  float *x, *g, *m, *v;
+  float b1, omb1, b2, omb2, eps;
+  const int32_t* state;
+};
+static_assert(sizeof(VfFinishTable) <= 3584, "kernel arguments are limited to 4 KB");
+
+constexpr int FIN_T = 64;
+constexpr int FIN_LD = FIN_T + 1;
+constexpr int FIN_LIN_BLOCK = 4096;
+
+__device__ __forceinline__ int fin_lds(int row, int col) { return row * FIN_LD + col + ((row >> 5) << 1); }
+
+__device__ __forceinline__ void fin_upd4(const VfFinishTable& T, float step, f32x4& xv, const f32x4& gv, f32x4& mv, f32x4& vv) {
+#pragma unroll
+  for (int e = 0; e < 4; ++e) {
+    float xe = xv[e], me = mv[e], ve = vv[e];
+    vf_adam_upd(xe, gv[e], me, ve, T.b1, T.omb1, T.b2, T.omb2, T.eps, step);
+    xv[e] = xe;
+    mv[e] = me;
+    vv[e] = ve;
+  }
+}
+__device__ __forceinline__ void fin_store_planes(void* planes, int64_t pstride, int64_t idx, const f32x4& w, int npl) {
+  unsigned short* p = (unsigned short*)planes + idx;
+  if (npl == 1) {
+    *(u32x2*)p = vf_round4(w);
+  } else {
+    u32x2 o[3];
+    vf_split3(w, o);
+#pragma unroll
+    for (int q = 0; q < 3; ++q) *(u32x2*)(p + q * pstride) = o[q];
+  }
+}
+
+__global__ __launch_bounds__(256) void k_adam_finish_multi(const VfFinishTable T) {
+  int l = 0;
+  while (l + 1 < T.n && (int)blockIdx.x >= T.blk_off[l + 1]) ++l;
+  const VfFinishEntry& E = T.e[l];
+  const int local = (int)blockIdx.x - T.blk_off[l];
+  const int tid = threadIdx.x;
+  const float step = __int_as_float(T.state[1]);
+  float *x = T.x + E.off, *g = T.g + E.off, *m = T.m + E.off, *v = T.v + E.off;
+  const int ksplit = E.ksplit;
+  const float beta = E.beta;
+  __shared__ __attribute__((aligned(16))) float lds[FIN_T * FIN_LD + 2];
+
+  if (E.kind == VF_FIN_TILED) {
+    const int d0 = E.d0, d1 = E.d1, NC = 16 * d1;
+    const int r0 = (local / E.tiles_c) * FIN_T, c0 = (local % E.tiles_c) * FIN_T;
+    const int64_t total4 = E.n >> 2, pstride = E.n;
+    const int cl = (tid & 15) * 4, rl = tid >> 4;
+    const bool col_ok = c0 + cl < NC;
+#pragma unroll 1
+    for (int h = 0; h < 2; ++h) {
+      bool ok[2];
+      int64_t i4[2];
+      f32x4 gv[2], xv[2], mv[2], vv[2];
+#pragma unroll
+      for (int i = 0; i < 2; ++i) {
+        const int row = r0 + rl + 16 * (2 * h + i);
+        ok[i] = col_ok && row < d0;
+        i4[i] = ok[i] ? ((int64_t)row * NC + c0 + cl) >> 2 : 0;
+      }
+      if (E.slab) {
+        const f32x4* slab = (const f32x4*)E.slab;
+        f32x4 s[2][4];
+#pragma unroll
+        for (int i = 0; i < 2; ++i)
+#pragma unroll
+          for (int sl = 0; sl < 4; ++sl) s[i][sl] = f32x4{0.f, 0.f, 0.f, 0.f};
+        int k = 0;
+        for (; k + 4 <= ksplit; k += 4) {
+          f32x4 t[2][4];
+#pragma unroll
+          for (int sl = 0; sl < 4; ++sl)
+#pragma unroll
+            for (int i = 0; i < 2; ++i) t[i][sl] = slab[(int64_t)(k + sl) * total4 + i4[i]];
+#pragma unroll
+          for (int sl = 0; sl < 4; ++sl)
+#pragma unroll
+            for (int i = 0; i < 2; ++i) s[i][sl] += t[i][sl];
+        }
+#pragma unroll
+        for (int i = 0; i < 2; ++i) {
+          xv[i] = ((const f32x4*)x)[i4[i]];
+          mv[i] = ((const f32x4*)m)[i4[i]];
+          vv[i] = ((const f32x4*)v)[i4[i]];
+        }
+#pragma unroll
+        for (int sl = 0; sl < 3; ++sl)
+          if (k + sl < ksplit) {
+            const f32x4 t0 = slab[(int64_t)(k + sl) * total4 + i4[0]], t1 = slab[(int64_t)(k + sl) * total4 + i4[1]];
+            s[0][sl] += t0;
+            s[1][sl] += t1;
+          }
+#pragma unroll
+        for (int i = 0; i < 2; ++i) {
+          gv[i] = ((s[i][0] + s[i][1]) + s[i][2]) + s[i][3];
+          if (beta != 0.f) gv[i] += beta * ((const f32x4*)g)[i4[i]];
+          if (ok[i]) ((f32x4*)g)[i4[i]] = gv[i];
+        }
+      } else {
+#pragma unroll
+        for (int i = 0; i < 2; ++i) {
+          gv[i] = ((const f32x4*)g)[i4[i]];
+          xv[i] = ((const f32x4*)x)[i4[i]];
+          mv[i] = ((const f32x4*)m)[i4[i]];
+          vv[i] = ((const f32x4*)v)[i4[i]];
+        }
+      }
+#pragma unroll
+      for (int i = 0; i < 2; ++i) {
+        fin_upd4(T, step, xv[i], gv[i], mv[i], vv[i]);
+        if (ok[i]) {
+          ((f32x4*)x)[i4[i]] = xv[i];
+          ((f32x4*)m)[i4[i]] = mv[i];
+          ((f32x4*)v)[i4[i]] = vv[i];
+          if (E.nat) fin_store_planes(E.nat, pstride, i4[i] << 2, xv[i], E.npl);
+        }
+        const int row = rl + 16 * (2 * h + i);
+#pragma unroll
+        for (int e = 0; e < 4; ++e) lds[fin_lds(row, cl + e)] = xv[i][e];
+      }
+    }
+    if (!E.tr) return;
+    __syncthreads();
+    const int al = (tid & 15) * 4;
+#pragma unroll
+    for (int i = 0; i < 4; ++i) {
+      const int colL = (tid >> 4) + 16 * i, col = c0 + colL, a = r0 + al;
+      if (col < NC && a < d0) {
+        const int tap = col / d1, b = col - tap * d1;
+        f32x4 w;
+#pragma unroll
+        for (int e = 0; e < 4; ++e) w[e] = lds[fin_lds(al + e, colL)];
+        fin_store_planes(E.tr, pstride, ((int64_t)b * 16 + tap) * d0 + a, w, E.npl);
+      }
+    }
+    return;
+  }
+
+  if (E.kind == VF_FIN_SCALAR) {
+    for (int j = 0; j < FIN_LIN_BLOCK / 256; ++j) {
+      const int64_t i = (int64_t)local * FIN_LIN_BLOCK + j * 256 + tid;
+      if (i < E.n) vf_adam_upd(x[i], g[i], m[i], v[i], T.b1, T.omb1, T.b2, T.omb2, T.eps, step);
+    }
+    return;
+  }
+
+  if (E.slab) {
+    const int L = E.lanes, COLS = 256 / L;
+    const int tx = tid % COLS, sl = tid / COLS;
+    const int64_t total4 = E.n >> 2, i4 = (int64_t)local * COLS + tx;
+    f32x4 s = {0.f, 0.f, 0.f, 0.f};
+    if (i4 < total4) {
+#pragma unroll 4
+      for (int k = sl; k < ksplit; k += L) s += ((const f32x4*)E.slab)[(int64_t)k * total4 + i4];
+    }
+    f32x4* red = (f32x4*)lds;
+    red[sl * COLS + tx] = s;
+    __syncthreads();
+    if (sl == 0 && i4 < total4) {
+      f32x4 t = red[tx];
+      for (int q = 1; q < L; ++q) t += red[q * COLS + tx];
+      if (beta != 0.f) t += beta * ((const f32x4*)g)[i4];
+      ((f32x4*)g)[i4] = t;
+      f32x4 xv = ((const f32x4*)x)[i4], mv = ((const f32x4*)m)[i4], vv = ((const f32x4*)v)[i4];
+      fin_upd4(T, step, xv, t, mv, vv);
+      ((f32x4*)x)[i4] = xv;
+      ((f32x4*)m)[i4] = mv;
+      ((f32x4*)v)[i4] = vv;
+    }
+    return;
+  }
+
+  const int64_t n4 = E.n >> 2;
+#pragma unroll
+  for (int j = 0; j < FIN_LIN_BLOCK / 1024; ++j) {
+    const int64_t i4 = (int64_t)local * (FIN_LIN_BLOCK / 4) + j * 256 + tid;
+    if (i4 < n4) {
+      f32x4 xv = ((const f32x4*)x)[i4], mv = ((const f32x4*)m)[i4], vv = ((const f32x4*)v)[i4];
+      const f32x4 gv = ((const f32x4*)g)[i4];
+      fin_upd4(T, step, xv, gv, mv, vv);
+      ((f32x4*)x)[i4] = xv;
+      ((f32x4*)m)[i4] = mv;
+      ((f32x4*)v)[i4] = vv;
+    }
+  }
+  const int64_t it = (n4 << 2) + tid;
+  if (local == T.blk_off[l + 1] - T.blk_off[l] - 1 && it < E.n) vf_adam_upd(x[it], g[it], m[it], v[it], T.b1, T.omb1, T.b2, T.omb2, T.eps, step);
+}
+
+}
+
+int vf_internal_adam_finish(vf_ctx* ctx, const VfFinishEntry* entries, int ne, float* x, float* g, float* m, float* v, double beta1,
+                            double beta2, double eps, const int32_t* t_dev) {
+  VF_REQUIRE(ctx && entries && x && g && m && v && t_dev, "vf_internal_adam_finish: NULL argument");
+  VF_REQUIRE((((uintptr_t)x | (uintptr_t)g | (uintptr_t)m | (uintptr_t)v) & 15) == 0, "adam operands must be 16-byte aligned");
+  VfFinishTable T;
+  memset(&T, 0, sizeof(T));
+  T.x = x; T.g = g; T.m = m; T.v = v;
+  T.b1 = (float)beta1; T.omb1 = (float)(1.0 - beta1);
+  T.b2 = (float)beta2; T.omb2 = (float)(1.0 - beta2);
+  T.eps = (float)eps;
+  T.state = t_dev;
+  double bytes = 0;
+  auto fire = [&]() -> int {
+    if (T.n == 0) return 0;
+    VF_LAUNCH_TIMED(ctx, "adam_finish_multi", 0.0, bytes, k_adam_finish_multi, dim3((unsigned)T.blk_off[T.n]), dim3(256), T);
+    VF_LAUNCH_CHECK();
+    T.n = 0;
+    bytes = 0;
+    return 0;
+  };
+  for (int i = 0; i < ne; ++i) {
+    VfFinishEntry E = entries[i];
+    if (E.n <= 0) continue;
+    const bool tiled = E.kind == VF_FIN_TILED;
+    VF_REQUIRE(E.off >= 0 && (E.kind == VF_FIN_SCALAR || E.off % 4 == 0), "vf_internal_adam_finish: entry %d starts at element %lld", i,
+               (long long)E.off);
+    VF_REQUIRE(!E.slab || (E.kind != VF_FIN_SCALAR && E.n % 4 == 0 && ((uintptr_t)E.slab & 15) == 0 && E.ksplit >= 1 &&
+                           (tiled ? E.lanes == 4 : (E.lanes == 4 || E.lanes == 16))),
+               "vf_internal_adam_finish: entry %d: slabs need whole float4s and 4 (or, linear, 16) split lanes", i);
+    int blocks;
+    if (tiled) {
+      VF_REQUIRE(E.d0 > 0 && E.d1 > 0 && E.d0 % 4 == 0 && E.d1 % 4 == 0 && (int64_t)E.d0 * 16 * E.d1 == E.n && (E.npl == 1 || E.npl == 3) &&
+                     (((uintptr_t)E.nat | (uintptr_t)E.tr) & 7) == 0,
+                 "vf_internal_adam_finish: entry %d is no [%d][16][%d] weight with planes", i, E.d0, E.d1);
+      E.tiles_c = (16 * E.d1 + FIN_T - 1) / FIN_T;
+      blocks = E.tiles_c * ((E.d0 + FIN_T - 1) / FIN_T);
+    } else if (E.kind == VF_FIN_LINEAR && E.slab) {
+      blocks = (int)vf_cdiv(E.n / 4, 256 / E.lanes);
+    } else {
+      blocks = (int)vf_cdiv(E.n, FIN_LIN_BLOCK);
+    }
+    bytes += (double)E.n * (28.0 + (E.slab ? 4.0 * E.ksplit + (E.beta != 0.f ? 4.0 : 0.0) : 0.0) +
+                            (tiled ? 2.0 * E.npl * ((E.nat ? 1 : 0) + (E.tr ? 1 : 0)) : 0.0));
+    T.e[T.n] = E;
+    T.blk_off[T.n + 1] = T.blk_off[T.n] + blocks;
+    if (++T.n == VF_FINISH_MAX)
+      if (int rc = fire()) return rc;
+  }
+  return fire();
+}
diff --git a/video-filler_amd/csrc/vf_internal.h b/video-filler_amd/csrc/vf_internal.h
--- a/video-filler_amd/csrc/vf_internal.h
+++ b/video-filler_amd/csrc/vf_internal.h
@@ -1,5 +1,5 @@
 #pragma once
-struct vf_ctx; struct VfBnSt; struct VfBnRequest; struct VfConvExtras; struct VfPWGradGroup; struct VfFusedLayer; struct WgRecorder;
+struct vf_ctx; struct VfBnSt; struct VfBnRequest; struct VfConvExtras; struct VfPWGradGroup; struct VfFusedLayer; struct WgRecorder; struct VfFinishEntry; struct VfHeldSlab;
 
 struct VfConvShape {
   int B, H, W, Cin, Cout, k, stride, pad;
@@ -59,5 +59,12 @@
 int vf_internal_wgrad_smallk(vf_ctx* ctx, const float* U, const float* V, float* dW, int K, int Nu, int Ncols, float beta);
 int vf_internal_adam_fused_multi(vf_ctx* ctx, const VfFusedLayer* layers, int nl, double beta1, double beta2, double eps,
                                  const int32_t* t_dev);
+size_t vf_internal_adam_fused_prep_bytes(int K, int Nu, int Ncols);
 
 int vf_internal_colsum(vf_ctx* ctx, const float* g, float* gb, int64_t P, int C, float beta);
+
+int vf_internal_adam_finish(vf_ctx* ctx, const VfFinishEntry* entries, int ne, float* x, float* g, float* m, float* v, double beta1,
+                            double beta2, double eps, const int32_t* t_dev);
+
+int vf_internal_wgrad_group_hold(vf_ctx* ctx);
+int vf_internal_wgrad_group_end_hold(vf_ctx* ctx, size_t tail_bytes, VfHeldSlab* held, int cap, int* nheld);
diff --git a/video-filler_amd/csrc/vf_net.hip b/video-filler_amd/csrc/vf_net.hip
--- a/video-filler_amd/csrc/vf_net.hip
+++ b/video-filler_amd/csrc/vf_net.hip
@@ -50,6 +50,7 @@
   bool fa = false;
   const float *fa_u = nullptr, *fa_v = nullptr;
   int fa_k = 0;
+  VfHeldSlab fs = {};
   VfConvShape shape(int Bn) const { return {Bn, H, W, C, Co, d.k, d.stride, d.pad}; }
   VfConvShape grad_shape(int Bn) const { return d.kind == VF_L_FULLCONV ? shape(Bn).gradient_of_full() : shape(Bn).gradient_of_conv(); }
 };
@@ -99,6 +100,9 @@
   };
   std::map<const vf_net*, BothTable> both_tables;
   bool fused_adam = false;
+  bool finish_hold = false;
+  bool fs_pending = false;
+  size_t fs_front0 = 0;
   std::vector<int> fa_layers;
   vf_comm* fwd_wait_comm = nullptr;
   std::vector<int> fwd_wait_tickets;
@@ -156,6 +160,12 @@
   }
   if (edited > 0 && planes) return vf_planes_split(n->ctx, y, const_cast<void*>(planes), numel);
   return 0;
+}
+
+void finish_release(vf_net* n) {
+  for (Layer& l : n->L) l.fs = VfHeldSlab{};
+  if (n->fs_pending) n->ctx->ws_front = n->fs_front0;
+  n->fs_pending = false;
 }
 
 int weight_planes(vf_net* n, Layer& l, bool transposed, const void** out) {
@@ -337,6 +347,9 @@
     return vf_internal_colsum(ctx, go, gb, (int64_t)Bn * l.Ho * l.Wo, l.Co, beta);
   }
   l.fa_k = 0;
+  VF_REQUIRE(!(l.fs.slab && beta != 0.f), "finishing update: a second backward pass accumulates onto a weight gradient whose slabs were "
+                                          "left for vf_net_adam_finish (one backward per zeroGradParameters)");
+  l.fs = VfHeldSlab{};
   const bool planes = g_pwgrad && !g_no_pconv && l.x_seen == x && l.xp_seen && l.g_seen == go && l.gp_seen;
   const void *xp = l.xp_seen, *gp = l.gp_seen;
   l.g_seen = nullptr;
@@ -395,6 +408,8 @@
 int bias_grad_flush(vf_net* n, const std::vector<Deferred>& items) {
   if (items.empty()) return 0;
   std::string key((const char*)items.data(), items.size() * sizeof(Deferred));
+  const char* ws_base = vf_ws_ptr(n->ctx);
+  key.append((const char*)&ws_base, sizeof(ws_base));
   auto it = n->colsum_plans.find(key);
   if (it == n->colsum_plans.end()) {
     std::vector<VfColsumDesc> desc(items.size());
@@ -418,6 +433,35 @@
   }
   const std::vector<int>& g = it->second.second;
   return vf_bias_grad_multi(n->ctx, it->second.first, g[0], g[1], g[2]);
+}
+
+int finish_group_end(vf_net* n, const std::vector<Deferred>& deferred) {
+  vf_ctx* ctx = n->ctx;
+  size_t tail = 0;
+  for (const Deferred& d : deferred) {
+    int cq, rpb, gx, gy;
+    if (int rc = vf_bias_grad_plan(d.P, d.C, &cq, &rpb, &gx, &gy)) return rc;
+    tail += ((size_t)gx * d.C * 8 + 255) / 256 * 256;
+  }
+  VfHeldSlab held[64];
+  int nh = 0;
+  if (int rc = vf_internal_wgrad_group_hold(ctx)) return rc;
+  if (int rc = vf_internal_wgrad_group_end_hold(ctx, tail, held, 64, &nh)) return rc;
+  size_t end = 0;
+  for (int i = 0; i < nh; ++i) {
+    Layer* owner = nullptr;
+    for (Layer& l : n->L)
+      if (is_conv(l) && l.w_off >= 0 && n->grads + l.w_off == held[i].dW && l.w_n == held[i].total) owner = &l;
+    VF_REQUIRE(owner != nullptr, "vf_net: held split-K slabs belong to no layer of this net");
+    owner->fs = held[i];
+    end = std::max(end, held[i].end);
+  }
+  if (nh) {
+    if (!n->fs_pending) n->fs_front0 = ctx->ws_front;
+    n->fs_pending = true;
+    ctx->ws_front += (end + 255) & ~(size_t)255;
+  }
+  return 0;
 }
 
 int net_walk_back(vf_net* n, const float* x_in, const float* gy, const float** gx_out, bool want_gp, bool need_input_grad, int hi,
@@ -524,6 +568,8 @@
         if (rc) break;
       }
       if (want_gp) {
+        if (n->finish_hold && gi < 0 && defer_cut < 0 && idx == lo && l.Co % 4 == 0 && ((uintptr_t)go & 15) == 0)
+          if ((rc = vf_internal_wgrad_group_hold(ctx))) break;
         rc = conv_acc(n, l, x, go, Bn, &deferred, &ex);
         if (rc) break;
       }
@@ -553,7 +599,7 @@
       n->pending_bias.assign((const char*)(deferred.data() + cut_bias), (deferred.size() - cut_bias) * sizeof(Deferred));
       n->split_pending = true;
     } else {
-      if ((rc = vf_wgrad_group_end(ctx))) return rc;
+      if ((rc = n->finish_hold && gi < 0 ? finish_group_end(n, deferred) : vf_wgrad_group_end(ctx))) return rc;
       if ((rc = bias_grad_flush(n, deferred))) return rc;
     }
   }
@@ -827,6 +873,7 @@
     l.fresh = true;
     l.fa_k = 0;
   }
+  finish_release(n);
   return 0;
 }
 VF_API int vf_net_zero_conv_biases(vf_net* n, vf_net* other) {
@@ -1058,6 +1105,8 @@
     if (l.fa) n->fa_layers.push_back((int)i);
   }
   n->fused_adam = !n->fa_layers.empty();
+  n->finish_hold = on == 2;
+  finish_release(n);
   if (count) *count = (int)n->fa_layers.size();
   return 0;
 }
@@ -1125,7 +1174,97 @@
 }
 VF_API int vf_net_adam_fused(vf_net* n, float* m, float* v, double beta1, double beta2, double eps, const int32_t* t_dev, int keep_grad) {
   VF_REQUIRE(n && m && v && t_dev, "vf_net_adam_fused: NULL argument");
+  VF_REQUIRE(!n->fs_pending, "vf_net_adam_fused: split-K slabs are held for vf_net_adam_finish (vf_net_set_fused_adam(2))");
   return fused_layers_launch(n, nullptr, 1, 0, m, v, beta1, beta2, eps, t_dev, keep_grad);
+}
+VF_API int vf_net_adam_finish(vf_net* n, float* m, float* v, double beta1, double beta2, double eps, const int32_t* t_dev, int keep_grad,
+                              int* planes_current) {
+  VF_REQUIRE(n && m && v && t_dev, "vf_net_adam_finish: NULL argument");
+  const int mode = n->ctx->mfma_bf16;
+  const bool planes_on = n->wp_managed && !g_no_pconv && (mode == 3 || mode == 1);
+  std::vector<VfFinishEntry> special;
+  std::vector<std::pair<int64_t, int64_t>> taken;
+  bool current = planes_on;
+  for (Layer& l : n->L) {
+    if (!is_conv(l) || l.w_off < 0) continue;
+    if (n->fused_adam && l.fa) {
+      taken.emplace_back(l.w_off, l.w_n);
+      continue;
+    }
+    const int d0 = is_full(l) ? l.d.nin : l.d.nout, d1 = is_full(l) ? l.d.nout : l.d.nin;
+    const bool live = l.wp_live && l.wp_mode == mode;
+    const bool tiled = planes_on && live && l.d.k == 4 && l.w_off % 4 == 0 && d0 % 4 == 0 && d1 % 4 == 0 && (int64_t)d0 * 16 * d1 == l.w_n &&
+                       (!l.fs.slab || l.fs.lanes == 4);
+    if (live && !tiled) current = false;
+    if (!tiled && !l.fs.slab) continue;
+    VfFinishEntry E;
+    memset(&E, 0, sizeof(E));
+    E.off = l.w_off; E.n = l.w_n;
+    E.kind = tiled ? VF_FIN_TILED : VF_FIN_LINEAR;
+    if (l.fs.slab) {
+      VF_REQUIRE(l.fs.total == l.w_n && l.w_off % 4 == 0, "vf_net_adam_finish: held slabs do not match their layer");
+      E.slab = l.fs.slab; E.ksplit = l.fs.ksplit; E.lanes = l.fs.lanes; E.beta = l.fs.beta;
+    }
+    if (tiled) {
+      E.nat = l.wp_nat; E.tr = l.wp_tr;
+      E.d0 = d0; E.d1 = d1; E.npl = mode == 1 ? 1 : 3;
+    }
+    special.push_back(E);
+  }
+  std::sort(special.begin(), special.end(), [](const VfFinishEntry& a, const VfFinishEntry& b) { return a.off < b.off; });
+  std::sort(taken.begin(), taken.end());
+  std::vector<VfFinishEntry> entries;
+  auto linear = [&](int64_t lo, int64_t hi) {
+    for (const auto& t : taken) {
+      if (t.first >= hi || t.first + t.second <= lo) continue;
+      if (t.first > lo) {
+        VfFinishEntry E;
+        memset(&E, 0, sizeof(E));
+        E.off = lo; E.n = t.first - lo;
+        E.kind = lo % 4 == 0 ? VF_FIN_LINEAR : VF_FIN_SCALAR;
+        entries.push_back(E);
+      }
+      lo = t.first + t.second;
+    }
+    if (hi > lo) {
+      VfFinishEntry E;
+      memset(&E, 0, sizeof(E));
+      E.off = lo; E.n = hi - lo;
+      E.kind = lo % 4 == 0 ? VF_FIN_LINEAR : VF_FIN_SCALAR;
+      entries.push_back(E);
+    }
+  };
+  int64_t pos = 0;
+  for (const VfFinishEntry& E : special) {
+    linear(pos, E.off);
+    entries.push_back(E);
+    pos = E.off + E.n;
+  }
+  linear(pos, n->nparams);
+  size_t prep = 0;
+  for (int i : n->fa_layers) {
+    const Layer& l = n->L[i];
+    const bool full = is_full(l);
+    if (l.fa_k >= 64 && l.fa_k % 16 == 0) prep += vf_internal_adam_fused_prep_bytes(l.fa_k, full ? l.C : l.Co, 16 * (full ? l.Co : l.C));
+  }
+  const bool pair_first = !n->fs_pending || prep <= vf_ws_avail(n->ctx);
+  int rc = 0;
+  if (pair_first) rc = fused_layers_launch(n, nullptr, 1, 0, m, v, beta1, beta2, eps, t_dev, keep_grad);
+  if (!rc) rc = vf_internal_adam_finish(n->ctx, entries.data(), (int)entries.size(), n->params, n->grads, m, v, beta1, beta2, eps, t_dev);
+  finish_release(n);
+  if (!rc && !pair_first) rc = fused_layers_launch(n, nullptr, 1, 0, m, v, beta1, beta2, eps, t_dev, keep_grad);
+  if (rc) return rc;
+  if (planes_current) *planes_current = current ? 1 : 0;
+  return 0;
+}
+VF_API int vf_net_layer_finish_info(const vf_net* n, int layer, const void** planes_native, const void** planes_transposed, int* held_ksplit) {
+  VF_REQUIRE(n && layer >= 0 && layer < (int)n->L.size(), "vf_net_layer_finish_info: bad layer %d", layer);
+  const Layer& l = n->L[layer];
+  const bool live = l.wp_live && l.wp_mode == n->ctx->mfma_bf16;
+  if (planes_native) *planes_native = live ? l.wp_nat : nullptr;
+  if (planes_transposed) *planes_transposed = live ? l.wp_tr : nullptr;
+  if (held_ksplit) *held_ksplit = l.fs.slab ? l.fs.ksplit : 0;
+  return 0;
 }
 VF_API int vf_net_fused_adam_pack_size(const vf_net* n, int64_t* floats) {
   VF_REQUIRE(n && floats, "vf_net_fused_adam_pack_size: NULL argument");
diff --git a/video-filler_amd/csrc/vf_wgrad_small.hip b/video-filler_amd/csrc/vf_wgrad_small.hip
--- a/video-filler_amd/csrc/vf_wgrad_small.hip
+++ b/video-filler_amd/csrc/vf_wgrad_small.hip
@@ -298,6 +298,9 @@
 
 VF_API int vf_wgrad_adam_outer_supported(int K, int Nu, int Ncols) {
   return K >= 1 && Ncols % 128 == 0 && Nu % 2 == 0 && Nu >= 64 && (int64_t)Nu * Ncols < ((int64_t)1 << 31);
+}
+size_t vf_internal_adam_fused_prep_bytes(int K, int Nu, int Ncols) {
+  return (size_t)(vf_cdiv(Nu, 64) + Ncols / 64) * 2 * (K / 16) * 3 * 64 * 16;
 }
 int vf_internal_adam_fused_multi(vf_ctx* ctx, const VfFusedLayer* layers, int nl, double beta1, double beta2, double eps,
                                  const int32_t* t_dev) {
@@ -343,7 +346,7 @@
     size_t need = 0;
     for (int i = 0; i < nl && ok; ++i) {
       ok = T.K[i] >= 64 && T.K[i] % 16 == 0;
-      need += (size_t)(vf_cdiv(T.Nu[i], 64) + T.Ncols[i] / 64) * 2 * (T.K[i] / 16) * 3 * 64 * 16;
+      need += vf_internal_adam_fused_prep_bytes(T.K[i], T.Nu[i], T.Ncols[i]);
     }
     if (ok && need <= vf_ws_avail(ctx)) {
       VfPrepTable P;
diff --git a/video-filler_amd/optim.py b/video-filler_amd/optim.py
--- a/video-filler_amd/optim.py
+++ b/video-filler_amd/optim.py
@@ -62,6 +62,13 @@
     state["t"] += 1
     m, v, t_dev = state["m"], state["v"], state["t_dev"]
     B.adam_prep(lr, beta1, beta2, t_dev)
+    if gathered is None and getattr(net, "finish_armed", lambda: False)():
+        assert net._flat[0].data_ptr() == x.data_ptr() and net._flat[1].data_ptr() == dfdx.data_ptr(), "the net's own flat vectors"
+        current = net.adam_finish(m, v, beta1, beta2, eps, t_dev, keep_grad)
+        bump_param_version(x)
+        if current:
+            net.planes_current()
+        return
     pos, plain = 0, []
     for lo, hi in sorted(net.fused_adam_ranges()) + [(x.numel(), x.numel())]:
         if lo > pos:
diff --git a/video-filler_amd/trainers.py b/video-filler_amd/trainers.py
--- a/video-filler_amd/trainers.py
+++ b/video-filler_amd/trainers.py
@@ -327,12 +327,20 @@
                 torch.cuda.synchronize()
         rng = B.range if hasattr(B, "range") else _no_range
         with rng("optim.adam(fDx)"):
-            optim.adam(self.fDx, self.parametersD, self.optimStateD)
+            if self.batch_d and self._fuse_adam_possible(dp=False) and self._finish_host(self.netD):
+                self.netD.set_fused_adam(True, finish=True)
+                try:
+                    self.fDx(self.parametersD)
+                    optim.adam_update_fused(self.parametersD, self.gradParametersD, self.optimStateD, self.netD, True)
+                finally:
+                    self.netD.set_fused_adam(False)
+            else:
+                optim.adam(self.fDx, self.parametersD, self.optimStateD)
         with rng("optim.adam(fGx)"):
             if (self.defer_adam_g and self.side_g is not None) or self.adam_overlap:
                 self.fGx(self.parametersG)
                 self._pending_g = True
-            elif self._fuse_adam_ranges():
+            elif self._fuse_adam_ranges() or (self._finish_host(self.netG) and self.netG.finish_armed()):
                 try:
                     self.fGx(self.parametersG)
                     optim.adam_update_fused(self.parametersG, self.gradParametersG, self.optimStateG, self.netG, self.fuse_adam == "keep")
@@ -340,6 +348,11 @@
                     self.netG.set_fused_adam(False)
             else:
                 optim.adam(self.fGx, self.parametersG, self.optimStateG)
+
+    @staticmethod
+    def _finish_host(net):
+        from .cnet import CNet
+        return isinstance(net, CNet) and net._net is not None
 
     def _fuse_adam_possible(self, dp=None):
         from .cnet import CNet
@@ -387,7 +400,11 @@
         del self.optimStateG["row_shard"]
 
     def _fuse_adam_ranges(self):
-        return self.netG.set_fused_adam(True) if self._fuse_adam_possible(dp=False) else []
+        if not self._fuse_adam_possible(dp=False):
+            return []
+        if self._finish_host(self.netG):
+            return self.netG.set_fused_adam(True, finish=True)
+        return self.netG.set_fused_adam(True)
 
     def fuse_adam_slices(self):
         if not self._fuse_adam_possible():
```
